# nuggy875/NeRF_pytorch_paeng

Hardware: AMD Instinct MI355X
Metric: rays/sec (4096-ray batch, 64c+128f samples) + 800×800 frame render ms (higher is better)
Workload: dtype f32

## Files before the change

### include/mi_nerf.h

```cpp
#ifndef MI_NERF_H
#define MI_NERF_H

#include <stddef.h>
#include <stdint.h>

#ifdef __cplusplus
extern "C" {
#endif

#define MI_NERF_ABI_VERSION 4

#define MI_NERF_MODE_F32 0
#define MI_NERF_MODE_BF16 1
#define MI_NERF_MODE_BF16_64 2
#define MI_NERF_MODE_BF16_32 3
#define MI_NERF_MODE_F16S 5
#define MI_NERF_MODE_F16S_BF16 6
#define MI_NERF_MODE_F16 8
#define MI_NERF_MODE_F16_BF16 9

#define MI_NERF_OK 0
#define MI_NERF_EINVAL 1
#define MI_NERF_EHIP 2
#define MI_NERF_ERCCL 3

int mi_nerf_abi_version(void);
const char* mi_nerf_last_error(void);

typedef struct mi_nerf_net {
    int32_t D;
    int32_t W;
    int32_t skip;
    int32_t L_x;
    int32_t L_d;
} mi_nerf_net;

typedef struct mi_nerf_params {
    const float* const* linear_x_w;
    const float* const* linear_x_b;
    const float* linear_density_w;
    const float* linear_density_b;
    const float* linear_feat_w;
    const float* linear_feat_b;
    const float* linear_d_w;
    const float* linear_d_b;
    const float* linear_color_w;
    const float* linear_color_b;
} mi_nerf_params;

size_t mi_nerf_packed_bytes(const mi_nerf_net* net);
int mi_nerf_pack_weights(const mi_nerf_net* net, const mi_nerf_params* params, void* host_blob, size_t blob_bytes);
size_t mi_nerf_packed_bytes_bf16(const mi_nerf_net* net);
int mi_nerf_pack_weights_bf16(const mi_nerf_net* net, const mi_nerf_params* params, void* host_blob, size_t blob_bytes);

int mi_nerf_make_o_d(int W, int H, const float k4[4], const float pose12[12], int row0, int n_rows,
                     float* rays_o_dev, float* rays_d_dev, void* stream);
int mi_nerf_make_o_d_pixels(int W, int H, const float k4[4], const float pose12[12], const int64_t* pix_dev,
                            int64_t n, float* rays_o_dev, float* rays_d_dev, void* stream);

int mi_nerf_ndc_rays(int H, int W, float focal, float near_, const float* o_in_dev, int64_t o_stride,
                     const float* d_in_dev, int64_t d_stride, int64_t n, float* o_out_dev, float* d_out_dev,
                     void* stream);

int mi_nerf_fill_uniform(uint32_t seed, uint32_t stream_id, int64_t ray0, int64_t n_rays, int n_samples,
                         float* out_dev, void* stream);

int mi_nerf_stratified_z(int64_t n_rays, int S, float near_, float far_, const float* t_rand_dev, float* z_dev,
                         void* stream);

int mi_nerf_sample_pdf(const float* bins_dev, const float* weights_dev, int64_t n, int B, int N, int det,
                       const float* u_dev, float* samples_dev, void* stream);
int mi_nerf_fine_z(const float* z_c_dev, const float* weights_c_dev, int64_t n, int Sc, int Nf, int det,
                   const float* u_dev, float* z_fine_dev, float* z_samples_dev, void* stream);

int mi_nerf_embed(const float* rays_dev, const float* z_dev, int64_t n_rays, int S, int L_x, int L_d,
                  float* embedded_dev, void* stream);

int mi_nerf_posenc(const float* x_dev, int64_t n, int L, float* out_dev, void* stream);

int mi_nerf_mlp_embedded(const mi_nerf_net* net, const void* packed_dev, const float* x_dev, int64_t n,
                         float* out_dev, void* stream);
int mi_nerf_mlp_rays(const mi_nerf_net* net, const void* packed_dev, const float* rays_dev, const float* z_dev,
                     int64_t n_rays, int S, float* raw_dev, void* stream);
int mi_nerf_mlp_rays_bf16(const mi_nerf_net* net, const void* packed_bf16_dev, const float* rays_dev,
                          const float* z_dev, int64_t n_rays, int S, float* raw_dev, void* stream);
int mi_nerf_mlp_rays_bf16_shape(const mi_nerf_net* net, const void* packed_bf16_dev, const float* rays_dev,
                                const float* z_dev, int64_t n_rays, int S, float* raw_dev, int points_per_wave, void* stream);

size_t mi_nerf_packed_bytes_f16s(const mi_nerf_net* net);
int mi_nerf_pack_weights_f16s(const mi_nerf_net* net, const mi_nerf_params* params, void* host_blob, size_t blob_bytes);
int mi_nerf_mlp_rays_f16s(const mi_nerf_net* net, const void* packed_f16s_dev, const float* rays_dev, const float* z_dev,
                          int64_t n_rays, int S, float* raw_dev, void* stream);
int mi_nerf_mlp_rays_train_f16s(const mi_nerf_net* net, const void* packed_f16s_dev, const float* rays_dev, const float* z_dev,
                                int64_t n_rays, int S, float* raw_dev, void* stash_dev, size_t stash_bytes, void* stream);
size_t mi_nerf_pack_map_f16s_len(const mi_nerf_net* net);
int mi_nerf_pack_map_f16s(const mi_nerf_net* net, int32_t* map_host, size_t map_len);
int mi_nerf_pack_apply_f16s(const mi_nerf_net* net, const int32_t* map_dev, const float* flat_dev, void* blob_dev, size_t blob_bytes,
                            uint32_t* out_of_range_dev, void* stream);
size_t mi_nerf_packed_bytes_bwd_f16s(const mi_nerf_net* net);
int mi_nerf_pack_weights_bwd_f16s(const mi_nerf_net* net, const mi_nerf_params* params, void* host_blob, size_t blob_bytes);
size_t mi_nerf_pack_map_bwd_f16s_len(const mi_nerf_net* net);
int mi_nerf_pack_map_bwd_f16s(const mi_nerf_net* net, int32_t* map_host, size_t map_len);
int mi_nerf_pack_apply_bwd_f16s(const mi_nerf_net* net, const int32_t* map_dev, const float* flat_dev, void* blob_dev, size_t blob_bytes,
                                uint32_t* out_of_range_dev, void* stream);

int mi_nerf_composite(const float* raw_dev, const float* z_dev, const float* rays_dev, int ray_stride, int64_t n,
                      int S, float* rgb_dev, float* disp_dev, float* acc_dev, float* weights_dev,
                      float* depth_dev, void* stream);

typedef struct mi_nerf_render_cfg {
    float near_, far_;
    int32_t Sc, Nf;
    int32_t det;
#if defined(__cplusplus) || (defined(__STDC_VERSION__) && __STDC_VERSION__ >= 201112L)
    union {
        int32_t mode;
        int32_t use_bf16;
    };
#else
    int32_t mode;
#endif
    uint32_t seed;
    uint32_t reserved;
    int64_t ray_offset;
} mi_nerf_render_cfg;
size_t mi_nerf_render_workspace_bytes(const mi_nerf_render_cfg* cfg, int64_t n_rays);
int mi_nerf_render_rays(const mi_nerf_net* net, const void* packed_coarse_dev, const void* packed_fine_dev,
                        const mi_nerf_render_cfg* cfg, const float* rays_dev, int64_t n_rays,
                        const float* t_rand_dev, const float* u_dev, void* workspace_dev, size_t workspace_bytes,
                        float* rgb_c_dev, float* disp_c_dev, float* rgb_f_dev, float* disp_f_dev, void* stream);
typedef struct mi_nerf_workspace_layout {
    size_t z_c, raw_c, weights_c, z_f, raw_f, total;
} mi_nerf_workspace_layout;
int mi_nerf_render_workspace_layout(const mi_nerf_render_cfg* cfg, int64_t n_rays, mi_nerf_workspace_layout* out);

int mi_nerf_composite_backward(const float* raw_dev, const float* z_dev, const float* rays_dev, int ray_stride,
                               int64_t n, int S, const float* d_rgb_dev, float* d_raw_dev, void* stream);

size_t mi_nerf_param_count(const mi_nerf_net* net);

size_t mi_nerf_packed_bytes_bwd(const mi_nerf_net* net);
int mi_nerf_pack_weights_bwd(const mi_nerf_net* net, const mi_nerf_params* params, void* host_blob, size_t blob_bytes);
int mi_nerf_pack_map(const mi_nerf_net* net, int kind, int32_t* map_host, size_t map_len);
int mi_nerf_pack_apply(const int32_t* map_dev, const float* flat_params_dev, size_t blob_bytes, void* blob_dev, void* stream);
size_t mi_nerf_pack_map_bf16_len(const mi_nerf_net* net);
int mi_nerf_pack_map_bf16(const mi_nerf_net* net, int32_t* map_host, size_t map_len);
int mi_nerf_pack_apply_bf16(const mi_nerf_net* net, const int32_t* map_dev, const float* flat_params_dev, void* blob_dev,
                            size_t blob_bytes, void* stream);

typedef struct mi_nerf_train_layout {
    size_t stash_h, stash_f, stash_g;
    size_t mask_h, mask_g, stash_bytes;
    size_t delta_h, delta_f, delta_d, emb, partial, work_bytes;
} mi_nerf_train_layout;
int mi_nerf_train_layout_query(const mi_nerf_net* net, int64_t n_rays, int S, mi_nerf_train_layout* out);

int mi_nerf_mlp_rays_train(const mi_nerf_net* net, const void* packed_dev, const float* rays_dev, const float* z_dev,
                           int64_t n_rays, int S, float* raw_dev, void* stash_dev, size_t stash_bytes, void* stream);
int mi_nerf_mlp_backward(const mi_nerf_net* net, const void* packed_dev, const void* packed_bwd_dev, const float* rays_dev,
                         const float* z_dev, int64_t n_rays, int S, const float* d_raw_dev, const void* stash_dev,
                         void* work_dev, size_t work_bytes, float* grads_dev, int stage, void* stream);
int mi_nerf_mlp_backward_mode(const mi_nerf_net* net, const void* packed_dev, const void* packed_bwd_dev, const float* rays_dev,
                              const float* z_dev, int64_t n_rays, int S, const float* d_raw_dev, const void* stash_dev, void* work_dev,
                              size_t work_bytes, float* grads_dev, int stage, int mode, void* stream);

int mi_nerf_mlp_embedded_train(const mi_nerf_net* net, const void* packed_dev, const float* x_dev, int64_t n, float* out_dev,
                               void* stash_dev, size_t stash_bytes, void* stream);
int mi_nerf_mlp_embedded_backward(const mi_nerf_net* net, const void* packed_dev, const void* packed_bwd_dev, const float* x_dev,
                                  int64_t n, const float* d_out_dev, const void* stash_dev, void* work_dev, size_t work_bytes,
                                  float* grads_dev, void* stream);

size_t mi_nerf_wgrad_scratch_bytes(void);
int mi_nerf_wgrad_products(int n, const float* const* delta_dev, const int* ldd, const int* M, const float* const* x_dev, const int* ldx,
                           const int* N, int64_t P, float* const* out_dev, const int* ldo, float* const* bias_dev, void* scratch_dev,
                           size_t scratch_bytes, int iters, float* avg_ms_out, void* stream);
int mi_nerf_wgrad_products_f16s(int n, const float* const* delta_dev, const int* ldd, const int* M, const float* const* x_dev, const int* ldx,
                                const int* N, int64_t P, float* const* out_dev, const int* ldo, float* const* bias_dev, void* scratch_dev,
                                size_t scratch_bytes, int iters, float* avg_ms, void* stream);

#define MI_NERF_REDUCE_SCRATCH_BYTES 8192
int mi_nerf_image_metrics(const float* pred_dev, const float* target_dev, int64_t n, float* out2_dev, void* scratch_dev,
                          size_t scratch_bytes, void* stream);
int mi_nerf_nanmax(const float* x_dev, int64_t n, float* out_dev, void* scratch_dev, size_t scratch_bytes, void* stream);
int mi_nerf_to8b(const float* x_dev, int64_t n, const float* divisor_dev, uint8_t* out_dev, void* stream);
int mi_nerf_rays_rgb(int W, int H, const float k4[4], const float* poses_dev, const float* images_dev, int64_t n_img,
                     float* rays_rgb_dev, void* stream);
int mi_nerf_permute_rows(const float* src_dev, const int64_t* perm_dev, int64_t n, int row_floats, float* dst_dev, void* stream);

#define MI_NERF_COMM_ID_BYTES 128
int mi_nerf_rccl_available(void);
int mi_nerf_comm_unique_id(void* id_host);
int mi_nerf_comm_init_rank(const void* id_host, int world, int rank, void** comm_out);
int mi_nerf_comm_info(void* comm, int* world_out, int* rank_out, int* device_out);
int mi_nerf_comm_destroy(void* comm);
size_t mi_nerf_all_gather_staging_bytes(int world, int H, int W, int C);
int mi_nerf_all_gather_tiles(void* comm, const float* tile_dev, int rows_local, int H, int W, int C, float* frame_dev, void* staging_dev,
                             size_t staging_bytes, void* stream);
int mi_nerf_unpad_tiles(const float* staging_dev, int world, int H, int W, int C, float* frame_dev, void* stream);

int mi_nerf_time_mlp_rays(const mi_nerf_net* net, const void* packed_dev, const float* rays_dev, const float* z_dev,
                          int64_t n_rays, int S, float* raw_dev, int iters, int mode, float* avg_ms_out,
                          void* stream);

int mi_nerf_selftest_mfma(void* stream);

#ifdef __cplusplus
}
#endif
#endif
```

### nerf_pytorch_paeng_amd/_lib.py

```python
from __future__ import annotations

import ctypes as C
import os
from typing import Optional

import torch

HERE = os.path.dirname(os.path.abspath(__file__))
LIB_PATH = os.environ.get("MI_NERF_LIB") or os.path.join(HERE, "libmi_nerf.so")
ABI_VERSION = 4


class MiNerfError(RuntimeError):
    pass


def loader(module: dict, prefix: str, first=None):
    handle: Optional[C.CDLL] = None

    def lib() -> C.CDLL:
        nonlocal handle
        if handle is None:
            path = module["LIB_PATH"]
            if not os.path.exists(path):
                raise MiNerfError(
                    f"{path} not found: build it with `python -m nerf_pytorch_paeng_amd.build` "
                    "(hipcc --offload-arch=gfx950).  There is no CPU/PyTorch fallback for this path.")
            if first is not None:
                first()
            h = C.CDLL(path)
            for name, (res, args) in module["SIGNATURES"].items():
                try:
                    fn = getattr(h, name)
                except AttributeError as e:
                    raise MiNerfError(f"{path} does not export {name}: stale build?") from e
                fn.restype, fn.argtypes = res, args
            v = getattr(h, prefix + "_abi_version")()
            if v != module["ABI_VERSION"]:
                raise MiNerfError(f"ABI mismatch: library {v}, binding {module['ABI_VERSION']}")
            handle = h
        return handle

    def last_error() -> str:
        msg = getattr(lib(), prefix + "_last_error")()
        return msg.decode() if msg else ""

    def check(rc: int, what: str) -> None:
        if rc != 0:
            raise MiNerfError(f"{what} failed (status {rc}): {last_error() or '?'}")

    return lib, check, last_error


class Net(C.Structure):
    _fields_ = [("D", C.c_int32), ("W", C.c_int32), ("skip", C.c_int32), ("L_x", C.c_int32), ("L_d", C.c_int32)]


class Params(C.Structure):
    _fields_ = [("linear_x_w", C.POINTER(C.c_void_p)), ("linear_x_b", C.POINTER(C.c_void_p)),
                ("linear_density_w", C.c_void_p), ("linear_density_b", C.c_void_p),
                ("linear_feat_w", C.c_void_p), ("linear_feat_b", C.c_void_p),
                ("linear_d_w", C.c_void_p), ("linear_d_b", C.c_void_p),
                ("linear_color_w", C.c_void_p), ("linear_color_b", C.c_void_p)]


class RenderCfg(C.Structure):
    _fields_ = [("near_", C.c_float), ("far_", C.c_float), ("Sc", C.c_int32), ("Nf", C.c_int32),
                ("det", C.c_int32), ("mode", C.c_int32), ("seed", C.c_uint32), ("reserved", C.c_uint32), ("ray_offset", C.c_int64)]


class WorkspaceLayout(C.Structure):
    _fields_ = [("z_c", C.c_size_t), ("raw_c", C.c_size_t), ("weights_c", C.c_size_t), ("z_f", C.c_size_t),
                ("raw_f", C.c_size_t), ("total", C.c_size_t)]


class TrainLayout(C.Structure):
    _fields_ = [(n, C.c_size_t) for n in ("stash_h", "stash_f", "stash_g", "mask_h", "mask_g", "stash_bytes", "delta_h", "delta_f",
                                          "delta_d", "emb", "partial", "work_bytes")]


_P, _I, _I64, _F, _U32, _SZ = C.c_void_p, C.c_int, C.c_int64, C.c_float, C.c_uint32, C.c_size_t
_NETP = C.POINTER(Net)
_CFGP = C.POINTER(RenderCfg)

SIGNATURES = {
    "mi_nerf_abi_version": (_I, []),
    "mi_nerf_last_error": (C.c_char_p, []),
    "mi_nerf_packed_bytes": (_SZ, [_NETP]),
    "mi_nerf_pack_weights": (_I, [_NETP, C.POINTER(Params), _P, _SZ]),
    "mi_nerf_packed_bytes_bf16": (_SZ, [_NETP]),
    "mi_nerf_pack_weights_bf16": (_I, [_NETP, C.POINTER(Params), _P, _SZ]),
    "mi_nerf_make_o_d": (_I, [_I, _I, C.POINTER(_F), C.POINTER(_F), _I, _I, _P, _P, _P]),
    "mi_nerf_make_o_d_pixels": (_I, [_I, _I, C.POINTER(_F), C.POINTER(_F), _P, _I64, _P, _P, _P]),
    "mi_nerf_ndc_rays": (_I, [_I, _I, _F, _F, _P, _I64, _P, _I64, _I64, _P, _P, _P]),
    "mi_nerf_fill_uniform": (_I, [_U32, _U32, _I64, _I64, _I, _P, _P]),
    "mi_nerf_stratified_z": (_I, [_I64, _I, _F, _F, _P, _P, _P]),
    "mi_nerf_sample_pdf": (_I, [_P, _P, _I64, _I, _I, _I, _P, _P, _P]),
    "mi_nerf_fine_z": (_I, [_P, _P, _I64, _I, _I, _I, _P, _P, _P, _P]),
    "mi_nerf_embed": (_I, [_P, _P, _I64, _I, _I, _I, _P, _P]),
    "mi_nerf_posenc": (_I, [_P, _I64, _I, _P, _P]),
    "mi_nerf_mlp_embedded": (_I, [_NETP, _P, _P, _I64, _P, _P]),
    "mi_nerf_mlp_rays": (_I, [_NETP, _P, _P, _P, _I64, _I, _P, _P]),
    "mi_nerf_mlp_rays_bf16": (_I, [_NETP, _P, _P, _P, _I64, _I, _P, _P]),
    "mi_nerf_mlp_rays_bf16_shape": (_I, [_NETP, _P, _P, _P, _I64, _I, _P, _I, _P]),
    "mi_nerf_packed_bytes_f16s": (_SZ, [_NETP]),
    "mi_nerf_pack_weights_f16s": (_I, [_NETP, C.POINTER(Params), _P, _SZ]),
    "mi_nerf_mlp_rays_f16s": (_I, [_NETP, _P, _P, _P, _I64, _I, _P, _P]),
    "mi_nerf_composite": (_I, [_P, _P, _P, _I, _I64, _I, _P, _P, _P, _P, _P, _P]),
    "mi_nerf_render_workspace_bytes": (_SZ, [_CFGP, _I64]),
    "mi_nerf_render_rays": (_I, [_NETP, _P, _P, _CFGP, _P, _I64, _P, _P, _P, _SZ, _P, _P, _P, _P, _P]),
    "mi_nerf_render_workspace_layout": (_I, [_CFGP, _I64, C.POINTER(WorkspaceLayout)]),
    "mi_nerf_composite_backward": (_I, [_P, _P, _P, _I, _I64, _I, _P, _P, _P]),
    "mi_nerf_param_count": (_SZ, [_NETP]),
    "mi_nerf_packed_bytes_bwd": (_SZ, [_NETP]),
    "mi_nerf_pack_weights_bwd": (_I, [_NETP, C.POINTER(Params), _P, _SZ]),
    "mi_nerf_pack_map": (_I, [_NETP, _I, _P, _SZ]),
    "mi_nerf_pack_apply": (_I, [_P, _P, _SZ, _P, _P]),
    "mi_nerf_pack_map_bf16_len": (_SZ, [_NETP]),
    "mi_nerf_pack_map_bf16": (_I, [_NETP, _P, _SZ]),
    "mi_nerf_pack_apply_bf16": (_I, [_NETP, _P, _P, _P, _SZ, _P]),
    "mi_nerf_train_layout_query": (_I, [_NETP, _I64, _I, C.POINTER(TrainLayout)]),
    "mi_nerf_mlp_rays_train": (_I, [_NETP, _P, _P, _P, _I64, _I, _P, _P, _SZ, _P]),
    "mi_nerf_mlp_rays_train_f16s": (_I, [_NETP, _P, _P, _P, _I64, _I, _P, _P, _SZ, _P]),
    "mi_nerf_pack_map_f16s_len": (_SZ, [_NETP]),
    "mi_nerf_pack_map_f16s": (_I, [_NETP, _P, _SZ]),
    "mi_nerf_pack_apply_f16s": (_I, [_NETP, _P, _P, _P, _SZ, _P, _P]),
    "mi_nerf_packed_bytes_bwd_f16s": (_SZ, [_NETP]),
    "mi_nerf_pack_weights_bwd_f16s": (_I, [_NETP, C.POINTER(Params), _P, _SZ]),
    "mi_nerf_pack_map_bwd_f16s_len": (_SZ, [_NETP]),
    "mi_nerf_pack_map_bwd_f16s": (_I, [_NETP, _P, _SZ]),
    "mi_nerf_pack_apply_bwd_f16s": (_I, [_NETP, _P, _P, _P, _SZ, _P, _P]),
    "mi_nerf_mlp_backward": (_I, [_NETP, _P, _P, _P, _P, _I64, _I, _P, _P, _P, _SZ, _P, _I, _P]),
    "mi_nerf_mlp_backward_mode": (_I, [_NETP, _P, _P, _P, _P, _I64, _I, _P, _P, _P, _SZ, _P, _I, _I, _P]),
    "mi_nerf_mlp_embedded_train": (_I, [_NETP, _P, _P, _I64, _P, _P, _SZ, _P]),
    "mi_nerf_mlp_embedded_backward": (_I, [_NETP, _P, _P, _P, _I64, _P, _P, _P, _SZ, _P, _P]),
    "mi_nerf_wgrad_scratch_bytes": (_SZ, []),
    "mi_nerf_wgrad_products": (_I, [_I, _P, _P, _P, _P, _P, _P, _I64, _P, _P, _P, _P, _SZ, _I, C.POINTER(_F), _P]),
    "mi_nerf_wgrad_products_f16s": (_I, [_I, _P, _P, _P, _P, _P, _P, _I64, _P, _P, _P, _P, _SZ, _I, C.POINTER(_F), _P]),
    "mi_nerf_image_metrics": (_I, [_P, _P, _I64, _P, _P, _SZ, _P]),
    "mi_nerf_nanmax": (_I, [_P, _I64, _P, _P, _SZ, _P]),
    "mi_nerf_to8b": (_I, [_P, _I64, _P, _P, _P]),
    "mi_nerf_rays_rgb": (_I, [_I, _I, C.POINTER(_F), _P, _P, _I64, _P, _P]),
    "mi_nerf_permute_rows": (_I, [_P, _P, _I64, _I, _P, _P]),
    "mi_nerf_rccl_available": (_I, []),
    "mi_nerf_comm_unique_id": (_I, [_P]),
    "mi_nerf_comm_init_rank": (_I, [_P, _I, _I, C.POINTER(_P)]),
    "mi_nerf_comm_info": (_I, [_P, C.POINTER(_I), C.POINTER(_I), C.POINTER(_I)]),
    "mi_nerf_comm_destroy": (_I, [_P]),
    "mi_nerf_all_gather_staging_bytes": (_SZ, [_I, _I, _I, _I]),
    "mi_nerf_all_gather_tiles": (_I, [_P, _P, _I, _I, _I, _I, _P, _P, _SZ, _P]),
    "mi_nerf_unpad_tiles": (_I, [_P, _I, _I, _I, _I, _P, _P]),
    "mi_nerf_time_mlp_rays": (_I, [_NETP, _P, _P, _P, _I64, _I, _P, _I, _I, C.POINTER(_F), _P]),
    "mi_nerf_selftest_mfma": (_I, [_P]),
}

lib, check, last_error = loader(globals(), "mi_nerf")


def dev_ptr(t: Optional[torch.Tensor], name: str = "tensor", dtype=torch.float32, align: int = 4) -> Optional[int]:
    if t is None:
        return None
    if not t.is_cuda:
        raise MiNerfError(f"{name} must live on a HIP device (got {t.device}); this path has no CPU fallback")
    if t.dtype != dtype:
        raise MiNerfError(f"{name} must be {dtype} (got {t.dtype})")
    if not t.is_contiguous():
        raise MiNerfError(f"{name} must be contiguous")
    p = t.data_ptr()
    if p % align:
        raise MiNerfError(f"{name} must be {align}-byte aligned")
    return p


def stream_ptr(device: torch.device) -> int:
    return torch.cuda.current_stream(device).cuda_stream


def as_f32_dev(t, device=None) -> torch.Tensor:
    if not isinstance(t, torch.Tensor):
        t = torch.as_tensor(t)
    if device is not None and t.device != torch.device(device):
        t = t.to(device)
    if t.dtype != torch.float32:
        t = t.float()
    return t.contiguous()
```

### nerf_pytorch_paeng_amd/csrc/api.hip

```cpp
#include <string>
#include "half_layout.h"

namespace minerf {

ABI_ERROR_STATE(, MI_NERF_EHIP)

int device_cus() {
    static std::atomic<int> cus[MN_MAX_DEVICES] = {};
    int dev = 0;
    if (hipGetDevice(&dev) != hipSuccess) return 256;
    std::atomic<int>& slot = cus[dev & (MN_MAX_DEVICES - 1)];
    int c = slot.load(std::memory_order_relaxed);
    if (c <= 0) {
        hipDeviceProp_t prop;
        c = (hipGetDeviceProperties(&prop, dev) == hipSuccess && prop.multiProcessorCount > 0) ? prop.multiProcessorCount : 256;
        slot.store(c, std::memory_order_relaxed);
    }
    return c;
}
int ensure_lds_opt_in(LdsOptIn& state, const void* kernel) {
    int dev = 0;
    MN_HIP(hipGetDevice(&dev));
    std::atomic<bool>& done = state.done[dev & (MN_MAX_DEVICES - 1)];
    if (!done.load(std::memory_order_acquire)) {
        MN_HIP(hipFuncSetAttribute(kernel, hipFuncAttributeMaxDynamicSharedMemorySize, 160 * 1024));
        done.store(true, std::memory_order_release);
    }
    return MI_NERF_OK;
}

int mlp_rays_fp32(const mi_nerf_net*, const void*, const float*, const float*, int64_t, int, float*, hipStream_t);
int mlp_embedded_fp32(const mi_nerf_net*, const void*, const float*, int64_t, float*, hipStream_t);
int mlp_rays_bf16(const mi_nerf_net*, const void*, const float*, const float*, int64_t, int, float*, hipStream_t, int points_per_wave, const StratDraw* strat,
                  FineDraw* fine = nullptr);
int mlp_rays_f16(const mi_nerf_net*, const void*, const float*, const float*, int64_t, int, float*, hipStream_t, int points_per_wave, const StratDraw* strat,
                 FineDraw* fine);
int mlp_rays_f16s(const mi_nerf_net*, const void*, const float*, const float*, int64_t, int, float*, hipStream_t);
int mlp_rays_f16s_stash(const mi_nerf_net*, const void*, const float*, const float*, int64_t, int, float*, float*, float*, float*, unsigned*, unsigned*,
                        hipStream_t);
int wgrad_products(int, const float* const*, const int*, const int*, const float* const*, const int*, const int*, int64_t, float* const*, const int*,
                   float* const*, void*, size_t, hipStream_t, bool);
int mlp_rays_fp32_stash(const mi_nerf_net*, const void*, const float*, const float*, int64_t, int, float*, float*, float*, float*, unsigned*,
                        unsigned*, hipStream_t);
int mlp_backward_fp32(const mi_nerf_net*, const void*, const void*, const float*, const float*, int64_t, int, const float*, const void*, void*,
                      size_t, float*, int, hipStream_t, const float*, int64_t, int);
int mlp_embedded_fp32_stash(const mi_nerf_net*, const void*, const float*, int64_t, float*, float*, float*, float*, unsigned*, unsigned*,
                            hipStream_t);
int train_layout(const mi_nerf_net*, int64_t, int, mi_nerf_train_layout*);
size_t wgrad_scratch_bytes();
int pack_apply(const int32_t*, const float*, size_t, void*, hipStream_t);
int frames_image_metrics(const float*, const float*, int64_t, float*, void*, size_t, hipStream_t);
int frames_nanmax(const float*, int64_t, float*, void*, size_t, hipStream_t);
int frames_to8b(const float*, int64_t, const float*, unsigned char*, hipStream_t);
int frames_rays_rgb(int, int, const float*, const float*, const float*, int64_t, float*, hipStream_t);
int frames_permute_rows(const float*, const int64_t*, int64_t, int, float*, hipStream_t);
int stage_make_o_d(int, int, const float*, const float*, int, int, float*, float*, hipStream_t);
int stage_make_o_d_pixels(int, int, const float*, const float*, const int64_t*, int64_t, float*, float*, hipStream_t);
int stage_ndc(int, int, float, float, const float*, int64_t, const float*, int64_t, int64_t, float*, float*, hipStream_t);
int stage_fill_uniform(uint32_t, uint32_t, int64_t, int64_t, int, float*, hipStream_t);
int stage_stratified(int64_t, int, float, float, const float*, uint32_t, int64_t, float*, hipStream_t);
int stage_embed(const float*, const float*, int64_t, int, int, int, float*, hipStream_t);
int stage_posenc(const float*, int64_t, int, float*, hipStream_t);
int stage_composite(const float*, const float*, const float*, int, int64_t, int, float*, float*, float*, float*, float*, hipStream_t);
int stage_composite_backward(const float*, const float*, const float*, int, int64_t, int, const float*, float*, hipStream_t);
int stage_sample_pdf(const float*, const float*, int64_t, int, int, int, const float*, float*, hipStream_t);
int stage_fine_z(const float*, const float*, int64_t, int, int, int, const float*, uint32_t, int64_t, float*, float*, hipStream_t);
int stage_composite_fine_z(const float*, const float*, const float*, int64_t, int, int, int, const float*, uint32_t, int64_t, float*, float*, float*,
                           float*, hipStream_t);

static int check_net_basic(const mi_nerf_net* net) {
    MN_CHECK_ARG(net != nullptr, "net is NULL");
    MN_CHECK_ARG(net->W >= 2 && net->W <= MAX_KERNEL_WIDTH, "unsupported width W=%d (the fp32 inference kernels run 2 <= W <= %d, padded to 128 / 256 / 384 / 512; "
                 "training, bf16 and split precision: 128 / 256 and 256)", net->W, MAX_KERNEL_WIDTH);
    MN_CHECK_ARG(net->D >= 2 && net->D <= 16, "unsupported depth D=%d", net->D);
    MN_CHECK_ARG(net->L_x >= 0 && net->L_x <= 10 && net->L_d >= 0 && net->L_d <= 4,
                 "unsupported encoding L_x=%d L_d=%d (the kernels evaluate up to 10 / 4 frequencies; fewer run with zero weights on the rest)", net->L_x, net->L_d);
    MN_CHECK_ARG(net->skip >= -1, "bad skip=%d", net->skip);
    return MI_NERF_OK;
}

enum class Family { FP32, F16S, BF16, F16 };
struct ModePlan { Family coarse, fine; int points_per_wave; };

static int mode_plan(int mode, ModePlan* p) {
    switch (mode) {
        case MI_NERF_MODE_F32:       *p = {Family::FP32, Family::FP32, 0}; return MI_NERF_OK;
        case MI_NERF_MODE_BF16:      *p = {Family::BF16, Family::BF16, 0}; return MI_NERF_OK;
        case MI_NERF_MODE_BF16_64:   *p = {Family::BF16, Family::BF16, 64}; return MI_NERF_OK;
        case MI_NERF_MODE_BF16_32:   *p = {Family::BF16, Family::BF16, 32}; return MI_NERF_OK;
        case MI_NERF_MODE_F16S:      *p = {Family::F16S, Family::F16S, 0}; return MI_NERF_OK;
        case MI_NERF_MODE_F16S_BF16: *p = {Family::F16S, Family::BF16, 0}; return MI_NERF_OK;
        case MI_NERF_MODE_F16:       *p = {Family::F16, Family::F16, 0}; return MI_NERF_OK;
        case MI_NERF_MODE_F16_BF16:  *p = {Family::F16, Family::BF16, 0}; return MI_NERF_OK;
    }
    set_error("mode must be one of MI_NERF_MODE_* (0..3, 5, 6, 8, 9; got %d)", mode);
    return MI_NERF_EINVAL;
}

static int mlp_rays_family(Family family, const mi_nerf_net* net, const void* packed, const float* rays, const float* z, int64_t n, int S, float* raw,
                           hipStream_t st, int points_per_wave, const StratDraw* strat = nullptr, FineDraw* fine = nullptr) {
    if (family == Family::FP32) return mlp_rays_fp32(net, packed, rays, z, n, S, raw, st);
    if (family == Family::F16S) return mlp_rays_f16s(net, packed, rays, z, n, S, raw, st);
    return (family == Family::F16 ? mlp_rays_f16 : mlp_rays_bf16)(net, packed, rays, z, n, S, raw, st, points_per_wave, strat, fine);
}

static inline size_t align256(size_t v) { return (v + 255) & ~(size_t)255; }

static int workspace_layout(const mi_nerf_render_cfg* cfg, int64_t n, mi_nerf_workspace_layout* L) {
    MN_CHECK_ARG(cfg && L, "NULL cfg/layout");
    MN_CHECK_ARG(n >= 0 && cfg->Sc >= 1 && cfg->Nf >= 0, "bad sizes n=%lld Sc=%d Nf=%d", (long long)n, cfg->Sc, cfg->Nf);
    MN_CHECK_ARG(cfg->Nf == 0 || cfg->Sc >= 3, "hierarchical sampling needs at least 3 coarse samples");
    size_t off = 0;
    const size_t nn = (size_t)n, Sc = (size_t)cfg->Sc, St = (size_t)(cfg->Sc + cfg->Nf);
    L->z_c = off;       off += align256(nn * Sc * 4);
    L->raw_c = off;     off += align256(nn * Sc * 16);
    L->weights_c = off; off += align256(nn * Sc * 4);
    L->z_f = off;       off += cfg->Nf > 0 ? align256(nn * St * 4) : 0;
    L->raw_f = off;     off += cfg->Nf > 0 ? align256(nn * St * 16) : 0;
    L->total = off;
    return MI_NERF_OK;
}

__global__ void mfma_selftest_kernel(const float* __restrict__ A, const float* __restrict__ B, float* __restrict__ D) {
    const int lane = threadIdx.x & 63;
    f32x16 acc;
#pragma unroll
    for (int r = 0; r < 16; ++r) acc[r] = 0.0f;
#pragma unroll
    for (int s = 0; s < 4; ++s) {
        const int k = 2 * s + (lane >> 5);
        const float a = A[(lane & 31) * 8 + k];
        const float b = B[k * 32 + (lane & 31)];
        acc = __builtin_amdgcn_mfma_f32_32x32x2f32(a, b, acc, 0, 0, 0);
    }
#pragma unroll
    for (int r = 0; r < 16; ++r) {
        const int i = (r & 3) + 8 * (r >> 2) + 4 * (lane >> 5);
        D[i * 32 + (lane & 31)] = acc[r];
    }
}

}

using namespace minerf;

extern "C" {

int mi_nerf_abi_version(void) { return MI_NERF_ABI_VERSION; }
const char* mi_nerf_last_error(void) { return g_err; }

size_t mi_nerf_packed_bytes(const mi_nerf_net* net) {
    if (check_net_basic(net)) return 0;
    return make_layout(net->D, net->W, net->skip, net->L_x, net->L_d).total_bytes;
}
int mi_nerf_pack_weights(const mi_nerf_net* net, const mi_nerf_params* params, void* blob, size_t bytes) {
    if (int rc = check_net_basic(net)) return rc;
    MN_CHECK_ARG(params && blob, "NULL params/blob");
    MN_CHECK_ARG(params->linear_x_w && params->linear_x_b && params->linear_density_w && params->linear_density_b &&
                 params->linear_feat_w && params->linear_feat_b && params->linear_d_w && params->linear_d_b &&
                 params->linear_color_w && params->linear_color_b, "NULL parameter pointer");
    for (int l = 0; l < net->D; ++l) MN_CHECK_ARG(params->linear_x_w[l] && params->linear_x_b[l], "NULL trunk layer %d", l);
    return pack_fp32(net, params, blob, bytes);
}
size_t mi_nerf_packed_bytes_bf16(const mi_nerf_net* net) {
    if (check_net_basic(net)) return 0;
    return packed_bytes_bf16(net);
}
size_t mi_nerf_packed_bytes_f16s(const mi_nerf_net* net) {
    return packed_bytes_f16s(net);
}
int mi_nerf_pack_weights_f16s(const mi_nerf_net* net, const mi_nerf_params* params, void* blob, size_t bytes) {
    MN_CHECK_ARG(net && params && blob, "NULL argument");
    return pack_f16s(net, params, blob, bytes);
}
int mi_nerf_pack_weights_bf16(const mi_nerf_net* net, const mi_nerf_params* params, void* blob, size_t bytes) {
    if (int rc = check_net_basic(net)) return rc;
    MN_CHECK_ARG(params && blob, "NULL params/blob");
    return pack_bf16(net, params, blob, bytes);
}

int mi_nerf_make_o_d(int W, int H, const float k4[4], const float pose12[12], int row0, int n_rows, float* o, float* d, void* st) {
    MN_CHECK_ARG(k4 && pose12, "NULL camera");
    return stage_make_o_d(W, H, k4, pose12, row0, n_rows, o, d, (hipStream_t)st);
}
int mi_nerf_make_o_d_pixels(int W, int H, const float k4[4], const float pose12[12], const int64_t* pix, int64_t n, float* o,
                            float* d, void* st) {
    MN_CHECK_ARG(k4 && pose12, "NULL camera");
    return stage_make_o_d_pixels(W, H, k4, pose12, pix, n, o, d, (hipStream_t)st);
}
int mi_nerf_ndc_rays(int H, int W, float focal, float near_, const float* o_in, int64_t os, const float* d_in, int64_t ds, int64_t n,
                     float* o_out, float* d_out, void* st) {
    return stage_ndc(H, W, focal, near_, o_in, os, d_in, ds, n, o_out, d_out, (hipStream_t)st);
}
int mi_nerf_fill_uniform(uint32_t seed, uint32_t stream_id, int64_t ray0, int64_t n_rays, int S, float* out, void* st) {
    return stage_fill_uniform(seed, stream_id, ray0, n_rays, S, out, (hipStream_t)st);
}
int mi_nerf_stratified_z(int64_t n_rays, int S, float near_, float far_, const float* t_rand, float* z, void* st) {
    MN_CHECK_ARG(t_rand != nullptr || n_rays == 0, "t_rand is NULL");
    return stage_stratified(n_rays, S, near_, far_, t_rand, 0, 0, z, (hipStream_t)st);
}
int mi_nerf_sample_pdf(const float* bins, const float* weights, int64_t n, int B, int N, int det, const float* u, float* out, void* st) {
    return stage_sample_pdf(bins, weights, n, B, N, det, u, out, (hipStream_t)st);
}
int mi_nerf_fine_z(const float* z_c, const float* w_c, int64_t n, int Sc, int Nf, int det, const float* u, float* z_f, float* z_s,
                   void* st) {
    MN_CHECK_ARG(det || u != nullptr || n == 0, "u is NULL (and det == 0)");
    return stage_fine_z(z_c, w_c, n, Sc, Nf, det, u, 0, 0, z_f, z_s, (hipStream_t)st);
}
int mi_nerf_embed(const float* rays, const float* z, int64_t n_rays, int S, int L_x, int L_d, float* out, void* st) {
    return stage_embed(rays, z, n_rays, S, L_x, L_d, out, (hipStream_t)st);
}
int mi_nerf_posenc(const float* x, int64_t n, int L, float* out, void* st) { return stage_posenc(x, n, L, out, (hipStream_t)st); }
int mi_nerf_mlp_embedded(const mi_nerf_net* net, const void* packed, const float* x, int64_t n, float* out, void* st) {
    return mlp_embedded_fp32(net, packed, x, n, out, (hipStream_t)st);
}
int mi_nerf_mlp_rays(const mi_nerf_net* net, const void* packed, const float* rays, const float* z, int64_t n_rays, int S, float* raw,
                     void* st) {
    return mlp_rays_fp32(net, packed, rays, z, n_rays, S, raw, (hipStream_t)st);
}
int mi_nerf_mlp_rays_bf16(const mi_nerf_net* net, const void* packed, const float* rays, const float* z, int64_t n_rays, int S,
                          float* raw, void* st) {
    MN_CHECK_ARG(z != nullptr || n_rays == 0, "z is NULL");
    return mlp_rays_bf16(net, packed, rays, z, n_rays, S, raw, (hipStream_t)st, 0, nullptr);
}
int mi_nerf_mlp_rays_f16s(const mi_nerf_net* net, const void* packed, const float* rays, const float* z, int64_t n_rays, int S, float* raw,
                          void* st) {
    return mlp_rays_f16s(net, packed, rays, z, n_rays, S, raw, (hipStream_t)st);
}
int mi_nerf_mlp_rays_bf16_shape(const mi_nerf_net* net, const void* packed, const float* rays, const float* z, int64_t n_rays, int S,
                                float* raw, int points_per_wave, void* st) {
    MN_CHECK_ARG(z != nullptr || n_rays == 0, "z is NULL");
    return mlp_rays_bf16(net, packed, rays, z, n_rays, S, raw, (hipStream_t)st, points_per_wave, nullptr);
}
int mi_nerf_composite(const float* raw, const float* z, const float* rays, int ray_stride, int64_t n, int S, float* rgb, float* disp,
                      float* acc, float* weights, float* depth, void* st) {
    return stage_composite(raw, z, rays, ray_stride, n, S, rgb, disp, acc, weights, depth, (hipStream_t)st);
}

int mi_nerf_composite_backward(const float* raw, const float* z, const float* rays, int ray_stride, int64_t n, int S,
                               const float* d_rgb, float* d_raw, void* st) {
    return stage_composite_backward(raw, z, rays, ray_stride, n, S, d_rgb, d_raw, (hipStream_t)st);
}

size_t mi_nerf_param_count(const mi_nerf_net* net) {
    if (check_net_basic(net)) return 0;
    return make_param_offsets(net->D, net->W, net->skip, net->L_x, net->L_d).total;
}
size_t mi_nerf_packed_bytes_bwd(const mi_nerf_net* net) {
    if (check_net_basic(net)) return 0;
    return packed_bytes_bwd(net);
}
int mi_nerf_pack_weights_bwd(const mi_nerf_net* net, const mi_nerf_params* params, void* host_blob, size_t blob_bytes) {
    if (int rc = check_net_basic(net)) return rc;
    MN_CHECK_ARG(params && host_blob, "NULL params/blob");
    return pack_bwd_fp32(net, params, host_blob, blob_bytes);
}
int mi_nerf_pack_map(const mi_nerf_net* net, int kind, int32_t* map_host, size_t map_len) {
    if (int rc = check_net_basic(net)) return rc;
    return pack_map(net, kind, map_host, map_len);
}
size_t mi_nerf_pack_map_bf16_len(const mi_nerf_net* net) {
    if (!net) return 0;
    return pack_map_bf16_len(net);
}
int mi_nerf_pack_map_bf16(const mi_nerf_net* net, int32_t* map_host, size_t map_len) {
    MN_CHECK_ARG(net && map_host, "NULL pointer");
    return pack_map_bf16(net, map_host, map_len);
}
int mi_nerf_pack_apply_bf16(const mi_nerf_net* net, const int32_t* map_dev, const float* flat_dev, void* blob_dev, size_t blob_bytes, void* st) {
    MN_CHECK_ARG(net, "net is NULL");
    return pack_apply_bf16(net, map_dev, flat_dev, blob_dev, blob_bytes, (hipStream_t)st);
}
int mi_nerf_pack_apply(const int32_t* map_dev, const float* flat_dev, size_t blob_bytes, void* blob_dev, void* st) {
    return pack_apply(map_dev, flat_dev, blob_bytes, blob_dev, (hipStream_t)st);
}
int mi_nerf_train_layout_query(const mi_nerf_net* net, int64_t n_rays, int S, mi_nerf_train_layout* out) {
    if (int rc = check_net_basic(net)) return rc;
    return train_layout(net, n_rays, S, out);
}
int mi_nerf_mlp_rays_train(const mi_nerf_net* net, const void* packed, const float* rays, const float* z, int64_t n_rays, int S,
                           float* raw, void* stash, size_t stash_bytes, void* st) {
    if (int rc = check_net_basic(net)) return rc;
    MN_CHECK_ARG(n_rays >= 0 && S >= 1, "bad sizes n_rays=%lld S=%d", (long long)n_rays, S);
    mi_nerf_train_layout L;
    if (int rc = train_layout(net, n_rays, S, &L)) return rc;
    if (n_rays == 0) return MI_NERF_OK;
    MN_CHECK_ARG(stash != nullptr && stash_bytes >= L.stash_bytes, "stash too small: %zu < %zu", stash_bytes, L.stash_bytes);
    return mlp_rays_fp32_stash(net, packed, rays, z, n_rays, S, raw, (float*)((char*)stash + L.stash_h), (float*)((char*)stash + L.stash_f),
                               (float*)((char*)stash + L.stash_g), (unsigned*)((char*)stash + L.mask_h), (unsigned*)((char*)stash + L.mask_g),
                               (hipStream_t)st);
}
int mi_nerf_mlp_rays_train_f16s(const mi_nerf_net* net, const void* packed_f16s, const float* rays, const float* z, int64_t n_rays, int S,
                                float* raw, void* stash, size_t stash_bytes, void* st) {
    if (int rc = check_net_basic(net)) return rc;
    MN_CHECK_ARG(n_rays >= 0 && S >= 1, "bad sizes n_rays=%lld S=%d", (long long)n_rays, S);
    mi_nerf_train_layout L;
    if (int rc = train_layout(net, n_rays, S, &L)) return rc;
    if (n_rays == 0) return MI_NERF_OK;
    MN_CHECK_ARG(stash != nullptr && stash_bytes >= L.stash_bytes, "stash too small: %zu < %zu", stash_bytes, L.stash_bytes);
    return mlp_rays_f16s_stash(net, packed_f16s, rays, z, n_rays, S, raw, (float*)((char*)stash + L.stash_h), (float*)((char*)stash + L.stash_f),
                               (float*)((char*)stash + L.stash_g), (unsigned*)((char*)stash + L.mask_h), (unsigned*)((char*)stash + L.mask_g),
                               (hipStream_t)st);
}
size_t mi_nerf_pack_map_f16s_len(const mi_nerf_net* net) {
    if (!net) return 0;
    return pack_map_f16s_len(net);
}
int mi_nerf_pack_map_f16s(const mi_nerf_net* net, int32_t* map_host, size_t map_len) {
    MN_CHECK_ARG(net && map_host, "NULL pointer");
    return pack_map_f16s(net, map_host, map_len);
}
size_t mi_nerf_packed_bytes_bwd_f16s(const mi_nerf_net* net) {
    if (!net) return 0;
    return packed_bytes_bwd_f16s(net);
}
int mi_nerf_pack_weights_bwd_f16s(const mi_nerf_net* net, const mi_nerf_params* params, void* host_blob, size_t blob_bytes) {
    MN_CHECK_ARG(net && params && host_blob, "NULL pointer");
    return pack_bwd_f16s(net, params, host_blob, blob_bytes);
}
size_t mi_nerf_pack_map_bwd_f16s_len(const mi_nerf_net* net) {
    if (!net) return 0;
    return pack_map_bwd_f16s_len(net);
}
int mi_nerf_pack_map_bwd_f16s(const mi_nerf_net* net, int32_t* map_host, size_t map_len) {
    MN_CHECK_ARG(net && map_host, "NULL pointer");
    return pack_map_bwd_f16s(net, map_host, map_len);
}
int mi_nerf_pack_apply_bwd_f16s(const mi_nerf_net* net, const int32_t* map_dev, const float* flat_dev, void* blob_dev, size_t blob_bytes,
                                uint32_t* out_of_range_dev, void* st) {
    MN_CHECK_ARG(net, "net is NULL");
    return pack_apply_bwd_f16s(net, map_dev, flat_dev, blob_dev, blob_bytes, out_of_range_dev, (hipStream_t)st);
}
int mi_nerf_pack_apply_f16s(const mi_nerf_net* net, const int32_t* map_dev, const float* flat_dev, void* blob_dev, size_t blob_bytes,
                            uint32_t* out_of_range_dev, void* st) {
    MN_CHECK_ARG(net, "net is NULL");
    return pack_apply_f16s(net, map_dev, flat_dev, blob_dev, blob_bytes, out_of_range_dev, (hipStream_t)st);
}
int mi_nerf_mlp_backward(const mi_nerf_net* net, const void* packed, const void* packed_bwd, const float* rays, const float* z,
                         int64_t n_rays, int S, const float* d_raw, const void* stash, void* work, size_t work_bytes, float* grads,
                         int stage, void* st) {
    if (int rc = check_net_basic(net)) return rc;
    return mlp_backward_fp32(net, packed, packed_bwd, rays, z, n_rays, S, d_raw, stash, work, work_bytes, grads, stage, (hipStream_t)st, nullptr, -1, 0);
}
int mi_nerf_mlp_backward_mode(const mi_nerf_net* net, const void* packed, const void* packed_bwd, const float* rays, const float* z,
                              int64_t n_rays, int S, const float* d_raw, const void* stash, void* work, size_t work_bytes, float* grads,
                              int stage, int mode, void* st) {
    if (int rc = check_net_basic(net)) return rc;
    MN_CHECK_ARG((mode & ~3) == 0, "unknown backward mode %d", mode);
    return mlp_backward_fp32(net, packed, packed_bwd, rays, z, n_rays, S, d_raw, stash, work, work_bytes, grads, stage, (hipStream_t)st, nullptr, -1, mode);
}
int mi_nerf_mlp_embedded_train(const mi_nerf_net* net, const void* packed, const float* x, int64_t n, float* out, void* stash, size_t stash_bytes,
                               void* st) {
    if (int rc = check_net_basic(net)) return rc;
    MN_CHECK_ARG(n >= 0, "bad n=%lld", (long long)n);
    mi_nerf_train_layout L;
    if (int rc = train_layout(net, (n + 31) / 32, 32, &L)) return rc;
    if (n == 0) return MI_NERF_OK;
    MN_CHECK_ARG(stash != nullptr && stash_bytes >= L.stash_bytes, "stash too small: %zu < %zu", stash_bytes, L.stash_bytes);
    return mlp_embedded_fp32_stash(net, packed, x, n, out, (float*)((char*)stash + L.stash_h), (float*)((char*)stash + L.stash_f),
                                   (float*)((char*)stash + L.stash_g), (unsigned*)((char*)stash + L.mask_h), (unsigned*)((char*)stash + L.mask_g),
                                   (hipStream_t)st);
}
int mi_nerf_mlp_embedded_backward(const mi_nerf_net* net, const void* packed, const void* packed_bwd, const float* x, int64_t n, const float* d_out,
                                  const void* stash, void* work, size_t work_bytes, float* grads, void* st) {
    if (int rc = check_net_basic(net)) return rc;
    MN_CHECK_ARG(n >= 0, "bad n=%lld", (long long)n);
    MN_CHECK_ARG(x != nullptr || n == 0, "NULL device pointer");
    static const float no_rows = 0.0f;
    return mlp_backward_fp32(net, packed, packed_bwd, nullptr, nullptr, (n + 31) / 32, 32, d_out, stash, work, work_bytes, grads, 0, (hipStream_t)st,
                             x ? x : &no_rows, n, 0);
}

int mi_nerf_image_metrics(const float* pred, const float* target, int64_t n, float* out2, void* scratch, size_t scratch_bytes, void* st) {
    return frames_image_metrics(pred, target, n, out2, scratch, scratch_bytes, (hipStream_t)st);
}
int mi_nerf_nanmax(const float* x, int64_t n, float* out, void* scratch, size_t scratch_bytes, void* st) {
    return frames_nanmax(x, n, out, scratch, scratch_bytes, (hipStream_t)st);
}
int mi_nerf_to8b(const float* x, int64_t n, const float* divisor, uint8_t* out, void* st) {
    return frames_to8b(x, n, divisor, out, (hipStream_t)st);
}
int mi_nerf_rays_rgb(int W, int H, const float k4[4], const float* poses, const float* images, int64_t n_img, float* out, void* st) {
    return frames_rays_rgb(W, H, k4, poses, images, n_img, out, (hipStream_t)st);
}
int mi_nerf_permute_rows(const float* src, const int64_t* perm, int64_t n, int row_floats, float* dst, void* st) {
    return frames_permute_rows(src, perm, n, row_floats, dst, (hipStream_t)st);
}

size_t mi_nerf_render_workspace_bytes(const mi_nerf_render_cfg* cfg, int64_t n_rays) {
    mi_nerf_workspace_layout L;
    if (workspace_layout(cfg, n_rays, &L)) return 0;
    return L.total;
}
int mi_nerf_render_workspace_layout(const mi_nerf_render_cfg* cfg, int64_t n_rays, mi_nerf_workspace_layout* out) {
    return workspace_layout(cfg, n_rays, out);
}

int mi_nerf_render_rays(const mi_nerf_net* net, const void* packed_c, const void* packed_f, const mi_nerf_render_cfg* cfg,
                        const float* rays, int64_t n, const float* t_rand, const float* u, void* ws, size_t ws_bytes,
                        float* rgb_c, float* disp_c, float* rgb_f, float* disp_f, void* stream) {
    hipStream_t st = (hipStream_t)stream;
    mi_nerf_workspace_layout L;
    if (int rc = workspace_layout(cfg, n, &L)) return rc;
    if (n == 0) return MI_NERF_OK;
    MN_CHECK_ARG(ws_bytes >= L.total, "workspace too small: %zu < %zu", ws_bytes, L.total);
    MN_CHECK_ARG(rays && rgb_c && disp_c && packed_c && (ws || L.total == 0), "NULL pointer");
    MN_CHECK_ARG(cfg->Nf == 0 || (packed_f && rgb_f && disp_f), "fine pass needs packed_fine and outputs");
    MN_CHECK_ARG(cfg->reserved == 0, "mi_nerf_render_cfg.reserved must be 0");
    char* w = (char*)ws;
    float* z_c = (float*)(w + L.z_c);
    float* raw_c = (float*)(w + L.raw_c);
    float* wts_c = (float*)(w + L.weights_c);
    const int Sc = cfg->Sc, St = cfg->Sc + cfg->Nf;
    ModePlan p;
    if (int rc = mode_plan(cfg->mode, &p)) return rc;
    if (p.coarse == Family::F16 || p.fine == Family::F16)
        if (int rc = check_net_half(net, "f16")) return rc;
    FineDraw fd{};
    if (p.coarse == Family::BF16 || p.coarse == Family::F16) {
        const StratDraw sd{cfg->near_, cfg->far_, t_rand, cfg->seed, cfg->ray_offset, z_c};
        if (cfg->Nf > 0) fd = FineDraw{cfg->Nf, cfg->det, u, cfg->seed, cfg->ray_offset, rgb_c, disp_c, wts_c, (float*)(w + L.z_f), false};
        if (int rc = mlp_rays_family(p.coarse, net, packed_c, rays, nullptr, n, Sc, raw_c, st, p.points_per_wave, &sd,
                                     cfg->Nf > 0 && p.points_per_wave == 0 ? &fd : nullptr))
            return rc;
    } else {
        if (int rc = stage_stratified(n, Sc, cfg->near_, cfg->far_, t_rand, cfg->seed, cfg->ray_offset, z_c, st)) return rc;
        if (int rc = mlp_rays_family(p.coarse, net, packed_c, rays, z_c, n, Sc, raw_c, st, p.points_per_wave)) return rc;
    }
    if (cfg->Nf == 0) return stage_composite(raw_c, z_c, rays, 6, n, Sc, rgb_c, disp_c, nullptr, wts_c, nullptr, st);
    {
        float* z_f = (float*)(w + L.z_f);
        float* raw_f = (float*)(w + L.raw_f);
        if (!fd.taken)
            if (int rc = stage_composite_fine_z(raw_c, z_c, rays, n, Sc, cfg->Nf, cfg->det, u, cfg->seed, cfg->ray_offset, rgb_c, disp_c, wts_c, z_f, st))
                return rc;
        if (int rc = mlp_rays_family(p.fine, net, packed_f, rays, z_f, n, St, raw_f, st, p.points_per_wave)) return rc;
        if (int rc = stage_composite(raw_f, z_f, rays, 6, n, St, rgb_f, disp_f, nullptr, nullptr, nullptr, st)) return rc;
    }
    return MI_NERF_OK;
}

int mi_nerf_time_mlp_rays(const mi_nerf_net* net, const void* packed, const float* rays, const float* z, int64_t n_rays, int S,
                          float* raw, int iters, int mode, float* avg_ms, void* stream) {
    hipStream_t st = (hipStream_t)stream;
    MN_CHECK_ARG(iters >= 1 && avg_ms, "bad iters / NULL output");
    ModePlan p;
    if (int rc = mode_plan(mode, &p)) return rc;
    MN_CHECK_ARG(p.coarse == p.fine, "MI_NERF_MODE_* %d is two kernel families (mi_nerf_render_rays only): one network, one kernel family", mode);
    if (p.fine == Family::F16)
        if (int rc = check_net_half(net, "f16")) return rc;
    hipEvent_t e0, e1;
    MN_HIP(hipEventCreate(&e0));
    MN_HIP(hipEventCreate(&e1));
    int rc = MI_NERF_OK;
    MN_HIP(hipEventRecord(e0, st));
    for (int i = 0; i < iters && rc == MI_NERF_OK; ++i)
        rc = mlp_rays_family(p.fine, net, packed, rays, z, n_rays, S, raw, st, p.points_per_wave);
    MN_HIP(hipEventRecord(e1, st));
    MN_HIP(hipEventSynchronize(e1));
    float ms = 0.f;
    MN_HIP(hipEventElapsedTime(&ms, e0, e1));
    (void)hipEventDestroy(e0);
    (void)hipEventDestroy(e1);
    *avg_ms = ms / (float)iters;
    return rc;
}

size_t mi_nerf_wgrad_scratch_bytes(void) { return wgrad_scratch_bytes(); }
extern "C++" template <typename F>
static int timed_launches(int iters, float* avg_ms, hipStream_t st, F body) {
    MN_CHECK_ARG(iters >= 1, "bad iters");
    hipEvent_t e0 = nullptr, e1 = nullptr;
    if (avg_ms) {
        MN_HIP(hipEventCreate(&e0));
        MN_HIP(hipEventCreate(&e1));
        MN_HIP(hipEventRecord(e0, st));
    }
    int rc = MI_NERF_OK;
    for (int i = 0; i < iters && rc == MI_NERF_OK; ++i) rc = body();
    if (avg_ms) {
        MN_HIP(hipEventRecord(e1, st));
        MN_HIP(hipEventSynchronize(e1));
        float ms = 0.f;
        MN_HIP(hipEventElapsedTime(&ms, e0, e1));
        (void)hipEventDestroy(e0);
        (void)hipEventDestroy(e1);
        *avg_ms = ms / (float)iters;
    }
    return rc;
}
int mi_nerf_wgrad_products(int n, const float* const* delta, const int* ldd, const int* M, const float* const* x, const int* ldx, const int* N,
                           int64_t P, float* const* out, const int* ldo, float* const* bias, void* scratch, size_t scratch_bytes, int iters,
                           float* avg_ms, void* stream) {
    hipStream_t st = (hipStream_t)stream;
    return timed_launches(iters, avg_ms, st, [&] { return wgrad_products(n, delta, ldd, M, x, ldx, N, P, out, ldo, bias, scratch, scratch_bytes, st, false); });
}
int mi_nerf_wgrad_products_f16s(int n, const float* const* delta, const int* ldd, const int* M, const float* const* x, const int* ldx, const int* N,
                                int64_t P, float* const* out, const int* ldo, float* const* bias, void* scratch, size_t scratch_bytes, int iters,
                                float* avg_ms, void* stream) {
    hipStream_t st = (hipStream_t)stream;
    return timed_launches(iters, avg_ms, st, [&] { return wgrad_products(n, delta, ldd, M, x, ldx, N, P, out, ldo, bias, scratch, scratch_bytes, st, true); });
}

int mi_nerf_selftest_mfma(void* stream) {
    hipStream_t st = (hipStream_t)stream;
    float hA[32 * 8], hB[8 * 32], hD[32 * 32], ref[32 * 32];
    for (int i = 0; i < 32; ++i) for (int k = 0; k < 8; ++k) hA[i * 8 + k] = (float)((i * 3 + k * 7) % 11 - 5);
    for (int k = 0; k < 8; ++k) for (int j = 0; j < 32; ++j) hB[k * 32 + j] = (float)((k * 5 + j * 2 + (j > 9)) % 13 - 6);
    for (int i = 0; i < 32; ++i) for (int j = 0; j < 32; ++j) {
        float s = 0.f;
        for (int k = 0; k < 8; ++k) s += hA[i * 8 + k] * hB[k * 32 + j];
        ref[i * 32 + j] = s;
    }
    float *dA, *dB, *dD;
    MN_HIP(hipMalloc(&dA, sizeof(hA)));
    MN_HIP(hipMalloc(&dB, sizeof(hB)));
    MN_HIP(hipMalloc(&dD, sizeof(hD)));
    MN_HIP(hipMemcpyAsync(dA, hA, sizeof(hA), hipMemcpyHostToDevice, st));
    MN_HIP(hipMemcpyAsync(dB, hB, sizeof(hB), hipMemcpyHostToDevice, st));
    hipLaunchKernelGGL(mfma_selftest_kernel, dim3(1), dim3(64), 0, st, dA, dB, dD);
    MN_LAUNCH_CHECK("mfma_selftest_kernel");
    MN_HIP(hipMemcpyAsync(hD, dD, sizeof(hD), hipMemcpyDeviceToHost, st));
    MN_HIP(hipStreamSynchronize(st));
    (void)hipFree(dA); (void)hipFree(dB); (void)hipFree(dD);
    for (int i = 0; i < 32 * 32; ++i)
        if (hD[i] != ref[i]) {
            set_error("MFMA layout mismatch at D[%d][%d]: got %g want %g", i / 32, i % 32, hD[i], ref[i]);
            return MI_NERF_EINVAL;
        }
    return MI_NERF_OK;
}

}
```

### nerf_pytorch_paeng_amd/csrc/layout.h

```cpp
#pragma once
#include <stdint.h>
#include <stddef.h>

namespace minerf {

constexpr int QUAD_BYTES = 1024;
constexpr int SLOT_QUADS = 16;
constexpr int SLOT_BYTES = QUAD_BYTES * SLOT_QUADS;
constexpr int HEADER_BYTES = 1024;
constexpr uint32_t BLOB_MAGIC = 0x4D494E46u;

__host__ __device__ constexpr int pe_ksteps(int L) { return ((3 * L + 2 + 3) / 4) * 4; }

constexpr int KERNEL_LX = 10, KERNEL_LD = 4;

constexpr int MAX_KERNEL_WIDTH = 512;
__host__ __device__ constexpr int kernel_width(int W) { return W <= 128 ? 128 : (W <= 256 ? 256 : (W <= 384 ? 384 : 512)); }
__host__ __device__ constexpr bool wide_kernel_width(int Wk) { return Wk > 256; }
__host__ __device__ constexpr int pe_ksteps16(int L) { return (((3 * L + 1) / 2 + 1 + 3) / 4) * 4; }
__host__ __device__ constexpr bool native_width(int W) { return W == 128 || W == 256; }

struct BlobLayout {
    uint32_t stream_off;
    uint32_t stream_bytes_hoist;
    uint32_t stream_bytes_full;
    uint32_t side_off;
    uint32_t side_floats;
    uint32_t bias_trunk;
    uint32_t bias_feat;
    uint32_t bias_d;
    uint32_t dens_w;
    uint32_t dens_b;
    uint32_t color_w;
    uint32_t color_b;
    uint32_t wdir_t;
    uint32_t total_bytes;
};

__host__ __device__ inline uint32_t round_up_u32(uint32_t v, uint32_t m) { return (v + m - 1) / m * m; }

inline BlobLayout make_layout(int D, int W_net, int skip, int , int ) {
    constexpr int L_x = KERNEL_LX, L_d = KERNEL_LD;
    const int W = kernel_width(W_net);
    BlobLayout b{};
    const int NT = W / 32;
    const int in_d = 3 + 6 * L_d;
    const uint32_t pe_quads = (uint32_t)(pe_ksteps(L_x) / 4) * NT;
    const uint32_t h_quads = (uint32_t)(W / 2 / 4) * NT;
    uint32_t quads = pe_quads;
    for (int l = 1; l < D; ++l) quads += h_quads + ((skip >= 0 && l == skip + 1) ? pe_quads : 0);
    quads += h_quads;
    quads += (uint32_t)(W / 2 / 4) * (NT / 2);
    b.stream_off = HEADER_BYTES;
    b.stream_bytes_hoist = round_up_u32(quads, SLOT_QUADS) * QUAD_BYTES;
    uint32_t full = round_up_u32(quads, SLOT_QUADS) + round_up_u32((uint32_t)(pe_ksteps(L_d) / 4) * (NT / 2), SLOT_QUADS);
    b.stream_bytes_full = full * QUAD_BYTES;
    b.side_off = b.stream_off + b.stream_bytes_full;
    uint32_t f = 0;
    b.bias_trunk = f; f += (uint32_t)D * W;
    b.bias_feat = f;  f += W;
    b.bias_d = f;     f += W / 2;
    b.dens_w = f;     f += W;
    b.dens_b = f;     f += 4;
    b.color_w = f;    f += 3 * (W / 2);
    b.color_b = f;    f += 4;
    b.wdir_t = f;     f += (uint32_t)in_d * (W / 2);
    b.side_floats = round_up_u32(f, 4);
    b.total_bytes = b.side_off + b.side_floats * 4;
    return b;
}

struct ParamOffsets {
    uint32_t w_x[16], b_x[16];
    int in_l[16];
    uint32_t w_d, b_d, w_feat, b_feat, w_dens, b_dens, w_color, b_color;
    uint32_t total;
};

inline ParamOffsets make_param_offsets(int D, int W, int skip, int L_x, int L_d) {
    ParamOffsets p{};
    const int in_x = 3 + 6 * L_x, in_d = 3 + 6 * L_d;
    uint32_t f = 0;
    for (int l = 0; l < D; ++l) {
        p.in_l[l] = (l == 0) ? in_x : ((skip >= 0 && l == skip + 1) ? W + in_x : W);
        p.w_x[l] = f; f += (uint32_t)W * p.in_l[l];
        p.b_x[l] = f; f += W;
    }
    p.w_d = f;     f += (uint32_t)(W / 2) * (W + in_d);
    p.b_d = f;     f += W / 2;
    p.w_feat = f;  f += (uint32_t)W * W;
    p.b_feat = f;  f += W;
    p.w_dens = f;  f += W;
    p.b_dens = f;  f += 1;
    p.w_color = f; f += 3 * (W / 2);
    p.b_color = f; f += 3;
    p.total = f;
    return p;
}

inline uint32_t bwd_stream_bytes(int D, int W) {
    const uint32_t NT = W / 32;
    const uint32_t quads = (uint32_t)(W / 16) * NT + (uint32_t)D * (uint32_t)(W / 8) * NT;
    return round_up_u32(quads, SLOT_QUADS) * QUAD_BYTES;
}

}
```

### nerf_pytorch_paeng_amd/csrc/mlp_fp32.hip

```cpp
#include <stdlib.h>
#include <vector>
#include "common.h"
#include "layout.h"
#include "mlp_core.h"


namespace minerf {


struct MlpArgs {
    const char* stream;
    const float* side;
    const float* rays;
    const float* z;
    const float* x;
    int Lx_net, Ld_net;
    float* out;
    long long n_wtiles;
    long long n_pts;
    long long n_rays, walk_ray, walk_carry, n_iter;
    int walk_chunk, ray_major;
    int S;
    int tpr;
    int D;
    int skip_layer;
    unsigned stream_bytes;
    unsigned side_floats;
    unsigned o_bias_trunk, o_bias_feat, o_bias_d, o_dens_w, o_dens_b, o_color_w, o_color_b, o_wdir_t;
    unsigned long long* diag;
    float* stash_h;
    float* stash_f;
    float* stash_g;
    unsigned* mask_h;
    unsigned* mask_g;
    long long stash_rows;
};


template <int L, bool SLOW, int NPE>
__device__ __forceinline__ void encode_regs(float (&pe)[NPE], const float (&p)[3], int hh) {
#pragma unroll
    for (int s = 0; s < 3 * L; ++s) {
        const float y = p[s % 3] * (float)(1 << (s / 3));
        pe[s] = SLOW ? sin_cos_slow(y, hh) : sin_cos_fast(y, hh);
    }
    pe[3 * L] = hh ? p[1] : p[0];
    pe[3 * L + 1] = hh ? 0.0f : p[2];
#pragma unroll
    for (int s = 3 * L + 2; s < NPE; ++s) pe[s] = 0.0f;
}

template <int L, int NPE>
__device__ __forceinline__ void gather_regs(float (&pe)[NPE], const float* row, int hh, bool valid, int L_net) {
#pragma unroll
    for (int s = 0; s < 3 * L; ++s) {
        const int ch = 3 + 6 * (s / 3) + (s % 3) + 3 * hh;
        const bool have = valid && (s / 3) < L_net;
        pe[s] = have ? row[have ? ch : 0] : 0.0f;
    }
    pe[3 * L] = valid ? row[hh] : 0.0f;
    pe[3 * L + 1] = (valid && !hh) ? row[2] : 0.0f;
#pragma unroll
    for (int s = 3 * L + 2; s < NPE; ++s) pe[s] = 0.0f;
}

template <int W, int MODE, int LX, int LD, bool STASH>
__global__ __launch_bounds__(256) __attribute__((amdgpu_waves_per_eu(1, 1)))
void mlp_fp32_kernel(const MlpArgs a) {
    constexpr int NT = W / 32;
    constexpr int HN = W / 2;
    constexpr int KPE = pe_ksteps(LX);
    constexpr int KDE = pe_ksteps(LD);
    constexpr int IN_D = 3 + 6 * LD;
    constexpr int HK_B = NT - 3, HK_M = NT - 2, HK_S = NT - 1;
    constexpr int AL = STASH ? 8 : 4;
    extern __shared__ __attribute__((aligned(16))) char smem[];
    float* side = (float*)(smem + RING_BYTES);
    const int tid = threadIdx.x;
    const int lane = tid & 63;
    const int wave = __builtin_amdgcn_readfirstlane(tid >> 6);
    const int col = lane & 31, hh = lane >> 5;
    float* scratch = side + a.side_floats + wave * (W / 2);

    for (unsigned i = tid * 4; i < a.side_floats; i += 256 * 4) *(f32x4*)(side + i) = *(const f32x4*)(a.side + i);

    const long long n_wg_tiles = (a.n_wtiles + 3) >> 2;
    if ((long long)blockIdx.x >= n_wg_tiles) return;

    WRing ring = ring_start(a.stream, a.stream_bytes, smem, wave, lane);

    f32x16 acc[8];
    f32x4 aq[8];
    float h[HN];
    float pe[KPE];
    ring_advance(ring);
#pragma unroll
    for (int t = 0; t < NT; ++t) aq[t] = ring_read(smem, ring, lane, t);

#ifdef MN_DIAG
    unsigned long long seg[8] = {0, 0, 0, 0, 0, 0, 0, 0};
    unsigned long long tprev = mn_stamp();
#endif
    long long t_ray = 0;
    int t_chunk = 0;
    long long bias_ray = -1;
    float nx_o[3] = {0.f, 0.f, 0.f}, nx_d[3] = {0.f, 0.f, 0.f}, nx_z = 0.f;
    auto tile_inputs = [&](long long ray, int chunk) __attribute__((always_inline)) {
        const int sample = chunk * 32 + col;
        const int sc = sample < a.S ? sample : a.S - 1;
        const float* rp = a.rays + ray * 6;
        nx_o[0] = rp[0]; nx_o[1] = rp[1]; nx_o[2] = rp[2]; nx_d[0] = rp[3]; nx_d[1] = rp[4]; nx_d[2] = rp[5];
        nx_z = a.z[ray * a.S + sc];
    };
    const long long wid = (long long)blockIdx.x * 4 + wave;
    if constexpr (MODE == 0) {
        if (a.ray_major) { t_ray = wid; t_chunk = 0; }
        else { t_ray = wid / a.tpr; t_chunk = (int)(wid - t_ray * a.tpr); }
        const bool in = t_ray < a.n_rays;
        tile_inputs(in ? t_ray : a.n_rays - 1, in ? t_chunk : a.tpr - 1);
    }
    for (long long it = 0; it < a.n_iter; ++it) {
#ifdef MN_DIAG
        ring.dlog = (a.diag && it == 2 && blockIdx.x < 4) ? a.diag + (size_t)gridDim.x * 32 + ((size_t)blockIdx.x * 4 + wave) * 512 : nullptr;
        ring.dcnt = 0;
#endif
        bool wave_active;
        long long wt;
        bool valid;
        long long out_idx;
        float de[KDE];
        if constexpr (MODE == 0) {
            wave_active = t_ray < a.n_rays;
            const long long ray = wave_active ? t_ray : a.n_rays - 1;
            const int chunk = wave_active ? t_chunk : a.tpr - 1;
            wt = ray * a.tpr + chunk;
            const int sample = chunk * 32 + col;
            valid = wave_active && sample < a.S;
            const int sc = sample < a.S ? sample : a.S - 1;
            out_idx = ray * a.S + sc;
            const float ox = nx_o[0], oy = nx_o[1], oz = nx_o[2], dx = nx_d[0], dy = nx_d[1], dz = nx_d[2];
            const float zv = nx_z;
            t_ray += a.walk_ray;
            t_chunk += a.walk_chunk;
            if (t_chunk >= a.tpr) { t_chunk -= a.tpr; t_ray += a.walk_carry; }
            {
                const bool in = t_ray < a.n_rays;
                tile_inputs(in ? t_ray : a.n_rays - 1, in ? t_chunk : a.tpr - 1);
            }
            const float p[3] = {ox + dx * zv, oy + dy * zv, oz + dz * zv};
            const float amax = __builtin_fmaxf(__builtin_fmaxf(__builtin_fabsf(p[0]), __builtin_fabsf(p[1])), __builtin_fabsf(p[2])) * (float)(1 << (LX - 1));
            if (__builtin_expect(amax < SINCOS_FAST_LIMIT, 1)) encode_regs<LX, false>(pe, p, hh);
            else encode_regs<LX, true>(pe, p, hh);
            if (ray != bias_ray) {
                bias_ray = ray;
                const float nrm = __builtin_sqrtf(dx * dx + dy * dy + dz * dz);
                const float v[3] = {dx / nrm, dy / nrm, dz / nrm};
                float g[IN_D];
                g[0] = v[0]; g[1] = v[1]; g[2] = v[2];
#pragma unroll
                for (int k = 0; k < LD; ++k)
#pragma unroll
                    for (int c = 0; c < 3; ++c) {
                        const float y = v[c] * (float)(1 << k);
                        g[3 + 6 * k + c] = sin_cos_fast(y, 0);
                        g[3 + 6 * k + 3 + c] = sin_cos_fast(y, 1);
                    }
                const float* wdt = side + a.o_wdir_t;
                const float* bd = side + a.o_bias_d;
#pragma unroll
                for (int n0 = 0; n0 < W / 2; n0 += 64) {
                    const int n = n0 + lane;
                    float sacc = bd[n];
#pragma unroll
                    for (int f = 0; f < IN_D; ++f) sacc = __builtin_fmaf(wdt[f * (W / 2) + n], g[f], sacc);
                    scratch[n] = sacc;
                }
            }
        } else {
            wt = it * ((long long)gridDim.x * 4) + wid;
            wave_active = wt < a.n_wtiles;
            if (!wave_active) wt = a.n_wtiles - 1;
            const long long p0 = wt * 32 + col;
            valid = wave_active && p0 < a.n_pts;
            out_idx = p0 < a.n_pts ? p0 : a.n_pts - 1;
            const int in_x_net = 3 + 6 * a.Lx_net;
            const float* row = a.x + out_idx * (in_x_net + 3 + 6 * a.Ld_net);
            gather_regs<LX>(pe, row, hh, true, a.Lx_net);
            gather_regs<LD>(de, row + in_x_net, hh, true, a.Ld_net);
        }

        MN_STAMP(0);
        acc_init<NT>(acc, side + a.o_bias_trunk, hh);
        gemm_part<NT, KPE, NT, AL>(acc, pe, aq, smem, ring, lane);
        MN_STAMP(1);
#pragma unroll 1
        for (int l = 1; l < a.D; ++l) {
            acc_to_b<NT, true>(acc, h);
            acc_init<NT>(acc, side + a.o_bias_trunk + l * W, hh);
            if (l == a.skip_layer) gemm_part<NT, KPE, NT, AL>(acc, pe, aq, smem, ring, lane);
            if constexpr (STASH) {
                float* row = a.stash_h + ((long long)(l - 1) * a.stash_rows + out_idx) * W + 4 * hh;
                unsigned mw[4] = {0u, 0u, 0u, 0u};
                unsigned mb[4];
                auto hook = [&](int kq, int t) __attribute__((always_inline)) {
                    if (t == HK_B) mask_bits_chunk(h, kq, mb);
                    if (t == HK_M) mask_merge_chunk(mb, kq, mw);
                    if (t == HK_S) store_chunk(h, kq, row);
                };
                gemm_part<NT, HN, NT, AL>(acc, h, aq, smem, ring, lane, hook);
                if (wave_active) {
                    u32x4 m; m[0] = mw[0]; m[1] = mw[1]; m[2] = mw[2]; m[3] = mw[3];
                    *(u32x4*)(a.mask_h + (((long long)(l - 1) * a.n_wtiles + wt) * 64 + lane) * 4) = m;
                }
            } else {
                gemm_part<NT, HN, NT, AL>(acc, h, aq, smem, ring, lane);
            }
        }
        acc_to_b<NT, true>(acc, h);
        MN_STAMP(2);
        const float dens = xhalf_sum(dot_half<HN>(h, side + a.o_dens_w, hh)) + side[a.o_dens_b];
        acc_init<NT>(acc, side + a.o_bias_feat, hh);
        if constexpr (STASH) {
            float* row = a.stash_h + ((long long)(a.D - 1) * a.stash_rows + out_idx) * W + 4 * hh;
            unsigned mw[4] = {0u, 0u, 0u, 0u};
            unsigned mb[4];
            auto hook = [&](int kq, int t) __attribute__((always_inline)) {
                if (t == HK_B) mask_bits_chunk(h, kq, mb);
                if (t == HK_M) mask_merge_chunk(mb, kq, mw);
                if (t == HK_S) store_chunk(h, kq, row);
            };
            gemm_part<NT, HN, NT / 2, AL>(acc, h, aq, smem, ring, lane, hook);
            if (wave_active) {
                u32x4 m; m[0] = mw[0]; m[1] = mw[1]; m[2] = mw[2]; m[3] = mw[3];
                *(u32x4*)(a.mask_h + (((long long)(a.D - 1) * a.n_wtiles + wt) * 64 + lane) * 4) = m;
            }
        } else {
            gemm_part<NT, HN, NT / 2, AL>(acc, h, aq, smem, ring, lane);
        }
        acc_to_b<NT, false>(acc, h);
        MN_STAMP(3);
        if constexpr (MODE == 0) {
            acc_init<NT / 2>(acc, scratch, hh);
            if constexpr (STASH) {
                float* row = a.stash_f + out_idx * W + 4 * hh;
                auto hook = [&](int kq, int t) __attribute__((always_inline)) {
                    if (t == NT / 2 - 1) store_chunk(h, kq, row);
                };
                gemm_part<NT / 2, HN, NT, AL>(acc, h, aq, smem, ring, lane, hook);
            } else {
                gemm_part<NT / 2, HN, NT, AL>(acc, h, aq, smem, ring, lane);
            }
        } else {
            acc_init<NT / 2>(acc, side + a.o_bias_d, hh);
            if constexpr (STASH) {
                float* row = a.stash_f + out_idx * W + 4 * hh;
                auto hook = [&](int kq, int t) __attribute__((always_inline)) {
                    if (t == NT / 2 - 1) store_chunk(h, kq, row);
                };
                gemm_part<NT / 2, HN, NT / 2, AL>(acc, h, aq, smem, ring, lane, hook);
            } else {
                gemm_part<NT / 2, HN, NT / 2, AL>(acc, h, aq, smem, ring, lane);
            }
            gemm_part<NT / 2, KDE, NT, AL>(acc, de, aq, smem, ring, lane);
        }
        float h2[HN / 2];
        acc_to_b<NT / 2, true>(acc, h2);
        if constexpr (STASH) {
            store_rows<NT / 2>(h2, a.stash_g + out_idx * (W / 2) + 4 * hh, valid);
            unsigned mg[2] = {0u, 0u};
#pragma unroll
            for (int q = 0; q < HN / 8; ++q) mask_pack_chunk(h2, q, mg);
            if (wave_active) {
                u32x2 m; m[0] = mg[0]; m[1] = mg[1];
                *(u32x2*)(a.mask_g + (wt * 64 + lane) * 2) = m;
            }
        }
        MN_STAMP(4);
        const float* cw = side + a.o_color_w;
        const float r0 = xhalf_sum(dot_half<HN / 2>(h2, cw, hh)) + side[a.o_color_b + 0];
        const float r1 = xhalf_sum(dot_half<HN / 2>(h2, cw + W / 2, hh)) + side[a.o_color_b + 1];
        const float r2 = xhalf_sum(dot_half<HN / 2>(h2, cw + W, hh)) + side[a.o_color_b + 2];
        if (valid && hh == 0) {
            f32x4 o; o[0] = r0; o[1] = r1; o[2] = r2; o[3] = dens;
            *(f32x4*)(a.out + out_idx * 4) = o;
        }
        MN_STAMP(5);
    }
#ifdef MN_DIAG
    if (a.diag && lane == 0) {
        unsigned long long* d = a.diag + ((size_t)blockIdx.x * 4 + wave) * 8;
        for (int i = 0; i < 8; ++i) d[i] = seg[i];
    }
#endif
    asm volatile("s_waitcnt vmcnt(0)" ::: "memory");
    __syncthreads();
}

static int check_net(const mi_nerf_net* net) {
    MN_CHECK_ARG(net != nullptr, "net is NULL");
    MN_CHECK_ARG(net->W >= 2 && net->W <= MAX_KERNEL_WIDTH, "unsupported width W=%d (the fp32 inference kernels run 2 <= W <= %d, padded to 128 / 256 / 384 / 512)", net->W, MAX_KERNEL_WIDTH);
    MN_CHECK_ARG(net->D >= 2 && net->D <= 16, "unsupported depth D=%d", net->D);
    MN_CHECK_ARG(net->L_x >= 0 && net->L_x <= KERNEL_LX && net->L_d >= 0 && net->L_d <= KERNEL_LD,
                 "unsupported encoding L_x=%d L_d=%d (the kernels evaluate up to %d / %d frequencies)", net->L_x, net->L_d, KERNEL_LX, KERNEL_LD);
    MN_CHECK_ARG(net->skip >= -1, "bad skip=%d", net->skip);
    return MI_NERF_OK;
}

static int num_cus() { return device_cus(); }

int mlp_rays_fp32_wide(const mi_nerf_net*, const void*, const float*, const float*, int64_t, int, float*, hipStream_t);
int mlp_embedded_fp32_wide(const mi_nerf_net*, const void*, const float*, int64_t, float*, hipStream_t);

template <int W, int MODE, bool STASH = false>
static int launch(const MlpArgs& args_in, long long n_wtiles, hipStream_t st) {
    MlpArgs args = args_in;
    const size_t lds = RING_BYTES + (size_t)args.side_floats * 4 + 4 * (W / 2) * 4;
    MN_CHECK_ARG(lds <= 160 * 1024, "LDS budget exceeded: %zu bytes", lds);
    auto kern = mlp_fp32_kernel<W, MODE, 10, 4, STASH>;
    static LdsOptIn opt_in = {};
    if (int rc = ensure_lds_opt_in(opt_in, (const void*)kern)) return rc;
    const long long n_wg = (n_wtiles + 3) / 4;
    const int grid = (int)(n_wg < (long long)num_cus() ? n_wg : (long long)num_cus());
    {
        const long long NW = (long long)grid * 4;
        const long long it_ray = (args.n_rays + NW - 1) / NW * args.tpr, it_flat = (n_wg + grid - 1) / grid;
        args.ray_major = (MODE == 0 && args.n_rays >= NW && it_ray <= it_flat) ? 1 : 0;
        if (args.ray_major) {
            args.walk_ray = 0; args.walk_chunk = 1; args.walk_carry = NW;
            args.n_iter = (args.n_rays + NW - 1) / NW * args.tpr;
        } else {
            const long long tpr = MODE == 0 ? args.tpr : 1;
            args.walk_ray = NW / tpr; args.walk_chunk = (int)(NW % tpr); args.walk_carry = 1;
            args.n_iter = (n_wg + grid - 1) / grid;
        }
    }
#ifdef MN_DIAG
    {
        MlpArgs da = args;
        unsigned long long* dbuf = nullptr;
        const size_t n = (size_t)grid * 4 * 8 + 16 * 512;
        MN_HIP(hipMalloc(&dbuf, n * 8));
        MN_HIP(hipMemsetAsync(dbuf, 0, n * 8, st));
        da.diag = dbuf;
        hipLaunchKernelGGL(kern, dim3(grid), dim3(256), lds, st, da);
        MN_HIP(hipStreamSynchronize(st));
        std::vector<unsigned long long> hbuf(n);
        MN_HIP(hipMemcpy(hbuf.data(), dbuf, n * 8, hipMemcpyDeviceToHost));
        (void)hipFree(dbuf);
        const double tiles = (double)((n_wg + grid - 1) / grid);
        static const char* names[6] = {"prologue", "layer0", "trunk", "dens+feature", "viewdir", "colour+store"};
        double tot = 0;
        fprintf(stderr, "[mn_diag] W=%d MODE=%d grid=%d tiles/wg=%.1f  cycles per tile (mean over waves):\n", W, MODE, grid, tiles);
        for (int sgi = 0; sgi < 6; ++sgi) {
            double sum = 0;
            for (size_t w = 0; w < (size_t)grid * 4; ++w) sum += (double)hbuf[w * 8 + sgi];
            const double per = sum / ((double)grid * 4) / tiles;
            tot += per;
            fprintf(stderr, "[mn_diag]   %-14s %10.0f\n", names[sgi], per);
        }
        fprintf(stderr, "[mn_diag]   %-14s %10.0f\n", "total", tot);
        if (const char* e = getenv("MN_DIAG_KQ")) {
            const int wsel = atoi(e);
            const unsigned long long* lg = hbuf.data() + (size_t)grid * 32 + (size_t)wsel * 512;
            fprintf(stderr, "[mn_diag] k-quad deltas (cycles; ideal %d) of wave %d, tile 2:", 4 * 64 * (W / 32), wsel);
            for (int i = 1; i < 500 && lg[i]; ++i) fprintf(stderr, "%s%llu", (i % 16 == 1) ? "\n[mn_diag]   " : " ", lg[i] - lg[i - 1]);
            fprintf(stderr, "\n");
        }
        return MI_NERF_OK;
    }
#endif
    hipLaunchKernelGGL(kern, dim3(grid), dim3(256), lds, st, args);
    MN_LAUNCH_CHECK("mlp_fp32_kernel");
    return MI_NERF_OK;
}

static void fill_common(MlpArgs& a, const mi_nerf_net* net, const void* packed_dev, bool full_stream) {
    const BlobLayout L = make_layout(net->D, net->W, net->skip, net->L_x, net->L_d);
    a.stream = (const char*)packed_dev + L.stream_off;
    a.side = (const float*)((const char*)packed_dev + L.side_off);
    a.D = net->D;
    a.Lx_net = net->L_x; a.Ld_net = net->L_d;
    a.skip_layer = (net->skip >= 0 && net->skip + 1 < net->D) ? net->skip + 1 : -1;
    a.stream_bytes = full_stream ? L.stream_bytes_full : L.stream_bytes_hoist;
    a.side_floats = L.side_floats;
    a.o_bias_trunk = L.bias_trunk; a.o_bias_feat = L.bias_feat; a.o_bias_d = L.bias_d;
    a.o_dens_w = L.dens_w; a.o_dens_b = L.dens_b; a.o_color_w = L.color_w; a.o_color_b = L.color_b;
    a.o_wdir_t = L.wdir_t;
}

int mlp_rays_fp32(const mi_nerf_net* net, const void* packed_dev, const float* rays_dev, const float* z_dev,
                  int64_t n_rays, int S, float* raw_dev, hipStream_t st) {
    if (int rc = check_net(net)) return rc;
    MN_CHECK_ARG(n_rays >= 0 && S >= 1, "bad sizes n_rays=%lld S=%d", (long long)n_rays, S);
    if (n_rays == 0) return MI_NERF_OK;
    MN_CHECK_ARG(packed_dev && rays_dev && z_dev && raw_dev, "NULL device pointer");
    if (wide_kernel_width(kernel_width(net->W))) return mlp_rays_fp32_wide(net, packed_dev, rays_dev, z_dev, n_rays, S, raw_dev, st);
    MlpArgs a{};
    fill_common(a, net, packed_dev, false);
    a.rays = rays_dev; a.z = z_dev; a.out = raw_dev; a.S = S; a.tpr = (S + 31) / 32;
    a.n_wtiles = (long long)n_rays * a.tpr; a.n_rays = n_rays;
    return kernel_width(net->W) == 256 ? launch<256, 0>(a, a.n_wtiles, st) : launch<128, 0>(a, a.n_wtiles, st);
}

int mlp_rays_fp32_stash(const mi_nerf_net* net, const void* packed_dev, const float* rays_dev, const float* z_dev,
                        int64_t n_rays, int S, float* raw_dev, float* stash_h, float* stash_f, float* stash_g, unsigned* mask_h,
                        unsigned* mask_g, hipStream_t st) {
    if (int rc = check_net(net)) return rc;
    MN_CHECK_ARG(native_width(net->W), "the training kernels exist for W = 128 and 256 (got %d)", net->W);
    MN_CHECK_ARG(n_rays >= 0 && S >= 1, "bad sizes n_rays=%lld S=%d", (long long)n_rays, S);
    if (n_rays == 0) return MI_NERF_OK;
    MN_CHECK_ARG(packed_dev && rays_dev && z_dev && raw_dev && stash_h && stash_f && stash_g && mask_h && mask_g, "NULL device pointer");
    MlpArgs a{};
    fill_common(a, net, packed_dev, false);
    a.rays = rays_dev; a.z = z_dev; a.out = raw_dev; a.S = S; a.tpr = (S + 31) / 32;
    a.n_wtiles = (long long)n_rays * a.tpr; a.n_rays = n_rays;
    a.stash_h = stash_h; a.stash_f = stash_f; a.stash_g = stash_g; a.stash_rows = (long long)n_rays * S;
    a.mask_h = mask_h; a.mask_g = mask_g;
    return net->W == 256 ? launch<256, 0, true>(a, a.n_wtiles, st) : launch<128, 0, true>(a, a.n_wtiles, st);
}

int mlp_embedded_fp32_stash(const mi_nerf_net* net, const void* packed_dev, const float* x_dev, int64_t n, float* out_dev, float* stash_h,
                            float* stash_f, float* stash_g, unsigned* mask_h, unsigned* mask_g, hipStream_t st) {
    if (int rc = check_net(net)) return rc;
    MN_CHECK_ARG(native_width(net->W), "the training kernels exist for W = 128 and 256 (got %d)", net->W);
    MN_CHECK_ARG(n >= 0, "bad n=%lld", (long long)n);
    if (n == 0) return MI_NERF_OK;
    MN_CHECK_ARG(packed_dev && x_dev && out_dev && stash_h && stash_f && stash_g && mask_h && mask_g, "NULL device pointer");
    MlpArgs a{};
    fill_common(a, net, packed_dev, true);
    a.x = x_dev; a.out = out_dev; a.n_pts = n;
    a.n_wtiles = (n + 31) / 32;
    a.stash_h = stash_h; a.stash_f = stash_f; a.stash_g = stash_g; a.stash_rows = a.n_wtiles * 32;
    a.mask_h = mask_h; a.mask_g = mask_g;
    return net->W == 256 ? launch<256, 1, true>(a, a.n_wtiles, st) : launch<128, 1, true>(a, a.n_wtiles, st);
}

int mlp_embedded_fp32(const mi_nerf_net* net, const void* packed_dev, const float* x_dev, int64_t n, float* out_dev,
                      hipStream_t st) {
    if (int rc = check_net(net)) return rc;
    MN_CHECK_ARG(n >= 0, "bad n=%lld", (long long)n);
    if (n == 0) return MI_NERF_OK;
    MN_CHECK_ARG(packed_dev && x_dev && out_dev, "NULL device pointer");
    if (wide_kernel_width(kernel_width(net->W))) return mlp_embedded_fp32_wide(net, packed_dev, x_dev, n, out_dev, st);
    MlpArgs a{};
    fill_common(a, net, packed_dev, true);
    a.x = x_dev; a.out = out_dev; a.n_pts = n;
    a.n_wtiles = (n + 31) / 32;
    return kernel_width(net->W) == 256 ? launch<256, 1>(a, a.n_wtiles, st) : launch<128, 1>(a, a.n_wtiles, st);
}

}
```

### nerf_pytorch_paeng_amd/csrc/occ.hip

```cpp
#include <hip/hip_runtime.h>
#include <math.h>
#include "../../include/mi_nerf_occ.h"
#include "abi_error.h"

namespace miocc {

ABI_ERROR_STATE(static, MI_OCC_EHIP)
ABI_NERF_FAIL(MI_OCC_EINVAL, MI_OCC_EHIP)
#define OCC_CHECK_ARG(cond, ...) ABI_CHECK_ARG(::miocc, MI_OCC_EINVAL, cond, __VA_ARGS__)
#define OCC_HIP(call) ABI_HIP(::miocc, call, #call)
#define OCC_LAUNCH_CHECK(name) ABI_LAUNCH_CHECK(::miocc, name)
#define OCC_NERF(call) ABI_NERF(::miocc, call, #call)

constexpr int TILE = MI_OCC_TILE;
static inline size_t align256(size_t v) { return (v + 255) & ~(size_t)255; }

struct GridDev {
    float lo[3], scale[3], fres[3];
    int res[3];
    int outside;
    long long cells;
};

static int resolve_grid(const mi_occ_grid* g, GridDev* out) {
// ... 146 lines not shown
}

__global__ __launch_bounds__(256) void cscan_reduce_kernel(const unsigned long long* __restrict__ data, long long n, unsigned long long* __restrict__ bsum) {
    __shared__ unsigned long long lds[4];
    const long long base = (long long)blockIdx.x * CSCAN_TILE + threadIdx.x * 4;
    unsigned long long s = 0;
#pragma unroll
    for (int k = 0; k < 4; ++k)
        if (base + k < n) s += data[base + k];
#pragma unroll
    for (int m = 32; m >= 1; m >>= 1) s += __shfl_xor(s, m, 64);
    if ((threadIdx.x & 63) == 0) lds[threadIdx.x >> 6] = s;
    __syncthreads();
    if (threadIdx.x == 0) bsum[blockIdx.x] = (lds[0] + lds[1]) + (lds[2] + lds[3]);
}

__global__ __launch_bounds__(1024) void cscan_sums_kernel(unsigned long long* __restrict__ bsum, int nb, unsigned* __restrict__ counts) {
    __shared__ unsigned long long lds[17];
    unsigned long long carry = 0;
    for (int c = 0; c < nb; c += 1024) {
        const int i = c + (int)threadIdx.x;
        const unsigned long long v = i < nb ? bsum[i] : 0ull;
        unsigned long long sum;
        const unsigned long long ex = cscan_block<1024>(v, &sum, lds);
        if (i < nb) bsum[i] = carry + ex;
        carry += sum;
    }
    if (threadIdx.x == 0) {
        counts[0] = (unsigned)(carry & 0xffffffffull);
        counts[1] = (unsigned)(carry >> 32);
    }
}

__global__ __launch_bounds__(256) void cscan_apply_kernel(unsigned long long* __restrict__ data, long long n, const unsigned long long* __restrict__ bsum) {
    __shared__ unsigned long long lds[5];
    const long long base = (long long)blockIdx.x * CSCAN_TILE + threadIdx.x * 4;
    unsigned long long v[4], s = 0;
#pragma unroll
    for (int k = 0; k < 4; ++k) {
        v[k] = base + k < n ? data[base + k] : 0ull;
        s += v[k];
    }
    unsigned long long sum;
    unsigned long long run = bsum[blockIdx.x] + cscan_block<256>(s, &sum, lds);
#pragma unroll
    for (int k = 0; k < 4; ++k) {
        if (base + k < n) data[base + k] = run;
        run += v[k];
    }
}

__global__ __launch_bounds__(256) void occ_compact_emit_kernel(GridDev G, const uint32_t* __restrict__ bits, const float* __restrict__ rays,
                                                               const float* __restrict__ z, long long n, int S,
                                                               const unsigned long long* __restrict__ first, float* __restrict__ tile_rays,
                                                               float* __restrict__ tile_z, int* __restrict__ tile_src, int* __restrict__ slot) {
    const int lane = threadIdx.x & 63;
    const long long ray = (long long)blockIdx.x * 4 + (threadIdx.x >> 6);
    if (ray >= n) return;
    const float* rp = rays + ray * 6;
    const float o[3] = {rp[0], rp[1], rp[2]}, d[3] = {rp[3], rp[4], rp[5]};
    const float* zr = z + ray * S;
    const long long base = (long long)(first[ray] & 0xffffffffull);
    const int j0 = (int)base * TILE;
    int run = 0;
    float last_z = 0.0f;
    for (int c = 0; c < S; c += 64) {
        const int s = c + lane;
        const float zv = s < S ? zr[s] : 0.0f;
        const bool occ = s < S && occ_lookup(G, bits, o, d, zv);
        const unsigned long long m = __ballot(occ);
        const int j = j0 + run + __popcll(m & ((1ull << lane) - 1ull));
        if (s < S) slot[ray * S + s] = occ ? j : -1;
        if (occ) {
            tile_z[j] = zv;
            tile_src[j] = (int)(ray * S + s);
        }
        run += __popcll(m);
        if (m) last_z = __shfl(zv, 63 - __clzll((long long)m), 64);
    }
    const int ntiles = (run + TILE - 1) / TILE;
    const int pad = ntiles * TILE - run;
    if (lane < pad) {
        tile_z[j0 + run + lane] = last_z;
        tile_src[j0 + run + lane] = -1;
    }
    for (int i = lane; i < ntiles * 6; i += 64) tile_rays[base * 6 + i] = rp[i % 6];
}

__global__ __launch_bounds__(256) void occ_gather_kernel(const int* __restrict__ tile_src, const float4* __restrict__ src, long long n_lanes,
                                                         float4* __restrict__ out) {
    const long long i = (long long)blockIdx.x * 256 + threadIdx.x;
    if (i >= n_lanes) return;
    const int j = tile_src[i];
    out[i] = j >= 0 ? src[j] : make_float4(0.0f, 0.0f, 0.0f, 0.0f);
}

struct BakeGeom {
    float lo[3], step[3];
    int rx, ry, rz, sub;
    int S;
    long long rows;
};

__global__ __launch_bounds__(256) void occ_bake_gen_kernel(BakeGeom B, long long row0, long long n_rows, float* __restrict__ rays, float* __restrict__ z) {
    const long long i = (long long)blockIdx.x * 256 + threadIdx.x;
    if (i >= n_rows * B.S) return;
    const long long r = i / B.S;
    const int jx = (int)(i - r * B.S);
    z[i] = ((float)jx + 0.5f) * B.step[0];
    if (jx == 0) {
        const long long row = row0 + r;
        const int ny = B.ry * B.sub;
        const int jz = (int)(row / ny), jy = (int)(row - (long long)jz * ny);
        float* rp = rays + r * 6;
        rp[0] = B.lo[0];
        rp[1] = B.lo[1] + ((float)jy + 0.5f) * B.step[1];
        rp[2] = B.lo[2] + ((float)jz + 0.5f) * B.step[2];
        rp[3] = 1.0f;
        rp[4] = 0.0f;
        rp[5] = 0.0f;
    }
}

__global__ __launch_bounds__(256) void occ_bake_reduce_kernel(BakeGeom B, long long row0, long long n_rows, const float* __restrict__ raw, float sigma_min,
                                                              uint32_t* __restrict__ bits) {
    const long long i = (long long)blockIdx.x * 256 + threadIdx.x;
    if (i >= n_rows * B.rx) return;
    const long long r = i / B.rx;
    const int ix = (int)(i - r * B.rx);
    const float* p = raw + (r * B.S + (long long)ix * B.sub) * 4 + 3;
    bool any = false;
    for (int a = 0; a < B.sub; ++a) any = any || p[a * 4] > sigma_min;
    if (!any) return;
    const long long row = row0 + r;
    const int ny = B.ry * B.sub;
    const int jz = (int)(row / ny), jy = (int)(row - (long long)jz * ny);
    const int b = ((jz / B.sub) * B.ry + jy / B.sub) * B.rx + ix;
    atomicOr(&bits[b >> 5], 1u << (b & 31));
}

__global__ __launch_bounds__(256) void occ_dilate_kernel(GridDev G, const uint32_t* __restrict__ in, uint32_t* __restrict__ out, int radius) {
    const long long cell = (long long)blockIdx.x * 256 + threadIdx.x;
    bool any = false;
    if (cell < G.cells) {
        const int rx = G.res[0], ry = G.res[1], rz = G.res[2];
        const int cx = (int)(cell % rx), cy = (int)((cell / rx) % ry), cz = (int)(cell / ((long long)rx * ry));
        for (int dz = -radius; dz <= radius; ++dz)
            for (int dy = -radius; dy <= radius; ++dy)
                for (int dx = -radius; dx <= radius; ++dx) {
                    const int x = cx + dx, y = cy + dy, zz = cz + dz;
                    if (x < 0 || x >= rx || y < 0 || y >= ry || zz < 0 || zz >= rz) continue;
                    const int b = (zz * ry + y) * rx + x;
                    any = any || ((in[b >> 5] >> (b & 31)) & 1u);
                }
    }
    const unsigned long long m = __ballot(any);
    const int lane = threadIdx.x & 63;
    const long long w0 = (cell - lane) >> 5;
    const long long words = (G.cells + 31) >> 5;
    if (lane == 0 && w0 < words) out[w0] = (uint32_t)m;
    if (lane == 32 && w0 + 1 < words) out[w0 + 1] = (uint32_t)(m >> 32);
}

__global__ __launch_bounds__(256) void occ_count_kernel(GridDev G, const uint32_t* __restrict__ bits, unsigned long long* __restrict__ count) {
    const long long words = (G.cells + 31) >> 5;
    unsigned long long c = 0;
    for (long long w = (long long)blockIdx.x * 256 + threadIdx.x; w < words; w += (long long)gridDim.x * 256) {
        uint32_t v = bits[w];
        const long long left = G.cells - w * 32;
        if (left < 32) v &= (1u << left) - 1u;
        c += __popc(v);
    }
#pragma unroll
    for (int m = 32; m >= 1; m >>= 1) c += __shfl_xor(c, m, 64);
    if ((threadIdx.x & 63) == 0 && c) atomicAdd(count, c);
}

static inline unsigned blocks_for(long long n, int per) { return (unsigned)((n + per - 1) / per); }

static int resolve_bake(const mi_occ_grid* grid, int sub, GridDev* G, BakeGeom* B) {
    if (int rc = resolve_grid(grid, G)) return rc;
    OCC_CHECK_ARG(sub >= 1 && sub <= MI_OCC_MAX_SUB, "sub=%d: 1..%d lattice points per cell and axis", sub, MI_OCC_MAX_SUB);
    for (int i = 0; i < 3; ++i) {
        B->lo[i] = grid->lo[i];
        B->step[i] = (grid->hi[i] - grid->lo[i]) / (float)(grid->res[i] * sub);
    }
    B->rx = grid->res[0]; B->ry = grid->res[1]; B->rz = grid->res[2]; B->sub = sub;
    B->S = B->rx * sub;
    B->rows = (long long)B->ry * sub * B->rz * sub;
    return MI_OCC_OK;
}

static inline size_t bake_slab_bytes(long long R, int S) {
    return align256((size_t)R * 24) + align256((size_t)R * S * 4) + align256((size_t)R * S * 16);
}
static inline long long bake_min_rows(const BakeGeom& B) {
    const long long want = ((1LL << 22) + B.S - 1) / B.S;
    return want < B.rows ? want : B.rows;
}

typedef int (*mlp_rays_fn)(const mi_nerf_net*, const void*, const float*, const float*, int64_t, int, float*, void*);
static int mlp_entry(int mode, mlp_rays_fn* fn) {
    switch (mode) {
        case MI_NERF_MODE_F32:  *fn = mi_nerf_mlp_rays; return MI_OCC_OK;
        case MI_NERF_MODE_F16S: *fn = mi_nerf_mlp_rays_f16s; return MI_OCC_OK;
        case MI_NERF_MODE_BF16: *fn = mi_nerf_mlp_rays_bf16; return MI_OCC_OK;
    }
    set_error("mode %d: the occupancy path runs MI_NERF_MODE_F32 (0), MI_NERF_MODE_BF16 (1) and MI_NERF_MODE_F16S (5)", mode);
    return MI_OCC_EINVAL;
}

static int bake(const mi_occ_grid* grid, uint32_t* bits, const mi_nerf_net* net, const void* packed, int mode, int sub, float sigma_min, int accumulate,
                void* scratch, size_t scratch_bytes, hipStream_t st) {
    GridDev G;
    BakeGeom B;
    if (int rc = resolve_bake(grid, sub, &G, &B)) return rc;
    mlp_rays_fn fn;
    if (int rc = mlp_entry(mode, &fn)) return rc;
    OCC_CHECK_ARG(bits && net && packed && scratch, "NULL pointer (bits, net, packed and scratch are required)");
    OCC_CHECK_ARG(!isnan(sigma_min), "sigma_min is NaN");
    OCC_CHECK_ARG(((uintptr_t)scratch & 255) == 0, "scratch must be 256-byte aligned");
    const size_t need = bake_slab_bytes(bake_min_rows(B), B.S);
    OCC_CHECK_ARG(scratch_bytes >= need, "scratch too small: %zu < %zu (mi_occ_bake_scratch_bytes)", scratch_bytes, need);
    long long R = (long long)((scratch_bytes - 768) / ((size_t)24 + (size_t)B.S * 20));
    if (R < bake_min_rows(B)) R = bake_min_rows(B);
    if (R > B.rows) R = B.rows;
    const long long r_cap = ((1LL << 31) - 1) / B.S;
    if (R > r_cap) R = r_cap;
    char* w = (char*)scratch;
    float* rays = (float*)w;
    float* z = (float*)(w + align256((size_t)R * 24));
    float* raw = (float*)(w + align256((size_t)R * 24) + align256((size_t)R * B.S * 4));
    if (!accumulate) OCC_HIP(hipMemsetAsync(bits, 0, grid_words(G) * 4, st));
    for (long long r0 = 0; r0 < B.rows; r0 += R) {
        const long long nr = B.rows - r0 < R ? B.rows - r0 : R;
        hipLaunchKernelGGL(occ_bake_gen_kernel, dim3(blocks_for(nr * B.S, 256)), dim3(256), 0, st, B, r0, nr, rays, z);
        OCC_LAUNCH_CHECK("occ_bake_gen_kernel");
        OCC_NERF(fn(net, packed, rays, z, nr, B.S, raw, (void*)st));
        hipLaunchKernelGGL(occ_bake_reduce_kernel, dim3(blocks_for(nr * B.rx, 256)), dim3(256), 0, st, B, r0, nr, raw, sigma_min, bits);
        OCC_LAUNCH_CHECK("occ_bake_reduce_kernel");
    }
    return MI_OCC_OK;
}

static int render_layout(const mi_nerf_render_cfg* cfg, int64_t n, mi_occ_workspace_layout* L) {
    OCC_CHECK_ARG(cfg && L, "NULL cfg/layout");
    OCC_CHECK_ARG(n >= 0 && cfg->Sc >= 1 && cfg->Nf >= 0, "bad sizes n=%lld Sc=%d Nf=%d", (long long)n, cfg->Sc, cfg->Nf);
    OCC_CHECK_ARG(cfg->Nf == 0 || cfg->Sc >= 3, "hierarchical sampling needs at least 3 coarse samples");
    OCC_CHECK_ARG((long long)cfg->Sc + cfg->Nf <= 1024, "Sc + Nf = %lld: at most 1024 samples per ray (mi_nerf_composite)", (long long)cfg->Sc + cfg->Nf);
    const size_t nn = (size_t)n, Sc = (size_t)cfg->Sc, Nf = (size_t)cfg->Nf, St = Sc + Nf;
    OCC_CHECK_ARG((long long)n * (long long)(St + 31) < (1LL << 31), "n_rays=%lld x %zu samples: n_rays * (Sc + Nf + 31) must stay below 2^31", (long long)n, St);
    const size_t T = nn * ((St + TILE - 1) / TILE);
    size_t off = 0;
    L->z_c = off;       off += align256(nn * Sc * 4);
    L->raw_c = off;     off += align256(nn * Sc * 16);
    L->weights_c = off; off += align256(nn * Sc * 4);
    L->z_f = off;       off += Nf > 0 ? align256(nn * St * 4) : 0;
    L->raw_f = off;     off += Nf > 0 ? align256(nn * St * 16) : 0;
    L->t_rand = off;    off += align256(nn * Sc * 4);
    L->u = off;         off += Nf > 0 ? align256(nn * Nf * 4) : 0;
    L->slot = off;      off += align256(nn * St * 4);
    L->tile_rays = off; off += align256(T * 6 * 4);
    L->tile_z = off;    off += align256(T * TILE * 4);
    L->tile_src = off;  off += align256(T * TILE * 4);
    L->tile_raw = off;  off += align256(T * TILE * 16);
    L->counters = off;  off += 256;
    L->total = off;
    return MI_OCC_OK;
}

struct Pass {
    float* tile_rays; float* tile_z; int* tile_src; float* tile_raw; int* slot; unsigned* counters;
};

static int network_pass(const GridDev& G, const uint32_t* bits, mlp_rays_fn fn, const mi_nerf_net* net, const void* packed, const float* rays, const float* z,
                        int64_t n, int S, const Pass& P, float* raw, int64_t* evaluated, int64_t* padded, hipStream_t st) {
    static thread_local unsigned* pinned = nullptr;
    if (!pinned) OCC_HIP(hipHostMalloc((void**)&pinned, 8, hipHostMallocPortable));
    OCC_HIP(hipMemsetAsync(P.counters, 0, 8, st));
    hipLaunchKernelGGL(occ_cull_kernel, dim3(blocks_for(n, 4)), dim3(256), 0, st, G, bits, rays, z, (long long)n, S, P.tile_rays, P.tile_z, P.tile_src, P.slot,
                       P.counters);
    OCC_LAUNCH_CHECK("occ_cull_kernel");
    OCC_HIP(hipMemcpyAsync(pinned, P.counters, 8, hipMemcpyDeviceToHost, st));
    OCC_HIP(hipStreamSynchronize(st));
    const int64_t tiles = pinned[0], survivors = pinned[1];
    *evaluated = survivors;
    *padded = tiles * TILE - survivors;
    if (tiles > 0) OCC_NERF(fn(net, packed, P.tile_rays, P.tile_z, tiles, TILE, P.tile_raw, (void*)st));
    hipLaunchKernelGGL(occ_scatter_kernel, dim3(blocks_for((long long)n * S, 256)), dim3(256), 0, st, P.slot, (const float4*)P.tile_raw, (long long)n * S,
                       (float4*)raw);
    OCC_LAUNCH_CHECK("occ_scatter_kernel");
    return MI_OCC_OK;
}

static int render(const mi_nerf_net* net, const void* packed_c, const void* packed_f, const mi_nerf_render_cfg* cfg, const mi_occ_grid* grid,
                  const uint32_t* bits_c, const uint32_t* bits_f, const float* rays, int64_t n, const float* t_rand, const float* u, void* ws, size_t ws_bytes,
                  float* rgb_c, float* disp_c, float* rgb_f, float* disp_f, mi_occ_stats* stats, hipStream_t st) {
    mi_occ_workspace_layout L;
    if (int rc = render_layout(cfg, n, &L)) return rc;
    GridDev G;
    if (int rc = resolve_grid(grid, &G)) return rc;
    mlp_rays_fn fn;
    if (int rc = mlp_entry(cfg->mode, &fn)) return rc;
    OCC_CHECK_ARG(cfg->reserved == 0, "mi_nerf_render_cfg.reserved must be 0");
    OCC_CHECK_ARG(net != nullptr, "net is NULL");
    OCC_CHECK_ARG(rays && rgb_c && disp_c && packed_c && bits_c && ws, "NULL pointer (rays, rgb_c, disp_c, packed_coarse, bits_coarse and workspace are required)");
    OCC_CHECK_ARG(cfg->Nf == 0 || (packed_f && bits_f && rgb_f && disp_f), "the fine pass needs packed_fine, bits_fine and its outputs");
    OCC_CHECK_ARG(ws_bytes >= L.total, "workspace too small: %zu < %zu", ws_bytes, L.total);
    OCC_CHECK_ARG(((uintptr_t)ws & 255) == 0, "workspace must be 256-byte aligned");
    if (stats) *stats = mi_occ_stats{0, 0, 0, 0, 0, 0};
    if (n == 0) return MI_OCC_OK;
    hipStreamCaptureStatus cap = hipStreamCaptureStatusNone;
    OCC_HIP(hipStreamIsCapturing(st, &cap));
    OCC_CHECK_ARG(cap == hipStreamCaptureStatusNone, "the stream is being captured: mi_occ_render_rays synchronises it once per network pass and cannot be recorded into a graph");
    char* w = (char*)ws;
    float* z_c = (float*)(w + L.z_c);
    float* raw_c = (float*)(w + L.raw_c);
    float* wts_c = (float*)(w + L.weights_c);
    const Pass P{(float*)(w + L.tile_rays), (float*)(w + L.tile_z), (int*)(w + L.tile_src), (float*)(w + L.tile_raw), (int*)(w + L.slot), (unsigned*)(w + L.counters)};
    const int Sc = cfg->Sc, St = cfg->Sc + cfg->Nf;
    mi_occ_stats s{0, 0, 0, 0, 0, 0};
    if (!t_rand) {
        float* tr = (float*)(w + L.t_rand);
        OCC_NERF(mi_nerf_fill_uniform(cfg->seed, 0, cfg->ray_offset, n, Sc, tr, (void*)st));
        t_rand = tr;
    }
    OCC_NERF(mi_nerf_stratified_z(n, Sc, cfg->near_, cfg->far_, t_rand, z_c, (void*)st));
    s.total_c = n * Sc;
    if (int rc = network_pass(G, bits_c, fn, net, packed_c, rays, z_c, n, Sc, P, raw_c, &s.evaluated_c, &s.padded_c, st)) return rc;
    OCC_NERF(mi_nerf_composite(raw_c, z_c, rays, 6, n, Sc, rgb_c, disp_c, nullptr, wts_c, nullptr, (void*)st));
    if (cfg->Nf > 0) {
        float* z_f = (float*)(w + L.z_f);
        float* raw_f = (float*)(w + L.raw_f);
        if (!cfg->det && !u) {
            float* ub = (float*)(w + L.u);
            OCC_NERF(mi_nerf_fill_uniform(cfg->seed, 1, cfg->ray_offset, n, cfg->Nf, ub, (void*)st));
            u = ub;
        }
        OCC_NERF(mi_nerf_fine_z(z_c, wts_c, n, Sc, cfg->Nf, cfg->det, cfg->det ? nullptr : u, z_f, nullptr, (void*)st));
        s.total_f = n * St;
        if (int rc = network_pass(G, bits_f, fn, net, packed_f, rays, z_f, n, St, P, raw_f, &s.evaluated_f, &s.padded_f, st)) return rc;
        OCC_NERF(mi_nerf_composite(raw_f, z_f, rays, 6, n, St, rgb_f, disp_f, nullptr, nullptr, nullptr, (void*)st));
    }
    if (stats) *stats = s;
    return MI_OCC_OK;
}

static inline size_t compact_scratch_bytes(int64_t n) {
    const size_t nb = ((size_t)n + CSCAN_TILE - 1) / CSCAN_TILE;
    return align256((size_t)n * 8) + align256(nb * 8) + 256;
}

static int check_tile_sizes(int64_t n, int S) {
    OCC_CHECK_ARG(n >= 0, "bad size n_rays=%lld", (long long)n);
    OCC_CHECK_ARG(S >= 1 && S <= 1024, "S=%d: 1..1024 samples per ray", S);
    OCC_CHECK_ARG((long long)n * ((S + TILE - 1) / TILE) * TILE < (1LL << 31), "n_rays=%lld x %d samples: n_rays * ceil(S / 32) * 32 must stay below 2^31",
                  (long long)n, S);
    return MI_OCC_OK;
}

static int compact(const mi_occ_grid* grid, const uint32_t* bits, const float* rays, const float* z, int64_t n, int S, float* tile_rays, float* tile_z,
                   int* tile_src, int* slot, unsigned* counts, void* scratch, size_t scratch_bytes, hipStream_t st) {
    GridDev G;
    if (int rc = resolve_grid(grid, &G)) return rc;
    if (int rc = check_tile_sizes(n, S)) return rc;
    OCC_CHECK_ARG(counts != nullptr, "counts is NULL");
    OCC_CHECK_ARG(((uintptr_t)counts & 3) == 0, "counts must be 4-byte aligned");
    if (n == 0) {
        OCC_HIP(hipMemsetAsync(counts, 0, 8, st));
        return MI_OCC_OK;
    }
    OCC_CHECK_ARG(bits && rays && z && tile_rays && tile_z && tile_src && slot && scratch,
                  "NULL pointer (bits, rays, z, tile_rays, tile_z, tile_src, slot, counts and scratch are required)");
    OCC_CHECK_ARG(((uintptr_t)scratch & 255) == 0, "scratch must be 256-byte aligned");
    const size_t need = compact_scratch_bytes(n);
    OCC_CHECK_ARG(scratch_bytes >= need, "scratch too small: %zu < %zu (mi_occ_compact_scratch_bytes)", scratch_bytes, need);
    unsigned long long* per_ray = (unsigned long long*)scratch;
    unsigned long long* sums = (unsigned long long*)((char*)scratch + align256((size_t)n * 8));
    const unsigned nb = blocks_for(n, CSCAN_TILE);
    hipLaunchKernelGGL(occ_compact_count_kernel, dim3(blocks_for(n, 4)), dim3(256), 0, st, G, bits, rays, z, (long long)n, S, per_ray);
    OCC_LAUNCH_CHECK("occ_compact_count_kernel");
    hipLaunchKernelGGL(cscan_reduce_kernel, dim3(nb), dim3(256), 0, st, per_ray, (long long)n, sums);
    OCC_LAUNCH_CHECK("cscan_reduce_kernel");
    hipLaunchKernelGGL(cscan_sums_kernel, dim3(1), dim3(1024), 0, st, sums, (int)nb, counts);
    OCC_LAUNCH_CHECK("cscan_sums_kernel");
    hipLaunchKernelGGL(cscan_apply_kernel, dim3(nb), dim3(256), 0, st, per_ray, (long long)n, sums);
    OCC_LAUNCH_CHECK("cscan_apply_kernel");
    hipLaunchKernelGGL(occ_compact_emit_kernel, dim3(blocks_for(n, 4)), dim3(256), 0, st, G, bits, rays, z, (long long)n, S, per_ray, tile_rays, tile_z, tile_src,
                       slot);
    OCC_LAUNCH_CHECK("occ_compact_emit_kernel");
    return MI_OCC_OK;
}

}

using namespace miocc;

extern "C" {

int mi_occ_abi_version(void) { return MI_OCC_ABI_VERSION; }
const char* mi_occ_last_error(void) { return g_err; }

size_t mi_occ_grid_words(const mi_occ_grid* grid) {
    GridDev G;
    return resolve_grid(grid, &G) == MI_OCC_OK ? grid_words(G) : 0;
}

size_t mi_occ_bake_scratch_bytes(const mi_occ_grid* grid, int sub) {
    GridDev G;
    BakeGeom B;
    if (resolve_bake(grid, sub, &G, &B) != MI_OCC_OK) return 0;
    return bake_slab_bytes(bake_min_rows(B), B.S);
}

int mi_occ_bake(const mi_occ_grid* grid, uint32_t* bits, const mi_nerf_net* net, const void* packed, int mode, int sub, float sigma_min, int accumulate,
                void* scratch, size_t scratch_bytes, void* stream) {
    return bake(grid, bits, net, packed, mode, sub, sigma_min, accumulate, scratch, scratch_bytes, (hipStream_t)stream);
}

int mi_occ_dilate(const mi_occ_grid* grid, const uint32_t* bits_in, uint32_t* bits_out, int radius, void* stream) {
    GridDev G;
    if (int rc = resolve_grid(grid, &G)) return rc;
    OCC_CHECK_ARG(radius >= 0 && radius <= MI_OCC_MAX_RADIUS, "radius=%d: 0..%d", radius, MI_OCC_MAX_RADIUS);
    OCC_CHECK_ARG(bits_in && bits_out, "NULL pointer");
    OCC_CHECK_ARG(bits_in != bits_out, "mi_occ_dilate works out of place: bits_out must not be bits_in");
    hipLaunchKernelGGL(occ_dilate_kernel, dim3(blocks_for(G.cells, 256)), dim3(256), 0, (hipStream_t)stream, G, bits_in, bits_out, radius);
    OCC_LAUNCH_CHECK("occ_dilate_kernel");
    return MI_OCC_OK;
}

int mi_occ_count(const mi_occ_grid* grid, const uint32_t* bits, uint64_t* count, void* stream) {
    GridDev G;
    if (int rc = resolve_grid(grid, &G)) return rc;
    OCC_CHECK_ARG(bits && count, "NULL pointer");
    OCC_CHECK_ARG(((uintptr_t)count & 7) == 0, "count must be 8-byte aligned");
    OCC_HIP(hipMemsetAsync(count, 0, 8, (hipStream_t)stream));
    const long long words = (long long)grid_words(G);
    const unsigned nb = blocks_for(words, 256) < 1024 ? blocks_for(words, 256) : 1024;
    hipLaunchKernelGGL(occ_count_kernel, dim3(nb), dim3(256), 0, (hipStream_t)stream, G, bits, (unsigned long long*)count);
    OCC_LAUNCH_CHECK("occ_count_kernel");
    return MI_OCC_OK;
}

int mi_occ_mark(const mi_occ_grid* grid, const uint32_t* bits, const float* rays, const float* z, int64_t n_rays, int S, uint8_t* mask, void* stream) {
    GridDev G;
    if (int rc = resolve_grid(grid, &G)) return rc;
    OCC_CHECK_ARG(n_rays >= 0 && S >= 1 && (long long)n_rays * S < (1LL << 38), "bad sizes n_rays=%lld S=%d", (long long)n_rays, S);
    if (n_rays == 0) return MI_OCC_OK;
    OCC_CHECK_ARG(bits && rays && z && mask, "NULL pointer");
    hipLaunchKernelGGL(occ_mark_kernel, dim3(blocks_for((long long)n_rays * S, 256)), dim3(256), 0, (hipStream_t)stream, G, bits, rays, z, (long long)n_rays * S, S,
                       mask);
    OCC_LAUNCH_CHECK("occ_mark_kernel");
    return MI_OCC_OK;
}

size_t mi_occ_compact_scratch_bytes(int64_t n_rays) {
    if (n_rays < 0 || n_rays >= (1LL << 26)) {
        set_error("n_rays=%lld: 0 .. 2^26 - 1 rays (n_rays * 32 tile lanes stay below 2^31)", (long long)n_rays);
        return 0;
    }
    return compact_scratch_bytes(n_rays);
}

int mi_occ_compact(const mi_occ_grid* grid, const uint32_t* bits, const float* rays, const float* z, int64_t n_rays, int S, float* tile_rays, float* tile_z,
                   int32_t* tile_src, int32_t* slot, uint32_t* counts, void* scratch, size_t scratch_bytes, void* stream) {
    return compact(grid, bits, rays, z, n_rays, S, tile_rays, tile_z, tile_src, slot, counts, scratch, scratch_bytes, (hipStream_t)stream);
}

int mi_occ_scatter_raw(const float* tile_vals, const int32_t* slot, int64_t n_rays, int S, float* out, void* stream) {
    if (int rc = check_tile_sizes(n_rays, S)) return rc;
    if (n_rays == 0) return MI_OCC_OK;
    OCC_CHECK_ARG(tile_vals && slot && out, "NULL pointer (tile_vals, slot and out are required)");
    OCC_CHECK_ARG((((uintptr_t)tile_vals | (uintptr_t)out) & 15) == 0, "tile_vals and out must be 16-byte aligned");
    const long long n_pts = (long long)n_rays * S;
    hipLaunchKernelGGL(occ_scatter_kernel, dim3(blocks_for(n_pts, 256)), dim3(256), 0, (hipStream_t)stream, slot, (const float4*)tile_vals, n_pts, (float4*)out);
    OCC_LAUNCH_CHECK("occ_scatter_kernel");
    return MI_OCC_OK;
}

int mi_occ_gather_raw(const float* src, const int32_t* tile_src, int64_t n_tiles, float* out, void* stream) {
    OCC_CHECK_ARG(n_tiles >= 0 && n_tiles * TILE < (1LL << 31), "n_tiles=%lld: n_tiles * 32 must stay below 2^31", (long long)n_tiles);
    if (n_tiles == 0) return MI_OCC_OK;
    OCC_CHECK_ARG(src && tile_src && out, "NULL pointer (src, tile_src and out are required)");
    OCC_CHECK_ARG((((uintptr_t)src | (uintptr_t)out) & 15) == 0, "src and out must be 16-byte aligned");
    const long long n_lanes = (long long)n_tiles * TILE;
    hipLaunchKernelGGL(occ_gather_kernel, dim3(blocks_for(n_lanes, 256)), dim3(256), 0, (hipStream_t)stream, tile_src, (const float4*)src, n_lanes, (float4*)out);
    OCC_LAUNCH_CHECK("occ_gather_kernel");
    return MI_OCC_OK;
}

size_t mi_occ_render_workspace_bytes(const mi_nerf_render_cfg* cfg, int64_t n_rays) {
    mi_occ_workspace_layout L;
    return render_layout(cfg, n_rays, &L) == MI_OCC_OK ? L.total : 0;
}

int mi_occ_render_workspace_layout(const mi_nerf_render_cfg* cfg, int64_t n_rays, mi_occ_workspace_layout* out) { return render_layout(cfg, n_rays, out); }

int mi_occ_render_rays(const mi_nerf_net* net, const void* packed_c, const void* packed_f, const mi_nerf_render_cfg* cfg, const mi_occ_grid* grid,
                       const uint32_t* bits_c, const uint32_t* bits_f, const float* rays, int64_t n_rays, const float* t_rand, const float* u, void* ws,
                       size_t ws_bytes, float* rgb_c, float* disp_c, float* rgb_f, float* disp_f, mi_occ_stats* stats, void* stream) {
    return render(net, packed_c, packed_f, cfg, grid, bits_c, bits_f, rays, n_rays, t_rand, u, ws, ws_bytes, rgb_c, disp_c, rgb_f, disp_f, stats,
                  (hipStream_t)stream);
}

}
```

### nerf_pytorch_paeng_amd/dist.py

```python
from __future__ import annotations

import ctypes as C
from typing import Callable, Dict, Optional, Sequence, Tuple

import torch
import torch.distributed as dist

from ._lib import MiNerfError, check, dev_ptr, lib, stream_ptr

COMM_ID_BYTES = 128


def shard_rows(H: int, world: int, rank: int) -> Tuple[int, int]:
    base, extra = divmod(H, world)
    n = base + (1 if rank < extra else 0)
    row0 = rank * base + min(rank, extra)
    return row0, n


def shard_range(n: int, world: int, rank: int) -> Tuple[int, int]:
    return shard_rows(n, world, rank)


class TileComm:

    def __init__(self, id_bytes: bytes, world: int, rank: int, device):
        self.device = torch.device(device)
        if self.device.type != "cuda":
            raise MiNerfError(f"TileComm lives on a HIP device, got {self.device}")
        if len(id_bytes) != COMM_ID_BYTES:
            raise MiNerfError(f"the unique id has {COMM_ID_BYTES} bytes, got {len(id_bytes)}")
        self.world, self.rank = int(world), int(rank)
        self._staging: Optional[torch.Tensor] = None
        handle = C.c_void_p()
        with torch.cuda.device(self.device):
            check(lib().mi_nerf_comm_init_rank(C.c_char_p(bytes(id_bytes)), self.world, self.rank, C.byref(handle)), "mi_nerf_comm_init_rank")
        self._handle = handle

    @staticmethod
    def available() -> None:
        check(lib().mi_nerf_rccl_available(), "mi_nerf_rccl_available")

    @staticmethod
    def unique_id() -> bytes:
        buf = C.create_string_buffer(COMM_ID_BYTES)
        check(lib().mi_nerf_comm_unique_id(buf), "mi_nerf_comm_unique_id")
        return buf.raw

    @classmethod
    def from_group(cls, device, group=None) -> "TileComm":
        device = torch.device(device)
        world, rank = dist.get_world_size(group), dist.get_rank(group)
        carrier = device if dist.get_backend(group) == "nccl" else torch.device("cpu")
        ident, why = bytes(COMM_ID_BYTES), None
        try:
            cls.available()
            if rank == 0:
                ident = cls.unique_id()
        except MiNerfError as e:
            why = e
        ok = torch.tensor([0 if why is not None else 1], dtype=torch.int32, device=carrier)
        dist.all_reduce(ok, op=dist.ReduceOp.MIN, group=group)
        if int(ok.item()) == 0:
            raise MiNerfError(f"TileComm.from_group: RCCL is not usable on every rank of the group (rank {rank}: {why if why is not None else 'ok here'})")
        t = torch.frombuffer(bytearray(ident), dtype=torch.uint8).to(carrier)
        dist.broadcast(t, src=dist.get_global_rank(group, 0) if group is not None else 0, group=group)
        return cls(bytes(t.cpu().numpy().tobytes()), world, rank, device)

    def all_gather_tiles(self, local: torch.Tensor, H: int, W: int, out: Optional[torch.Tensor] = None) -> torch.Tensor:
        if self._handle is None:
            raise MiNerfError("the communicator is closed")
        if local.dim() != 2 or local.shape[0] % W:
            raise MiNerfError(f"tile must be [rows_local * {W}, C], got {tuple(local.shape)}")
        Cc = int(local.shape[1])
        rows = local.shape[0] // W
        frame = torch.empty(H * W, Cc, dtype=torch.float32, device=local.device) if out is None else out
        if tuple(frame.shape) != (H * W, Cc) or frame.device != local.device:
            raise MiNerfError(f"out must be [{H * W}, {Cc}] on {local.device}, got {tuple(frame.shape)} on {frame.device}")
        need = int(lib().mi_nerf_all_gather_staging_bytes(self.world, H, W, Cc))
        if need and (self._staging is None or self._staging.numel() < need):
            self._staging = torch.empty(need, dtype=torch.uint8, device=local.device)
        with torch.cuda.device(local.device):
            check(lib().mi_nerf_all_gather_tiles(self._handle, dev_ptr(local, "tile"), rows, H, W, Cc, dev_ptr(frame, "frame"),
                                                 dev_ptr(self._staging, "staging", torch.uint8, 16) if need else None, need,
                                                 stream_ptr(local.device)), "mi_nerf_all_gather_tiles")
        return frame

    def close(self) -> None:
        if self._handle is not None:
            h, self._handle = self._handle, None
            with torch.cuda.device(self.device):
                check(lib().mi_nerf_comm_destroy(h), "mi_nerf_comm_destroy")


def unpad_tiles(staging: torch.Tensor, world: int, H: int, W: int, C_: int) -> torch.Tensor:
    frame = torch.empty(H * W, C_, dtype=torch.float32, device=staging.device)
    with torch.cuda.device(staging.device):
        check(lib().mi_nerf_unpad_tiles(dev_ptr(staging, "staging"), int(world), int(H), int(W), int(C_), dev_ptr(frame), stream_ptr(staging.device)),
              "mi_nerf_unpad_tiles")
    return frame


_tile_comms: Dict[Tuple[int, int], TileComm] = {}


def tile_comm(device, group=None) -> TileComm:
    device = torch.device(device)
    key = (id(group) if group is not None else 0, device.index if device.index is not None else torch.cuda.current_device())
    if key not in _tile_comms:
        _tile_comms[key] = TileComm.from_group(device, group)
    return _tile_comms[key]


def close_tile_comms() -> None:
    while _tile_comms:
        _tile_comms.popitem()[1].close()


def gather_tiles(local: torch.Tensor, H: int, W: int, group=None, force_collective: bool = False, via: str = "torch") -> torch.Tensor:
    if via not in ("torch", "c_abi"):
        raise ValueError(f"via must be 'torch' or 'c_abi', got {via!r}")
    if not (dist.is_available() and dist.is_initialized()) or (dist.get_world_size(group) == 1 and not force_collective):
        return local
    world, rank = dist.get_world_size(group), dist.get_rank(group)
    if via == "c_abi":
        if not local.is_cuda:
            raise MiNerfError(f"via='c_abi' gathers through the library's RCCL communicator and needs tiles on a HIP device (got {local.device}); there is no host fallback")
        _, n_rows = shard_rows(H, world, rank)
        if local.shape[0] != n_rows * W:
            raise ValueError(f"rank {rank}: tile has {local.shape[0]} rays, expected {n_rows * W}")
        return tile_comm(local.device, group).all_gather_tiles(local.contiguous(), H, W)
    C = local.shape[1]
    max_rows = (H + world - 1) // world
    _, n_rows = shard_rows(H, world, rank)
    if local.shape[0] != n_rows * W:
        raise ValueError(f"rank {rank}: tile has {local.shape[0]} rays, expected {n_rows * W}")
    padded = local
    if n_rows < max_rows:
        padded = torch.zeros(max_rows * W, C, dtype=local.dtype, device=local.device)
        padded[:n_rows * W] = local
    dev = local.device
    if dev.type == "cuda" and dist.get_backend(group) == "gloo":
        padded = padded.cpu()
    out = torch.empty(world * max_rows * W, C, dtype=local.dtype, device=padded.device)
    dist.all_gather_into_tensor(out, padded.contiguous(), group=group)
    out = out.to(dev)
    if H % world == 0:
        return out
    parts = []
    for r in range(world):
        _, nr = shard_rows(H, world, r)
        parts.append(out[r * max_rows * W:r * max_rows * W + nr * W])
    return torch.cat(parts, 0)


def assemble_tiles(tiles: Sequence[torch.Tensor], H: int, W: int) -> torch.Tensor:
    world = len(tiles)
    for r, t in enumerate(tiles):
        _, nr = shard_rows(H, world, r)
        if t.shape[0] != nr * W:
            raise ValueError(f"tile {r} of {world} has {t.shape[0]} rays, expected {nr * W}")
    return tiles[0] if world == 1 else torch.cat(list(tiles), 0)


def render_shard(H: int, W: int, K, pose, model, opts, world: int, rank: int, *, seed: int = 0, bf16: bool = False,
                 f16s: bool = False, coarse_f16s: bool = False) -> torch.Tensor:
    from . import nerf_process as NP
    from . import ops
    from .weights import packed_for
    packed = packed_for(model)
    r0, nr = shard_rows(H, world, rank)
    _, d = ops.make_o_d(W, H, K, pose, packed.device, row0=r0, n_rows=nr, want_origins=False)
    p = pose if isinstance(pose, torch.Tensor) else torch.as_tensor(pose)
    o = p[:3, -1].to(packed.device, torch.float32).expand(d.shape)
    rc, dc, rf, df = NP.batchify_rays_and_render_by_chunk(o, d, packed, None, H, W, K, opts, seed=seed, ray_offset=r0 * W, bf16=bf16, f16s=f16s,
                                                          coarse_f16s=coarse_f16s)
    rgb, disp = (rc, dc) if int(opts.N_samples_f) == 0 else (rf, df)
    return torch.cat([rgb, disp[:, None]], -1)


def render_frame(H: int, W: int, K, pose, model, opts, *, seed: int = 0, group=None, bf16: bool = False, f16s: bool = False,
                 render_rows_fn: Optional[Callable[[int, int], torch.Tensor]] = None, via: str = "torch",
                 force_collective: bool = False, coarse_f16s: bool = False) -> Tuple[torch.Tensor, torch.Tensor]:
    if dist.is_available() and dist.is_initialized():
        world, rank = dist.get_world_size(group), dist.get_rank(group)
    else:
        world, rank = 1, 0
    if render_rows_fn is None:
        local = render_shard(H, W, K, pose, model, opts, world, rank, seed=seed, bf16=bf16, f16s=f16s, coarse_f16s=coarse_f16s)
    else:
        local = render_rows_fn(*shard_rows(H, world, rank))
    full = gather_tiles(local, H, W, group, force_collective=force_collective, via=via)
    return full[:, :3].reshape(H, W, 3), full[:, 3].reshape(H, W)
```

### nerf_pytorch_paeng_amd/harness.py

```python
from __future__ import annotations

import os
import struct
import zlib
from typing import Dict, List, Optional, Sequence

import numpy as np
import torch

from . import nerf_process as NP
from . import ops
from ._lib import MiNerfError, as_f32_dev
from .rays import make_o_d


def write_png(path: str, img: np.ndarray) -> None:
    a = np.ascontiguousarray(img)
    if a.dtype != np.uint8:
        raise MiNerfError(f"write_png wants uint8, got {a.dtype}")
    if a.ndim == 3 and a.shape[2] == 1:
        a = a[:, :, 0]
    if a.ndim == 2:
        color, raw = 0, a
    elif a.ndim == 3 and a.shape[2] == 3:
        color, raw = 2, a.reshape(a.shape[0], -1)
    else:
        raise MiNerfError(f"write_png: unsupported shape {a.shape}")
    h, w = a.shape[0], a.shape[1]
    rows = np.concatenate([np.zeros((h, 1), np.uint8), raw], axis=1).tobytes()

    def chunk(tag: bytes, data: bytes) -> bytes:
        return struct.pack(">I", len(data)) + tag + data + struct.pack(">I", zlib.crc32(tag + data) & 0xFFFFFFFF)

    with open(path, "wb") as f:
        f.write(b"\x89PNG\r\n\x1a\n" + chunk(b"IHDR", struct.pack(">IIBBBBB", w, h, 8, color, 0, 0, 0))
                + chunk(b"IDAT", zlib.compress(rows, 6)) + chunk(b"IEND", b""))


def load_checkpoint(path: str, model: Optional[torch.nn.Module] = None, *, allow_pickle: bool = False) -> Dict:
    ck = torch.load(path, map_location="cpu", weights_only=not allow_pickle)
    if "model_state_dict" not in ck:
        raise MiNerfError(f"{path}: no 'model_state_dict' (keys: {sorted(ck)[:8]})")
    if model is not None:
        model.load_state_dict(ck["model_state_dict"])
    return ck


def _ckpt_path(log_dir: str, exp_name: str, idx) -> str:
    return os.path.join(log_dir, exp_name, f"{exp_name}_{idx}.pth.tar")


def spherical_poses(theta_deg, phi_deg: float, radius: float) -> np.ndarray:
    th = np.atleast_1d(np.asarray(theta_deg, dtype=np.float64)) / 180.0 * np.pi
    ph = float(phi_deg) / 180.0 * np.pi
    ct, st = np.cos(th).astype(np.float32), np.sin(th).astype(np.float32)
    cp, sp, r = np.float32(np.cos(ph)), np.float32(np.sin(ph)), np.float32(radius)
    zero, one = np.zeros_like(ct), np.ones_like(ct)
    fwd = np.stack([st * cp, ct * cp, -sp * one], -1)
    rows = np.stack([np.stack([-ct, st * sp, fwd[:, 0], fwd[:, 0] * r], -1),
                     np.stack([st, ct * sp, fwd[:, 1], fwd[:, 1] * r], -1),
                     np.stack([zero, cp * one, fwd[:, 2], fwd[:, 2] * r], -1),
                     np.stack([zero, zero, zero, one], -1)], 1)
    return rows.astype(np.float32)


def pose_spherical(theta: float, phi: float, radius: float) -> torch.Tensor:
    return torch.from_numpy(spherical_poses([theta], phi, radius)[0])


def get_render_pose(n_angle: int = 1, single_angle: float = -1, phi: float = -30.0, nf: float = 4.0, device=None) -> torch.Tensor:
    circle = n_angle != 1 and single_angle == -1
    azimuths = np.linspace(-180, 180, n_angle + 1)[:-1] if circle else [single_angle]
    poses = torch.from_numpy(spherical_poses(azimuths, phi, nf))
    return poses.to(device) if device is not None else poses


def _unit(v: np.ndarray) -> np.ndarray:
    if v.ndim == 1:
        return v / np.linalg.norm(v)
    return v / np.sqrt(np.square(v).sum(-1, keepdims=True))


def look_frames(back: np.ndarray, up: np.ndarray, eye: np.ndarray) -> np.ndarray:
    z = _unit(np.asarray(back))
    x = _unit(np.cross(np.broadcast_to(up, z.shape), z))
    y = _unit(np.cross(z, x))
    return np.stack([x, y, z, np.broadcast_to(eye, z.shape)], -1)


def rig_average(poses: np.ndarray) -> np.ndarray:
    frame = look_frames(_unit(poses[:, :3, 2].sum(0)), poses[:, :3, 1].sum(0), poses[:, :3, 3].mean(0))
    return np.concatenate([frame, poses[0, :3, -1:]], 1)


def spiral_path(c2w: np.ndarray, up: np.ndarray, radii, focus: float, zrate: float, rots: float, n: int) -> np.ndarray:
    t = np.linspace(0.0, 2.0 * np.pi * rots, int(n) + 1)[:-1]
    frame = c2w[:3, :4]
    local = np.stack([np.cos(t), -np.sin(t), -np.sin(t * zrate), np.ones_like(t)], -1) * np.append(np.asarray(radii, dtype=np.float64), 1.0)
    eyes = (local[:, None, :] * frame[None]).sum(-1)
    target = (frame * np.array([0.0, 0.0, -focus, 1.0])).sum(-1)
    cams = look_frames(eyes - target, up, eyes)
    return np.concatenate([cams, np.broadcast_to(c2w[:, 4:5], (len(t), 3, 1))], -1)


def recenter_rig(poses: np.ndarray) -> np.ndarray:
    last_row = np.array([0.0, 0.0, 0.0, 1.0])
    world_from_avg = np.vstack([rig_average(poses)[:3, :4], last_row])
    homog = np.concatenate([poses[:, :3, :4], np.broadcast_to(last_row, (poses.shape[0], 1, 4))], 1)
    out = poses + 0
    out[:, :3, :4] = (np.linalg.inv(world_from_avg) @ homog)[:, :3, :4]
    return out


def llff_render_poses(poses, bds, path_zflat: bool = False, n_views: int = 120, n_rots: int = 2) -> np.ndarray:
    centre = rig_average(poses)
    up = _unit(poses[:, :3, 1].sum(0))
    nearest, farthest = bds.min() * .9, bds.max() * 5.
    focus = 1. / (.25 / nearest + .75 / farthest)
    radii = np.percentile(np.abs(poses[:, :3, 3]), 90, 0)
    if path_zflat:
        centre[:3, 3] = centre[:3, 3] - nearest * .1 * centre[:3, 2]
        radii[2] = 0.
        n_rots, n_views = 1, n_views // 2
    return spiral_path(centre, up, radii, focus, zrate=.5, rots=n_rots, n=n_views).astype(np.float32)


def llff_cameras(raw_poses, raw_bds, bd_factor=.75, path_zflat: bool = False) -> Dict:
    poses = np.moveaxis(np.concatenate([raw_poses[:, 1:2, :], -raw_poses[:, 0:1, :], raw_poses[:, 2:, :]], 1), -1, 0).astype(np.float32)
    bds = np.moveaxis(raw_bds, -1, 0).astype(np.float32)
    scale = 1. if bd_factor is None else 1. / (bds.min() * bd_factor)
    poses[:, :3, 3] *= scale
    bds *= scale
    poses = recenter_rig(poses)
    render_poses = llff_render_poses(poses, bds, path_zflat)
    poses = poses.astype(np.float32)
    H, W, focal = poses[0, :3, -1]
    H, W = int(H), int(W)
    K = np.array([[focal, 0, 0.5 * W], [0, focal, 0.5 * H], [0, 0, 1]])
    return {"poses": poses, "bds": bds, "render_poses": render_poses, "gt_extrinsic": poses[:, :3, :4], "gt_intrinsic": K, "hw": [H, W]}


_PRECISIONS = {"fp32": (), "f16s": ("f16s",), "bf16": ("bf16",), "f16s+bf16": ("bf16", "coarse_f16s"), "f16": ("f16",), "f16+bf16": ("bf16", "coarse_f16")}


def _precision(opts) -> Dict[str, bool]:
    mode = str(getattr(opts, "precision", "fp32")).lower()
    if mode not in _PRECISIONS:
        raise ValueError(f"opts.precision must be one of {', '.join(repr(k) for k in _PRECISIONS)}, got {mode!r}")
    return {k: k in _PRECISIONS[mode] for k in ops.PRECISION_FLAGS}


def _frozen(model, opts):
    from .weights import packed_for
    packed = packed_for(model)
    if ops.precision(**_precision(opts)).reads_f16s:
        packed.f16s()
        packed.check_f16s_range()
    return packed


def _render_pose(model, posenc, K, pose, hw, opts):
    img_h, img_w = hw
    rays_o, rays_d = make_o_d(img_w, img_h, K, pose[:3, :4])
    rgb_c, disp_c, rgb_f, disp_f = NP.batchify_rays_and_render_by_chunk(rays_o, rays_d, model, posenc, img_h, img_w, K, opts, **_precision(opts),
                                                                        occupancy=getattr(opts, "occupancy", None))
    return (rgb_c, disp_c) if int(opts.N_samples_f) == 0 else (rgb_f, disp_f)


def test(idx, i_test, posenc, model, test_imgs, gt_intrinsic, gt_extrinsic, hw, opts, *, log_dir: Optional[str] = None,
         save_dir: Optional[str] = None, keep_frames: bool = False, ssim: bool = False) -> Dict:
    want_ssim = bool(ssim) or bool(getattr(opts, "ssim", False))
    if isinstance(model, torch.nn.Module):
        model.eval()
        if log_dir is not None:
            load_checkpoint(_ckpt_path(log_dir, opts.exp_name, idx), model)
    if save_dir is not None:
        os.makedirs(save_dir, exist_ok=True)
    img_h, img_w = hw
    dev = next(model.parameters()).device if isinstance(model, torch.nn.Module) else model.device
    n_pose = len(gt_extrinsic)
    want_frames = save_dir is not None or keep_frames
    metrics = torch.empty(n_pose, 3 if want_ssim else 2, dtype=torch.float32, device=dev)
    rgbs8 = torch.empty(n_pose, img_h, img_w, 3, dtype=torch.uint8, device=dev) if want_frames else None
    disps8 = torch.empty(n_pose, img_h, img_w, 1, dtype=torch.uint8, device=dev) if want_frames else None
    with torch.no_grad():
        frozen = _frozen(model, opts)
        for i, pose in enumerate(gt_extrinsic):
            pose = as_f32_dev(pose, dev)
            pred_rgb, pred_disp = _render_pose(frozen, posenc, gt_intrinsic, pose, hw, opts)
            target = as_f32_dev(test_imgs[i], pred_rgb.device).reshape(-1, 3)
            metrics[i, :2] = ops.image_metrics(pred_rgb, target)
            if want_ssim:
                metrics[i, 2:] = ops.ssim(pred_rgb.reshape(-1, 3), target, hw=(img_h, img_w))
            if want_frames:
                rgbs8[i] = ops.to8b(pred_rgb).reshape(img_h, img_w, 3)
                disps8[i] = ops.to8b(pred_disp, ops.nanmax(pred_disp)).reshape(img_h, img_w, 1)
    m_host = metrics.cpu().numpy()
    losses: List[float] = [float(v) for v in m_host[:, 0]]
    psnrs: List[float] = [float(v) for v in m_host[:, 1]]
    frames = []
    if want_frames:
        rgbs_np, disps_np = rgbs8.cpu().numpy(), disps8.cpu().numpy()
        for i in range(n_pose):
            if save_dir is not None:
                write_png(os.path.join(save_dir, f"{i:03d}.png"), rgbs_np[i])
                write_png(os.path.join(save_dir, f"{i:03d}_disp.png"), disps_np[i])
            if keep_frames:
                frames.append((rgbs_np[i], disps_np[i]))
    ssims: Optional[List[float]] = [float(v) for v in m_host[:, 2]] if want_ssim else None
    best = int(np.argmax(psnrs)) if psnrs else -1
    res = {"loss": losses, "psnr": psnrs, "ssim": ssims, "lpips": None, "best_idx": best,
           "best_psnr": psnrs[best] if psnrs else None, "mean_psnr": float(np.mean(psnrs)) if psnrs else None}
    if want_ssim:
        res["best_ssim"] = max(ssims) if ssims else None
        res["mean_ssim"] = float(np.mean(ssims)) if ssims else None
    if keep_frames:
        res["frames"] = frames
    if save_dir is not None:
        with open(os.path.join(save_dir, "_result.txt"), "w") as f:
            for i in range(len(losses)):
                f.write(f"idx:{i}\tloss:{losses[i]}\tpsnr:{psnrs[i]}\tssim:{ssims[i] if want_ssim else 'n/a'}\tlpips:n/a\n")
            f.write(f"\nBest Value ) PSNR : {res['best_psnr']}\tSSIM : {res['best_ssim'] if want_ssim else 'n/a'}\tLPIPS : n/a\n")
            f.write(f"Mean Value ) PSNR : {res['mean_psnr']}\tSSIM : {res['mean_ssim'] if want_ssim else 'n/a'}\tLPIPS : n/a")
    return res


def render(idx, posenc, model, gt_intrinsic, render_pose, hw, opts, *, log_dir: Optional[str] = None, save_dir: Optional[str] = None):
    dev = next(model.parameters()).device if isinstance(model, torch.nn.Module) else model.device
    if getattr(opts, "data_type", None) in ("blender", "custom"):
        render_pose = get_render_pose(n_angle=opts.n_angle, single_angle=opts.single_angle, phi=opts.phi, nf=opts.nf)
    elif render_pose is None:
        raise MiNerfError("render(): llff data needs the loader's render poses (harness.llff_render_poses); got None")
    poses = torch.as_tensor(np.asarray(render_pose) if not isinstance(render_pose, torch.Tensor) else render_pose, dtype=torch.float32).to(dev)
    if isinstance(model, torch.nn.Module):
        model.eval()
        if log_dir is not None:
            load_checkpoint(_ckpt_path(log_dir, opts.exp_name, idx), model)
    if save_dir is not None:
        os.makedirs(save_dir, exist_ok=True)
    img_h, img_w = hw
    n = poses.shape[0]
    rgbs = torch.empty(n, img_h, img_w, 3, dtype=torch.uint8, device=dev)
    disps = torch.empty(n, img_h, img_w, dtype=torch.uint8, device=dev)
    with torch.no_grad():
        frozen = _frozen(model, opts)
        for i in range(n):
            rgb, disp = _render_pose(frozen, posenc, gt_intrinsic, poses[i], hw, opts)
            rgbs[i] = ops.to8b(rgb).reshape(img_h, img_w, 3)
            disps[i] = ops.to8b(disp, ops.nanmax(disp)).reshape(img_h, img_w)
    rgbs_np, disps_np = rgbs.cpu().numpy(), disps.cpu().numpy()
    if save_dir is not None:
        for i in range(n):
            write_png(os.path.join(save_dir, f"{i}_rgb.png"), rgbs_np[i])
            write_png(os.path.join(save_dir, f"{i}_disp.png"), disps_np[i])
    return rgbs_np, disps_np


class ShuffledRows:

    def __init__(self, table: torch.Tensor, perm: torch.Tensor):
        self.table, self.perm = table, perm

    @property
    def shape(self):
        return self.table.shape

    @property
    def device(self):
        return self.table.device

    def __len__(self) -> int:
        return int(self.table.shape[0])

    def __getitem__(self, key) -> torch.Tensor:
        if not isinstance(key, slice):
            raise MiNerfError("a shuffled global batch is read in slices of consecutive rows (train.py:29); materialize() gives the whole array")
        return ops.gather_rows(self.table, self.perm[key].contiguous())

    def materialize(self) -> torch.Tensor:
        return ops.permute_rows(self.table, self.perm)


class GetterRayBatchIdx:

    def __init__(self, rays_rgb: torch.Tensor, generator: Optional[torch.Generator] = None, shuffle: bool = False):
        self.table = rays_rgb
        self.perm: Optional[torch.Tensor] = None
        self.epoch = 0
        self.i_batch = 0
        self._gen = generator
        if shuffle:
            self._draw()

    def _draw(self) -> None:
        self.perm = torch.randperm(self.table.shape[0], device=self.table.device, generator=self._gen)

    @property
    def rays_rgb(self):
        return self.table if self.perm is None else ShuffledRows(self.table, self.perm)

    def shuffle_ray_idx(self, batch_size: int) -> None:
        self._draw()
        self.i_batch = batch_size
        self.epoch += 1

    def __call__(self, batch_size: int):
        self.i_batch += batch_size
        if self.i_batch >= self.table.shape[0]:
            self.shuffle_ray_idx(batch_size)
        return self.i_batch, self.rays_rgb, self.epoch


def global_batch(images, gt_intrinsic, gt_extrinsic, i_train: Sequence[int], hw, device, generator: Optional[torch.Generator] = None,
                 shuffle: bool = True) -> GetterRayBatchIdx:
    img_h, img_w = hw
    idx = torch.as_tensor(np.asarray(list(i_train)), dtype=torch.long)
    imgs = torch.as_tensor(np.asarray(images) if not isinstance(images, torch.Tensor) else images)
    poses = torch.as_tensor(np.asarray(gt_extrinsic) if not isinstance(gt_extrinsic, torch.Tensor) else gt_extrinsic)
    imgs = imgs[idx.to(imgs.device)].to(device=device, dtype=torch.float32).contiguous()
    poses = poses[idx.to(poses.device)][:, :3, :4].to(device=device, dtype=torch.float32).contiguous()
    rr = ops.rays_rgb(img_w, img_h, gt_intrinsic, poses, imgs)
    return GetterRayBatchIdx(rr, generator, shuffle=shuffle)


def sample_rays_and_pixel(i, img_w, img_h, K, pose, target_img, opts, generator: Optional[torch.Generator] = None, *, pose_grad: bool = False):
    target_img = as_f32_dev(target_img)
    dev = target_img.device
    if i < int(getattr(opts, "precrop_iters", 0)):
        dH = int(img_h // 2 * opts.precrop_frac)
        dW = int(img_w // 2 * opts.precrop_frac)
        ys = torch.arange(img_h // 2 - dH, img_h // 2 + dH, device=dev)
        xs = torch.arange(img_w // 2 - dW, img_w // 2 + dW, device=dev)
    else:
        ys = torch.arange(img_h, device=dev)
        xs = torch.arange(img_w, device=dev)
    n_coords = ys.numel() * xs.numel()
    n = int(opts.N_rays)
    if n > n_coords:
        raise MiNerfError(f"cannot draw {n} pixels without replacement from {n_coords}")
    sel = torch.randperm(n_coords, device=dev, generator=generator)[:n]
    py, px = ys[sel // xs.numel()], xs[sel % xs.numel()]
    pix = (py * img_w + px).contiguous()
    if pose_grad:
        from . import pose as pose_mod
        rays_o, rays_d = pose_mod.make_o_d(int(img_w), int(img_h), K, pose, pixels=pix)
    else:
        rays_o, rays_d = ops.make_o_d_pixels(int(img_w), int(img_h), K, pose, pix)
    target = target_img.reshape(-1, 3)[pix]
    return rays_o, rays_d, target


def train(idx, i_train, images, gt_cam_param, hw, model, criterion, posenc, optimizer, global_batch_idx, vis, opts, *,
          log_dir: Optional[str] = None, generator: Optional[torch.Generator] = None) -> Dict:
    from . import geometry as geo
    geom = geo.parse_options(getattr(opts, "geometry", None), float(opts.near), float(opts.far))
    refiner = getattr(opts, "pose_refine", None)
    if refiner is not None:
        from .pose import CameraRefiner
        if not isinstance(refiner, CameraRefiner):
            raise MiNerfError(f"opts.pose_refine must be a pose.CameraRefiner, got {type(refiner).__name__}")
        if global_batch_idx is not None and getattr(opts, "global_batch", True):
            raise MiNerfError("opts.pose_refine needs the per-image branch: the global batch holds rays precomputed from fixed poses "
                              "(pass global_batch_idx=None or opts.global_batch=False)")
    model.train()
    img_h, img_w = hw
    gt_intrinsic, gt_extrinsic = gt_cam_param
    dev = next(model.parameters()).device
    if global_batch_idx is not None and getattr(opts, "global_batch", True):
        i_batch, rays_rgb, _ = global_batch_idx(int(opts.N_rays))
        batch = rays_rgb[i_batch - int(opts.N_rays):i_batch]
        rays_o, rays_d, target_img = batch[:, 0], batch[:, 1], batch[:, 2]
    else:
        i_img = int(np.random.choice(i_train))
        target_full = as_f32_dev(torch.as_tensor(images[i_img]), dev)
        pose = torch.as_tensor(np.asarray(gt_extrinsic[i_img]) if not isinstance(gt_extrinsic, torch.Tensor) else gt_extrinsic[i_img])
        if refiner is not None:
            rays_o, rays_d, target_img = sample_rays_and_pixel(idx, img_w, img_h, gt_intrinsic, refiner(i_img, pose[:3, :4]), target_full, opts,
                                                               generator, pose_grad=True)
        else:
            rays_o, rays_d, target_img = sample_rays_and_pixel(idx, img_w, img_h, gt_intrinsic, pose[:3, :4], target_full, opts, generator)
    train_grid = getattr(opts, "train_occupancy", None)
    rebake = int(getattr(opts, "occupancy_rebake_every", 0) or 0)
    if train_grid is not None and rebake > 0 and idx % rebake == 0:
        with torch.no_grad():
            train_grid.bake(model, **getattr(opts, "occupancy_bake_args", {}))
    rgb_c, _, rgb_f, _, *extras = NP.batchify_rays_and_render_by_chunk(rays_o.contiguous(), rays_d.contiguous(), model, posenc, img_h, img_w,
                                                                       gt_intrinsic, opts, **_precision(opts), train_occupancy=train_grid,
                                                                       **({} if geom is None else {"geometry": True}),
                                                                       **({} if refiner is None else {"ray_grad": True}))
    optimizer.zero_grad()
    target_img = target_img.contiguous()
    loss = criterion(rgb_c, target_img)
    out = {"loss_c": loss.detach(), "psnr_c": -10.0 * torch.log10(loss.detach())}
    if int(opts.N_samples_f) > 0:
        loss_f = criterion(rgb_f, target_img)
        out.update(loss_f=loss_f.detach(), psnr_f=-10.0 * torch.log10(loss_f.detach()))
        loss = loss + loss_f
    if geom is not None:
        acc_t = depth_t = None
        if geom["targets"] is not None:
            with torch.no_grad():
                acc_t, depth_t = geom["targets"](torch.cat([rays_o, rays_d], -1).detach().contiguous())
        for key in ("c", "f") if int(opts.N_samples_f) > 0 else ("c",):
            for name, term in geo.loss_terms(geom, extras[0], key, acc_t, depth_t).items():
                loss = loss + geom[name + "_weight"] * term
                out["loss_" + name] = out.get("loss_" + name, 0.0) + term.detach()
    out["loss"] = loss.detach()
    loss.backward()
    optimizer.step()
    if _precision(opts)["f16s"] and idx % int(getattr(opts, "idx_print", 0) or 100) == 0:
        from . import train_path
        out["f16s"] = train_path.f16s_status(model, reset=False)
    if log_dir is not None and idx % int(getattr(opts, "idx_save", 0) or (1 << 62)) == 0 and idx > 0:
        save_path = os.path.join(log_dir, opts.exp_name)
        os.makedirs(save_path, exist_ok=True)
        torch.save({"idx": idx, "model_state_dict": model.state_dict(), "optimizer_state_dict": optimizer.state_dict()},
                   _ckpt_path(log_dir, opts.exp_name, idx))
    return out
```

### nerf_pytorch_paeng_amd/nerf_process.py

```python
from __future__ import annotations

from typing import Dict, Optional

import torch

from . import ops
from ._lib import MiNerfError, as_f32_dev
from .weights import PackedNeRF, packed_for
from . import train_path
from . import occupancy as occ
from . import occupancy_train
from . import geometry as geo

MAX_RAYS_PER_LAUNCH = 1 << 20

_rng = {"seed": 0, "calls": 0}


def manual_seed(seed: int) -> None:
    _rng["seed"], _rng["calls"] = int(seed), 0


def _next_seed(seed: Optional[int]) -> int:
    if seed is not None:
        return int(seed)
    s = (_rng["seed"] * 0x9E3779B1 + _rng["calls"]) & 0xFFFFFFFF
    _rng["calls"] += 1
    return s


def _det(opts) -> bool:
    p = getattr(opts, "perturb", 1.0)
    return isinstance(p, (int, float)) and p == 0.0


def ndc_rays(H, W, focal, near, rays_o, rays_d):
    lead = rays_d.shape[:-1]
    d = as_f32_dev(rays_d).reshape(-1, 3)
    o = rays_o.to(torch.float32) if rays_o.dtype != torch.float32 else rays_o
    o = o.expand(rays_d.shape).reshape(-1, 3) if o.shape != rays_d.shape else o.reshape(-1, 3)
    if isinstance(focal, torch.Tensor):
        focal = float(focal.item())
    oo, dd = ops.ndc_rays(int(H), int(W), float(focal), float(near), o, d)
    return oo.reshape(*lead, 3), dd.reshape(*lead, 3)


def sample_pdf(bins, weights, N_samples, det=False, opts=None, *, u=None):
    assert opts is not None
    bins, weights = as_f32_dev(bins), as_f32_dev(weights, bins.device)
    lead = bins.shape[:-1]
    b2, w2 = bins.reshape(-1, bins.shape[-1]), weights.reshape(-1, weights.shape[-1])
    if not det:
        u = (ops.fill_uniform(_next_seed(None), 1, 0, b2.shape[0], int(N_samples), bins.device) if u is None
             else as_f32_dev(u, bins.device).reshape(-1, int(N_samples)))
    out = ops.sample_pdf(b2, w2, int(N_samples), bool(det), u)
    return out.reshape(*lead, int(N_samples))


def pre_process(rays, posenc, opts, z_vals=None, weights=None, isFine=False, *, t_rand=None, u=None):
    rays = as_f32_dev(rays)
    n = rays.shape[0]
    L_x, L_d = int(getattr(posenc[0], "L", 10)), int(getattr(posenc[1], "L", 4))
    if not isFine:
        if t_rand is None:
            t_rand = ops.fill_uniform(_next_seed(None), 0, 0, n, int(opts.N_samples_c), rays.device)
        z = ops.stratified_z(float(opts.near), float(opts.far), as_f32_dev(t_rand, rays.device))
    else:
        det = _det(opts)
        if not det and u is None:
            u = ops.fill_uniform(_next_seed(None), 1, 0, n, int(opts.N_samples_f), rays.device)
        z = ops.fine_z(as_f32_dev(z_vals, rays.device), as_f32_dev(weights, rays.device), int(opts.N_samples_f), det,
                       None if det else as_f32_dev(u, rays.device))
    embedded = ops.embed(rays, z, L_x, L_d)
    return embedded, z, rays[:, 3:]


class _Composite(torch.autograd.Function):

    @staticmethod
    def forward(ctx, raw, z, d, weights_grad=False):
        rgb, disp, acc, wts, depth = ops.composite(raw, z, d, want_all=True)
        ctx.save_for_backward(raw, z, d)
        ctx.mark_non_differentiable(*((disp,) if weights_grad else (disp, wts)))
        ctx.set_materialize_grads(False)
        return rgb, disp, acc, wts, depth

    @staticmethod
    def backward(ctx, g_rgb, g_disp, g_acc, g_wts, g_depth):
        if g_rgb is None and g_acc is None and g_wts is None and g_depth is None:
            return None, None, None, None
        raw, z, d = ctx.saved_tensors
        if g_acc is None and g_wts is None and g_depth is None:
            return ops.composite_backward(raw, z, d, g_rgb.contiguous().float()), None, None, None
        g_rgb, g_acc, g_wts, g_depth = (None if g is None else g.contiguous().float() for g in (g_rgb, g_acc, g_wts, g_depth))
        return geo.composite_geo_backward(raw, z, d, 0.0, 1.0, g_rgb, g_acc, g_depth, None, g_wts), None, None, None


def post_process(outputs, z_vals, rays_d, *, weights_grad: bool = False):
    z = as_f32_dev(z_vals)
    raw = as_f32_dev(outputs, z.device)
    d = as_f32_dev(rays_d, z.device)
    if torch.is_grad_enabled() and raw.requires_grad:
        return _Composite.apply(raw, z.detach(), d.detach(), bool(weights_grad))
    return ops.composite(raw, z, d, want_all=True)


raw2outputs = post_process


def run_network(model, embedded, is_fine: bool = False):
    if train_path.wants_grad(model):
        return model(embedded, is_fine)
    packed = packed_for(model)
    return ops.mlp_embedded(packed.net, packed.blob(is_fine), as_f32_dev(embedded, packed.device))


def _render(rays: torch.Tensor, packed: PackedNeRF, opts, t_rand, u, seed: int, ray_offset: int, prec: ops.Precision,
            intermediates: bool, occupancy=None, geometry: bool = False) -> Dict[str, torch.Tensor]:
    n = rays.shape[0]
    dev = rays.device
    Sc, Nf = int(opts.N_samples_c), int(opts.N_samples_f)
    det = _det(opts)
    cfg = ops.render_cfg(float(opts.near), float(opts.far), Sc, Nf, det, seed=seed, ray_offset=ray_offset)
    cfg.mode = prec.mode
    if t_rand is not None:
        t_rand = as_f32_dev(t_rand, dev)
    elif intermediates:
        t_rand = ops.fill_uniform(seed, 0, ray_offset, n, Sc, dev)
    if Nf > 0 and not det:
        if u is not None:
            u = as_f32_dev(u, dev)
        elif intermediates:
            u = ops.fill_uniform(seed, 1, ray_offset, n, Nf, dev)
    else:
        u = None
    net, blob_c, blob_f = packed.kernel_blobs(prec)
    stats = None
    if occupancy is None:
        rgb_c, disp_c, rgb_f, disp_f, ws = ops.render_rays(net, blob_c, blob_f if Nf > 0 else None, cfg, rays, t_rand, u)
        views = ops.workspace_views
    else:
        rgb_c, disp_c, rgb_f, disp_f, ws, stats = occ.render_rays(net, blob_c, blob_f if Nf > 0 else None, cfg, occupancy, rays, t_rand, u)
        occupancy.last_stats = occ.add_stats(occupancy.last_stats, stats)
        views = occ.workspace_views
    out = {"rgb_c": rgb_c, "disp_c": disp_c}
    if Nf > 0:
        out["rgb_f"], out["disp_f"] = rgb_f, disp_f
    if geometry:
        v = views(cfg, n, ws)
        for key in ("c", "f") if Nf > 0 else ("c",):
            extra = geo.composite_geo(v["raw_" + key], v["z_" + key], rays, float(opts.near), float(opts.far))
            out.update({name + "_" + key: t for name, t in zip(geo.EXTRA_KEYS, (extra[2], extra[4], extra[5]))})
    if intermediates:
        for k, v in views(cfg, n, ws).items():
            out["_" + k] = v
        out["_t_rand"], out["_u"] = t_rand, u
        if stats is not None:
            out["_occ_stats"] = stats
    return out


def _occupancy_arg(occupancy, training: bool, prec: ops.Precision):
    if occupancy is None:
        return None
    if training:
        raise MiNerfError("occupancy= is an inference feature (call under torch.no_grad(), or freeze the model); to train with a grid pass it as "
                          "train_occupancy=")
    if not isinstance(occupancy, occ.OccupancyGrid):
        raise MiNerfError(f"occupancy must be an occupancy.OccupancyGrid, got {type(occupancy).__name__}")
    occ.check_precision(prec)
    occupancy.last_stats = None
    return occupancy


def _train_occupancy_arg(grid, training: bool, prec: ops.Precision):
    if grid is None:
        return None
    if not isinstance(grid, occ.OccupancyGrid):
        raise MiNerfError(f"train_occupancy must be an occupancy.OccupancyGrid, got {type(grid).__name__}")
    if not training:
        raise MiNerfError("train_occupancy= is a training feature: gradients are disabled or no parameter of the model requires them "
                          "(under torch.no_grad() render with occupancy=)")
    if prec.coarse != prec.fine or prec.fine not in ("fp32", "f16s"):
        raise MiNerfError(f"training with a grid runs fp32 or f16s for both networks (got coarse {prec.coarse}, fine {prec.fine})")
    grid.last_stats = None
    return grid


def _train_f16s(prec: ops.Precision, intermediates: bool = False) -> bool:
    if prec.fine not in ("fp32", "f16s") or intermediates:
        raise MiNerfError("the training path has no bf16 / f16 mode (fp32, or f16s=True: split-precision forward, fp32 backward) and returns no intermediates")
    return prec.fine == "f16s"


def _geometry_kw(geometry, ray_grad=False) -> Dict[str, bool]:
    return {**({"geometry": True} if geometry else {}), **({"ray_grad": True} if ray_grad else {})}


def _ray_grad_arg(ray_grad, train_occupancy) -> bool:
    if ray_grad and train_occupancy is not None:
        raise MiNerfError("ray_grad=True with train_occupancy= is not built: the occupancy-training node differentiates the parameters only")
    return bool(ray_grad)


def render_rays(rays, model, posenc, opts, *, t_rand=None, u=None, seed=None, ray_offset: int = 0, bf16: bool = False,
                return_intermediates: bool = False, f16s: bool = False, coarse_f16s: bool = False, f16: bool = False, coarse_f16: bool = False,
                occupancy=None, train_occupancy=None, geometry: bool = False, ray_grad: bool = False):
    prec = ops.precision(bf16, f16s, coarse_f16s, f16, coarse_f16)
    ray_grad = _ray_grad_arg(ray_grad, train_occupancy)
    training = train_path.wants_grad(model) or train_path.wants_ray_grad(model, ray_grad, rays)
    occupancy = _occupancy_arg(occupancy, training, prec)
    train_occupancy = _train_occupancy_arg(train_occupancy, training, prec)
    if training:
        train_f16s = _train_f16s(prec, return_intermediates)
        if rays.dim() != 2 or rays.shape[1] != 6:
            raise MiNerfError(f"rays must be [n, 6] (o, d), got {tuple(rays.shape)}")
        if train_occupancy is not None:
            return occupancy_train.render_train(rays, model, opts, train_occupancy, t_rand=t_rand, u=u, seed=_next_seed(seed),
                                                ray_offset=int(ray_offset), f16s=train_f16s, **_geometry_kw(geometry))
        return train_path.render_train(rays, model, opts, t_rand=t_rand, u=u, seed=_next_seed(seed), ray_offset=int(ray_offset), f16s=train_f16s,
                                       **_geometry_kw(geometry, ray_grad))
    packed = packed_for(model)
    rays = as_f32_dev(rays, packed.device)
    if rays.dim() != 2 or rays.shape[1] != 6:
        raise MiNerfError(f"rays must be [n, 6] (o, d), got {tuple(rays.shape)}")
    if occupancy is not None and rays.shape[0] > occ.MAX_RAYS_PER_LAUNCH:
        raise MiNerfError(f"render_rays with a grid takes at most {occ.MAX_RAYS_PER_LAUNCH} rays per call (batchify_rays_and_render_by_chunk slabs them)")
    return _render(rays, packed, opts, t_rand, u, _next_seed(seed), int(ray_offset), prec, return_intermediates, occupancy, **_geometry_kw(geometry))


def batchify_rays_and_render_by_chunk(ray_o, ray_d, model, posenc, H, W, K, opts, *, t_rand=None, u=None, seed=None,
                                      ray_offset: int = 0, bf16: bool = False, f16s: bool = False, coarse_f16s: bool = False, f16: bool = False,
                                      coarse_f16: bool = False, occupancy=None, train_occupancy=None, geometry: bool = False,
                                      ray_grad: bool = False):
    prec = ops.precision(bf16, f16s, coarse_f16s, f16, coarse_f16)
    ray_grad = _ray_grad_arg(ray_grad, train_occupancy)
    training = train_path.wants_grad(model) or train_path.wants_ray_grad(model, ray_grad, ray_o, ray_d)
    occupancy = _occupancy_arg(occupancy, training, prec)
    train_occupancy = _train_occupancy_arg(train_occupancy, training, prec)
    train_f16s = _train_f16s(prec) if training else False
    packed = None if training else packed_for(model)
    dev = next(model.parameters()).device if training else packed.device
    ray_d = as_f32_dev(ray_d, dev)
    flat_d = ray_d.reshape(-1, 3)
    ray_o = ray_o.to(dev) if ray_o.device != dev else ray_o
    flat_o = ray_o.to(torch.float32).expand(ray_d.shape).reshape(-1, 3)
    if getattr(opts, "data_type", None) == "llff":
        k00 = K[0][0]
        focal = float(k00.item()) if isinstance(k00, torch.Tensor) else float(k00)
        if ray_grad:
            from . import pose
            flat_o, flat_d = pose.ndc_rays(H, W, focal, 1.0, flat_o, flat_d)
        else:
            flat_o, flat_d = ndc_rays(H, W, focal, 1.0, flat_o, flat_d)
    rays = torch.cat((flat_o, flat_d), dim=-1)
    N = rays.shape[0]
    seed = _next_seed(seed)
    Nf = int(opts.N_samples_f)
    parts = []
    train_stats = None
    slab = train_path.MAX_TRAIN_RAYS if training else (MAX_RAYS_PER_LAUNCH if occupancy is None else occ.MAX_RAYS_PER_LAUNCH)
    for i in range(0, N, slab):
        j = min(N, i + slab)
        tr, uu = (None if t_rand is None else t_rand[i:j]), (None if u is None else u[i:j])
        if train_occupancy is not None:
            parts.append(occupancy_train.render_train(rays[i:j].contiguous(), model, opts, train_occupancy, t_rand=tr, u=uu, seed=seed,
                                                      ray_offset=int(ray_offset) + i, f16s=train_f16s, **_geometry_kw(geometry)))
            train_stats = occ.add_stats(train_stats, train_occupancy.last_stats)
        elif training:
            parts.append(train_path.render_train(rays[i:j].contiguous(), model, opts, t_rand=tr, u=uu, seed=seed,
                                                 ray_offset=int(ray_offset) + i, f16s=train_f16s, **_geometry_kw(geometry, ray_grad)))
        else:
            parts.append(_render(rays[i:j], packed, opts, tr, uu, seed, int(ray_offset) + i, prec, False, occupancy, **_geometry_kw(geometry)))
    if train_occupancy is not None:
        train_occupancy.last_stats = train_stats
    def cat(key):
        return parts[0][key] if len(parts) == 1 else torch.cat([p[key] for p in parts], dim=0)
    res = (cat("rgb_c"), cat("disp_c"), cat("rgb_f"), cat("disp_f")) if Nf > 0 else (cat("rgb_c"), cat("disp_c"), None, None)
    if geometry:
        return (*res, {name + "_" + key: cat(name + "_" + key) for key in (("c", "f") if Nf > 0 else ("c",)) for name in geo.EXTRA_KEYS})
    return res
```

### nerf_pytorch_paeng_amd/ops.py

```python
from __future__ import annotations

import ctypes as C
from typing import Dict, NamedTuple, Optional, Sequence, Tuple

import numpy as np
import torch

from . import _lib as L
from ._lib import MiNerfError, Net, RenderCfg, TrainLayout, WorkspaceLayout, check, dev_ptr, lib, stream_ptr


def _guard(device):
    device = torch.device(device)
    if device.type != "cuda":
        raise MiNerfError(f"tensors must live on a HIP device (got {device}); this path has no CPU fallback")
    return torch.cuda.device(device)


def make_net(D: int, W: int, skip: int = 4, L_x: int = 10, L_d: int = 4) -> Net:
    return Net(D, W, skip, L_x, L_d)


def pack_module(sd: Dict[str, "np.ndarray | torch.Tensor"], prefix: str, net: Net, bf16: bool = False, backward: bool = False,
                f16s: bool = False) -> torch.Tensor:
# ... 247 lines not shown
def train_layout(net: Net, n_rays: int, S: int) -> TrainLayout:
    lay = TrainLayout()
    check(lib().mi_nerf_train_layout_query(C.byref(net), int(n_rays), int(S), C.byref(lay)), "mi_nerf_train_layout_query")
    return lay


def pack_map(net: Net, backward: bool = False) -> torch.Tensor:
    nbytes = (lib().mi_nerf_packed_bytes_bwd if backward else lib().mi_nerf_packed_bytes)(C.byref(net))
    if nbytes == 0:
        check(1, "mi_nerf_packed_bytes")
    m = torch.empty(nbytes // 4, dtype=torch.int32)
    check(lib().mi_nerf_pack_map(C.byref(net), int(backward), m.data_ptr(), m.numel()), "mi_nerf_pack_map")
    return m


def pack_apply(map_dev: torch.Tensor, flat: torch.Tensor, out: Optional[torch.Tensor] = None) -> torch.Tensor:
    dev = flat.device
    nbytes = map_dev.numel() * 4
    if out is None:
        out = torch.empty(nbytes, dtype=torch.uint8, device=dev)
    if out.numel() != nbytes:
        raise MiNerfError(f"blob must have {nbytes} bytes, got {out.numel()}")
    with _guard(dev):
        check(lib().mi_nerf_pack_apply(dev_ptr(map_dev, "map", torch.int32), dev_ptr(flat, "flat"), nbytes, dev_ptr(out, "blob", torch.uint8, 16),
                                       stream_ptr(dev)), "mi_nerf_pack_apply")
    return out


def pack_map_bf16(net: Net) -> torch.Tensor:
    n = lib().mi_nerf_pack_map_bf16_len(C.byref(net))
    if n == 0:
        check(1, "mi_nerf_pack_map_bf16_len")
    m = torch.empty(n, dtype=torch.int32)
    check(lib().mi_nerf_pack_map_bf16(C.byref(net), m.data_ptr(), m.numel()), "mi_nerf_pack_map_bf16")
    return m


def pack_apply_bf16(net: Net, map_dev: torch.Tensor, flat: torch.Tensor) -> torch.Tensor:
    dev = flat.device
    nbytes = lib().mi_nerf_packed_bytes_bf16(C.byref(net))
    out = torch.empty(nbytes, dtype=torch.uint8, device=dev)
    with _guard(dev):
        check(lib().mi_nerf_pack_apply_bf16(C.byref(net), dev_ptr(map_dev, "map", torch.int32), dev_ptr(flat, "flat"), dev_ptr(out, "blob", torch.uint8, 16),
                                            nbytes, stream_ptr(dev)), "mi_nerf_pack_apply_bf16")
    return out


def pack_map_f16s(net: Net, backward: bool = False) -> torch.Tensor:
    n = (lib().mi_nerf_pack_map_bwd_f16s_len if backward else lib().mi_nerf_pack_map_f16s_len)(C.byref(net))
    if n == 0:
        check(1, "mi_nerf_pack_map_f16s_len")
    m = torch.empty(n, dtype=torch.int32)
    check((lib().mi_nerf_pack_map_bwd_f16s if backward else lib().mi_nerf_pack_map_f16s)(C.byref(net), m.data_ptr(), m.numel()), "mi_nerf_pack_map_f16s")
    return m


def pack_apply_f16s(net: Net, map_dev: torch.Tensor, flat: torch.Tensor, out_of_range: Optional[torch.Tensor] = None, backward: bool = False) -> torch.Tensor:
    dev = flat.device
    nbytes = (lib().mi_nerf_packed_bytes_bwd_f16s if backward else lib().mi_nerf_packed_bytes_f16s)(C.byref(net))
    if nbytes == 0:
        check(1, "mi_nerf_packed_bytes_f16s")
    out = torch.empty(nbytes, dtype=torch.uint8, device=dev)
    fn = lib().mi_nerf_pack_apply_bwd_f16s if backward else lib().mi_nerf_pack_apply_f16s
    with _guard(dev):
        check(fn(C.byref(net), dev_ptr(map_dev, "map", torch.int32), dev_ptr(flat, "flat"), dev_ptr(out, "blob", torch.uint8, 16),
                 nbytes, None if out_of_range is None else dev_ptr(out_of_range, "out_of_range", torch.int32), stream_ptr(dev)),
              "mi_nerf_pack_apply_f16s")
    return out


def mlp_rays_train(net: Net, packed: torch.Tensor, rays: torch.Tensor, z: torch.Tensor, stash: Optional[torch.Tensor] = None, f16s: bool = False):
    n, S = z.shape
    if tuple(rays.shape) != (n, 6):
        raise MiNerfError(f"rays must be [n,6], got {tuple(rays.shape)}")
    lay = train_layout(net, n, S)
    if stash is None:
        stash = torch.empty(lay.stash_bytes, dtype=torch.uint8, device=z.device)
    raw = torch.empty(n, S, 4, dtype=torch.float32, device=z.device)
    with _guard(z.device):
        fn = lib().mi_nerf_mlp_rays_train_f16s if f16s else lib().mi_nerf_mlp_rays_train
        check(fn(C.byref(net), dev_ptr(packed, "packed", torch.uint8, 16), dev_ptr(rays, "rays"), dev_ptr(z, "z"), n, S,
                 dev_ptr(raw, "raw", align=16), dev_ptr(stash, "stash", torch.uint8, 16), stash.numel(),
                 stream_ptr(z.device)), "mi_nerf_mlp_rays_train_f16s" if f16s else "mi_nerf_mlp_rays_train")
    return raw, stash


def mlp_backward(net: Net, packed: torch.Tensor, packed_bwd: torch.Tensor, rays: torch.Tensor, z: torch.Tensor, d_raw: torch.Tensor,
                 stash: torch.Tensor, work: Optional[torch.Tensor] = None, stage: int = 0, grads: Optional[torch.Tensor] = None,
                 f16s_wgrad: bool = False, f16s_dgrad: bool = False):
    n, S = z.shape
    if tuple(d_raw.shape) != (n, S, 4) or tuple(rays.shape) != (n, 6):
        raise MiNerfError(f"d_raw must be {(n, S, 4)} and rays {(n, 6)}, got {tuple(d_raw.shape)} / {tuple(rays.shape)}")
    lay = train_layout(net, n, S)
    dev = z.device
    if work is None:
        work = torch.empty(lay.work_bytes, dtype=torch.uint8, device=dev)
    if grads is None:
        grads = torch.empty(param_count(net), dtype=torch.float32, device=dev)
    elif grads.numel() != param_count(net):
        raise MiNerfError(f"grads must have {param_count(net)} elements, got {grads.numel()}")
    with _guard(dev):
        check(lib().mi_nerf_mlp_backward_mode(C.byref(net), dev_ptr(packed, "packed", torch.uint8, 16), dev_ptr(packed_bwd, "packed_bwd", torch.uint8, 16),
                                              dev_ptr(rays, "rays"), dev_ptr(z, "z"), n, S, dev_ptr(d_raw, "d_raw", align=16),
                                              dev_ptr(stash, "stash", torch.uint8, 16), dev_ptr(work, "work", torch.uint8, 16), work.numel(),
                                              dev_ptr(grads, "grads"), int(stage), (1 if f16s_wgrad else 0) | (2 if f16s_dgrad else 0), stream_ptr(dev)), "mi_nerf_mlp_backward_mode")
    return (None if stage == 1 else grads), work


def mlp_embedded_train(net: Net, packed: torch.Tensor, x: torch.Tensor):
    n = x.shape[0]
    if x.dim() != 2 or x.shape[1] != 6 + 6 * net.L_x + 6 * net.L_d:
        raise MiNerfError(f"x must be [n, {6 + 6 * net.L_x + 6 * net.L_d}], got {tuple(x.shape)}")
    lay = train_layout(net, (n + 31) // 32, 32)
    stash = torch.empty(lay.stash_bytes, dtype=torch.uint8, device=x.device)
    out = torch.empty(n, 4, dtype=torch.float32, device=x.device)
    with _guard(x.device):
        check(lib().mi_nerf_mlp_embedded_train(C.byref(net), dev_ptr(packed, "packed", torch.uint8, 16), dev_ptr(x, "x"), n, dev_ptr(out, "out", align=16),
                                               dev_ptr(stash, "stash", torch.uint8, 16), stash.numel(), stream_ptr(x.device)), "mi_nerf_mlp_embedded_train")
    return out, stash


def mlp_embedded_backward(net: Net, packed: torch.Tensor, packed_bwd: torch.Tensor, x: torch.Tensor, d_out: torch.Tensor, stash: torch.Tensor,
                          grads: Optional[torch.Tensor] = None) -> torch.Tensor:
    n = x.shape[0]
    if tuple(d_out.shape) != (n, 4):
        raise MiNerfError(f"d_out must be {(n, 4)}, got {tuple(d_out.shape)}")
    lay = train_layout(net, (n + 31) // 32, 32)
    dev = x.device
    work = torch.empty(lay.work_bytes, dtype=torch.uint8, device=dev)
    if grads is None:
        grads = torch.empty(param_count(net), dtype=torch.float32, device=dev)
    with _guard(dev):
        check(lib().mi_nerf_mlp_embedded_backward(C.byref(net), dev_ptr(packed, "packed", torch.uint8, 16), dev_ptr(packed_bwd, "packed_bwd", torch.uint8, 16),
                                                  dev_ptr(x, "x"), n, dev_ptr(d_out, "d_out", align=16), dev_ptr(stash, "stash", torch.uint8, 16),
                                                  dev_ptr(work, "work", torch.uint8, 16), work.numel(), dev_ptr(grads, "grads"), stream_ptr(dev)),
              "mi_nerf_mlp_embedded_backward")
    return grads


def wgrad_product(delta: torch.Tensor, M: int, x: torch.Tensor, N: int, P: int, want_bias: bool = True, iters: int = 1, timed: bool = False):
    outs, biases, ms = wgrad_products([delta], [x], P, [int(M)], [int(N)], want_bias, iters, timed)
    return outs[0], (biases[0] if want_bias else None), ms


def wgrad_products(deltas: Sequence[torch.Tensor], xs: Sequence[torch.Tensor], P: int, Ms: Optional[Sequence[int]] = None,
                   Ns: Optional[Sequence[int]] = None, want_bias: bool = True, iters: int = 1, timed: bool = False, f16s: bool = False):
    n = len(deltas)
    if n == 0 or len(xs) != n:
        raise MiNerfError("deltas / xs must be non-empty lists of equal length")
    dev = deltas[0].device
    Ms = [d.shape[1] for d in deltas] if Ms is None else list(Ms)
    Ns = [x.shape[1] for x in xs] if Ns is None else list(Ns)
    for d, x, M, N in zip(deltas, xs, Ms, Ns):
        if d.dim() != 2 or x.dim() != 2 or d.shape[0] < P or x.shape[0] < P or d.shape[1] < M or x.shape[1] < N:
            raise MiNerfError(f"operands {tuple(d.shape)} / {tuple(x.shape)} too small for P={P}, M={M}, N={N}")
    outs = [torch.empty(M, N, dtype=torch.float32, device=dev) for M, N in zip(Ms, Ns)]
    biases = [torch.empty(M, dtype=torch.float32, device=dev) for M in Ms] if want_bias else None
    scratch = torch.empty(int(lib().mi_nerf_wgrad_scratch_bytes()), dtype=torch.uint8, device=dev)
    PP, II = C.c_void_p * n, C.c_int * n
    ms = C.c_float(0.0)
    with _guard(dev):
        check((lib().mi_nerf_wgrad_products_f16s if f16s else lib().mi_nerf_wgrad_products)(n, PP(*[dev_ptr(d, "delta") for d in deltas]), II(*[d.stride(0) for d in deltas]), II(*Ms),
                                           PP(*[dev_ptr(x, "x") for x in xs]), II(*[x.stride(0) for x in xs]), II(*Ns), int(P),
                                           PP(*[dev_ptr(o) for o in outs]), II(*Ns), PP(*[dev_ptr(b) for b in biases]) if want_bias else None,
                                           dev_ptr(scratch, "scratch", torch.uint8, 16), scratch.numel(), int(iters),
                                           C.byref(ms) if timed else None, stream_ptr(dev)), "mi_nerf_wgrad_products")
    return outs, biases, (float(ms.value) if timed else None)


def backward_range(net: Net, n_rays: int, S: int, work: torch.Tensor):
    lay = train_layout(net, n_rays, S)
    words = work[lay.work_bytes - 256:lay.work_bytes - 248].view(torch.float32).cpu()
    return float(words[0]), float(words[1])


def backward_range_words(net: Net, n_rays: int, S: int, work: torch.Tensor) -> torch.Tensor:
    lay = train_layout(net, n_rays, S)
    return work[lay.work_bytes - 256:lay.work_bytes - 248].view(torch.float32)


def train_views(net: Net, n_rays: int, S: int, stash: Optional[torch.Tensor] = None, work: Optional[torch.Tensor] = None):
    lay = train_layout(net, n_rays, S)
    n_pts = n_rays * S
    W, D = net.W, net.D
    out = {}
    def view(buf, off, shape):
        cnt = int(np.prod(shape))
        return buf[off:off + 4 * cnt].view(torch.float32).reshape(shape)
    if stash is not None:
        out["stash_h"] = view(stash, lay.stash_h, (D, n_pts, W))
        out["stash_f"] = view(stash, lay.stash_f, (n_pts, W))
        out["stash_g"] = view(stash, lay.stash_g, (n_pts, W // 2))
    if work is not None:
        out["delta_h"] = view(work, lay.delta_h, (D, n_pts, W))
        out["delta_f"] = view(work, lay.delta_f, (n_pts, W))
        out["delta_d"] = view(work, lay.delta_d, (n_pts, W // 2))
    return out


REDUCE_SCRATCH_BYTES = 8192


def image_metrics(pred: torch.Tensor, target: torch.Tensor) -> torch.Tensor:
    if pred.shape != target.shape or pred.numel() == 0:
        raise MiNerfError(f"pred {tuple(pred.shape)} and target {tuple(target.shape)} must match and be non-empty")
    dev = pred.device
    out = torch.empty(2, dtype=torch.float32, device=dev)
    scratch = torch.empty(REDUCE_SCRATCH_BYTES, dtype=torch.uint8, device=dev)
    with _guard(dev):
        check(lib().mi_nerf_image_metrics(dev_ptr(pred, "pred"), dev_ptr(target, "target"), pred.numel(), dev_ptr(out),
                                          dev_ptr(scratch, "scratch", torch.uint8), scratch.numel(), stream_ptr(dev)), "mi_nerf_image_metrics")
    return out


def ssim(pred: torch.Tensor, target: torch.Tensor, *, hw=None, downsample: int = 1, clamp_cs: bool = False, return_map: bool = False):
    from . import _iqa
    if pred.shape != target.shape or pred.numel() == 0:
        raise MiNerfError(f"pred {tuple(pred.shape)} and target {tuple(target.shape)} must match and be non-empty")
    shape = tuple(pred.shape)
    if len(shape) == 2 and shape[1] == 3 and hw is not None and int(hw[0]) * int(hw[1]) == shape[0]:
        n, H, W = 1, int(hw[0]), int(hw[1])
    elif len(shape) == 3 and shape[2] == 3 and hw is None:
        n, H, W = 1, shape[0], shape[1]
    elif len(shape) == 4 and shape[3] == 3 and hw is None:
        n, H, W = shape[0], shape[1], shape[2]
    else:
        raise MiNerfError(f"ssim takes [H,W,3], [H*W,3] with hw=(H,W), or [N,H,W,3]; got {shape} with hw={hw}")
    dev = pred.device
    with _guard(dev):
        L = _iqa.lib()
        ds = int(downsample)
        nbytes = L.mi_iqa_ssim_scratch_bytes(n, H, W, ds)
        f = L.mi_iqa_ssim_downsample_factor(H, W, ds)
        if nbytes == 0 or f == 0:
            raise MiNerfError(f"mi_iqa_ssim refused: {_iqa.last_error()}")
        out = torch.empty(n, dtype=torch.float32, device=dev)
        smap = torch.empty(n, H // f - 10, W // f - 10, 3, dtype=torch.float32, device=dev) if return_map else None
        scratch = torch.empty(nbytes // 8, dtype=torch.float64, device=dev)
        _iqa.check(L.mi_iqa_ssim(dev_ptr(pred, "pred"), dev_ptr(target, "target"), n, H, W, ds, _iqa.SSIM_CLAMP_CS if clamp_cs else 0,
                                 dev_ptr(out), dev_ptr(smap, "map"), dev_ptr(scratch, "scratch", torch.float64, 8), nbytes, stream_ptr(dev)),
                   "mi_iqa_ssim")
    return (out, smap) if return_map else out


def nanmax(x: torch.Tensor) -> torch.Tensor:
    if x.numel() == 0:
        raise MiNerfError("nanmax of an empty tensor")
    dev = x.device
    out = torch.empty(1, dtype=torch.float32, device=dev)
    scratch = torch.empty(REDUCE_SCRATCH_BYTES, dtype=torch.uint8, device=dev)
    with _guard(dev):
        check(lib().mi_nerf_nanmax(dev_ptr(x, "x"), x.numel(), dev_ptr(out), dev_ptr(scratch, "scratch", torch.uint8), scratch.numel(),
                                   stream_ptr(dev)), "mi_nerf_nanmax")
    return out


def to8b(x: torch.Tensor, divisor: Optional[torch.Tensor] = None) -> torch.Tensor:
    dev = x.device
    out = torch.empty(x.shape, dtype=torch.uint8, device=dev)
    with _guard(dev):
        check(lib().mi_nerf_to8b(dev_ptr(x, "x"), x.numel(), dev_ptr(divisor, "divisor"), dev_ptr(out, "out", torch.uint8, 1), stream_ptr(dev)),
              "mi_nerf_to8b")
    return out


def rays_rgb(W: int, H: int, K, poses: torch.Tensor, images: torch.Tensor) -> torch.Tensor:
    n_img = poses.shape[0]
    if tuple(poses.shape[1:]) != (3, 4) or tuple(images.shape) != (n_img, H, W, 3):
        raise MiNerfError(f"poses must be [n,3,4] and images [n,{H},{W},3]; got {tuple(poses.shape)} / {tuple(images.shape)}")
    dev = images.device
    k = K.detach().cpu().numpy() if isinstance(K, torch.Tensor) else np.asarray(K)
    k4 = (C.c_float * 4)(float(np.float32(k[0][0])), float(np.float32(k[1][1])), float(np.float32(k[0][2])), float(np.float32(k[1][2])))
    out = torch.empty(n_img * H * W, 3, 3, dtype=torch.float32, device=dev)
    with _guard(dev):
        check(lib().mi_nerf_rays_rgb(int(W), int(H), k4, dev_ptr(poses, "poses"), dev_ptr(images, "images"), n_img, dev_ptr(out),
                                     stream_ptr(dev)), "mi_nerf_rays_rgb")
    return out


def gather_rows(src: torch.Tensor, idx: torch.Tensor) -> torch.Tensor:
    if idx.dim() != 1 or idx.dtype != torch.int64:
        raise MiNerfError(f"idx must be a 1-d int64 tensor, got {tuple(idx.shape)} {idx.dtype}")
    n_src = src.shape[0]
    row = src.numel() // max(n_src, 1)
    n = int(idx.shape[0])
    dst = torch.empty((n, *src.shape[1:]), dtype=torch.float32, device=src.device)
    if n == 0:
        return dst
    with _guard(src.device):
        check(lib().mi_nerf_permute_rows(dev_ptr(src, "src"), dev_ptr(idx, "idx", torch.int64, 8), n, int(row), dev_ptr(dst), stream_ptr(src.device)),
              "mi_nerf_permute_rows")
    return dst


def permute_rows(src: torch.Tensor, perm: torch.Tensor) -> torch.Tensor:
    n = src.shape[0]
    if perm.shape != (n,):
        raise MiNerfError(f"perm must be [{n}], got {tuple(perm.shape)}")
    return gather_rows(src, perm)


MODE_F32, MODE_BF16, MODE_BF16_64, MODE_BF16_32, MODE_F16S, MODE_F16S_BF16, MODE_F16, MODE_F16_BF16 = 0, 1, 2, 3, 5, 6, 8, 9
PRECISION_FLAGS = ("bf16", "f16s", "coarse_f16s", "f16", "coarse_f16")
_FAMILIES = {(): ("fp32", "fp32"), ("bf16",): ("bf16", "bf16"), ("f16s",): ("f16s", "f16s"), ("bf16", "coarse_f16s"): ("f16s", "bf16"),
             ("f16",): ("f16", "f16"), ("bf16", "coarse_f16"): ("f16", "bf16")}
_MODES = {("fp32", "fp32", 0): MODE_F32, ("bf16", "bf16", 0): MODE_BF16, ("bf16", "bf16", 64): MODE_BF16_64, ("bf16", "bf16", 32): MODE_BF16_32,
          ("f16s", "f16s", 0): MODE_F16S, ("f16s", "bf16", 0): MODE_F16S_BF16, ("f16", "f16", 0): MODE_F16, ("f16", "bf16", 0): MODE_F16_BF16}


class Precision(NamedTuple):
    coarse: str
    fine: str
    points_per_wave: int = 0

    @property
    def mode(self) -> int:
        return _MODES[self]

    @property
    def reads_f16s(self) -> bool:
        return bool({self.coarse, self.fine} & {"f16s", "f16"})


def precision(bf16: bool = False, f16s: bool = False, coarse_f16s: bool = False, f16: bool = False, coarse_f16: bool = False,
              points_per_wave: int = 0) -> Precision:
    on = tuple(k for k, v in zip(PRECISION_FLAGS, (bf16, f16s, coarse_f16s, f16, coarse_f16)) if v)
    if on not in _FAMILIES:
        raise MiNerfError(f"no precision mode sets {' + '.join(on)}: none (fp32), bf16, f16s, f16, or bf16 with one of coarse_f16s / coarse_f16")
    coarse, fine = _FAMILIES[on]
    p = Precision(coarse, fine, 0 if fine in ("fp32", "f16s") else int(points_per_wave))
    if p not in _MODES:
        raise MiNerfError(f"points_per_wave={points_per_wave}: 0 (chosen per launch), or 64 / 32 with bf16 alone")
    return p


def render_cfg(near: float, far: float, Sc: int, Nf: int, det: bool, bf16: bool = False, points_per_wave: int = 0, seed: int = 0,
               ray_offset: int = 0, f16s: bool = False, coarse_f16s: bool = False, f16: bool = False, coarse_f16: bool = False) -> RenderCfg:
    mode = precision(bf16, f16s, coarse_f16s, f16, coarse_f16, points_per_wave).mode
    return RenderCfg(float(near), float(far), int(Sc), int(Nf), int(bool(det)), mode, int(seed) & 0xFFFFFFFF, 0, int(ray_offset))


def workspace_layout(cfg: RenderCfg, n: int) -> WorkspaceLayout:
    wl = WorkspaceLayout()
    check(lib().mi_nerf_render_workspace_layout(C.byref(cfg), n, C.byref(wl)), "mi_nerf_render_workspace_layout")
    return wl


def render_rays(net: Net, packed_c: torch.Tensor, packed_f: Optional[torch.Tensor], cfg: RenderCfg, rays: torch.Tensor,
                t_rand: Optional[torch.Tensor], u: Optional[torch.Tensor], workspace: Optional[torch.Tensor] = None,
                out: Optional[Sequence[torch.Tensor]] = None):
    n = rays.shape[0]
    dev = rays.device
    if tuple(rays.shape) != (n, 6) or (t_rand is not None and tuple(t_rand.shape) != (n, cfg.Sc)):
        raise MiNerfError(f"rays [n,6] / t_rand [n,{cfg.Sc}] expected, got {tuple(rays.shape)} / {None if t_rand is None else tuple(t_rand.shape)}")
    if cfg.Nf > 0 and not cfg.det and u is not None and tuple(u.shape) != (n, cfg.Nf):
        raise MiNerfError(f"u [n,{cfg.Nf}] expected")
    wl = workspace_layout(cfg, n)
    if workspace is None or workspace.numel() < wl.total:
        workspace = torch.empty(max(wl.total, 256), dtype=torch.uint8, device=dev)
    if out is None:
        rgb_c = torch.empty(n, 3, dtype=torch.float32, device=dev)
        disp_c = torch.empty(n, dtype=torch.float32, device=dev)
        rgb_f = torch.empty(n, 3, dtype=torch.float32, device=dev) if cfg.Nf > 0 else None
        disp_f = torch.empty(n, dtype=torch.float32, device=dev) if cfg.Nf > 0 else None
    else:
        rgb_c, disp_c, rgb_f, disp_f = out
    with _guard(dev):
        check(lib().mi_nerf_render_rays(C.byref(net), dev_ptr(packed_c, "packed_coarse", torch.uint8, 16),
                                        dev_ptr(packed_f, "packed_fine", torch.uint8, 16), C.byref(cfg), dev_ptr(rays, "rays"), n,
                                        dev_ptr(t_rand, "t_rand"), dev_ptr(u, "u") if (cfg.Nf > 0 and not cfg.det) else None,
                                        dev_ptr(workspace, "workspace", torch.uint8, 256), workspace.numel(), dev_ptr(rgb_c), dev_ptr(disp_c),
                                        dev_ptr(rgb_f), dev_ptr(disp_f), stream_ptr(dev)), "mi_nerf_render_rays")
    return rgb_c, disp_c, rgb_f, disp_f, workspace


def workspace_views(cfg: RenderCfg, n: int, workspace: torch.Tensor) -> Dict[str, torch.Tensor]:
    wl = workspace_layout(cfg, n)
    Sc, St = cfg.Sc, cfg.Sc + cfg.Nf
    def view(off, shape):
        cnt = int(np.prod(shape))
        return workspace[off:off + cnt * 4].view(torch.float32).view(*shape)
    v = {"z_c": view(wl.z_c, (n, Sc)), "raw_c": view(wl.raw_c, (n, Sc, 4)), "weights_c": view(wl.weights_c, (n, Sc))}
    if cfg.Nf > 0:
        v["z_f"] = view(wl.z_f, (n, St))
        v["raw_f"] = view(wl.raw_f, (n, St, 4))
    return v


def time_mlp_rays(net: Net, packed: torch.Tensor, rays: torch.Tensor, z: torch.Tensor, raw: torch.Tensor, iters: int, bf16: bool = False,
                  points_per_wave: int = 0, f16s: bool = False, f16: bool = False) -> float:
    mode = precision(bf16, f16s, f16=f16, points_per_wave=points_per_wave).mode
    n, S = z.shape
    ms = C.c_float(0.0)
    with _guard(z.device):
        check(lib().mi_nerf_time_mlp_rays(C.byref(net), dev_ptr(packed, "packed", torch.uint8, 16), dev_ptr(rays, "rays"), dev_ptr(z, "z"), n, S,
                                          dev_ptr(raw, "raw", align=16), iters, mode, C.byref(ms),
                                          stream_ptr(z.device)), "mi_nerf_time_mlp_rays")
    return float(ms.value)


def selftest_mfma(device) -> None:
    device = torch.device(device)
    with _guard(device):
        check(lib().mi_nerf_selftest_mfma(stream_ptr(device)), "mi_nerf_selftest_mfma")
```

Measured before the change: 493,500.

## Add fine-only render flag that runs a density-only coarse MLP pass

Adds a MI_NERF_RENDER_FINE_ONLY flag to the render config. When it is set and the coarse family is fp32, the coarse pass uses a new kernel mode that stops after the density head. That mode skips the view-direction encoding, the feature and colour layers, and streaming their weights. Frame rendering in the harness and the distributed path turns the flag on when a fine pass exists, because only the fine colours are used there. The coarse rgb output becomes undefined (None) in that mode, and the flag is rejected for training and geometry outputs.

```diff
diff --git a/include/mi_nerf.h b/include/mi_nerf.h
--- a/include/mi_nerf.h
+++ b/include/mi_nerf.h
@@ -18,6 +18,8 @@
 #define MI_NERF_MODE_F16S_BF16 6
 #define MI_NERF_MODE_F16 8
 #define MI_NERF_MODE_F16_BF16 9
+
+#define MI_NERF_RENDER_FINE_ONLY 1u
 
 #define MI_NERF_OK 0
 #define MI_NERF_EINVAL 1
@@ -121,7 +123,7 @@
     int32_t mode;
 #endif
     uint32_t seed;
-    uint32_t reserved;
+    uint32_t flags;
     int64_t ray_offset;
 } mi_nerf_render_cfg;
 size_t mi_nerf_render_workspace_bytes(const mi_nerf_render_cfg* cfg, int64_t n_rays);
diff --git a/nerf_pytorch_paeng_amd/_lib.py b/nerf_pytorch_paeng_amd/_lib.py
--- a/nerf_pytorch_paeng_amd/_lib.py
+++ b/nerf_pytorch_paeng_amd/_lib.py
@@ -66,7 +66,7 @@
 
 class RenderCfg(C.Structure):
     _fields_ = [("near_", C.c_float), ("far_", C.c_float), ("Sc", C.c_int32), ("Nf", C.c_int32),
-                ("det", C.c_int32), ("mode", C.c_int32), ("seed", C.c_uint32), ("reserved", C.c_uint32), ("ray_offset", C.c_int64)]
+                ("det", C.c_int32), ("mode", C.c_int32), ("seed", C.c_uint32), ("flags", C.c_uint32), ("ray_offset", C.c_int64)]
 
 
 class WorkspaceLayout(C.Structure):
diff --git a/nerf_pytorch_paeng_amd/csrc/api.hip b/nerf_pytorch_paeng_amd/csrc/api.hip
--- a/nerf_pytorch_paeng_amd/csrc/api.hip
+++ b/nerf_pytorch_paeng_amd/csrc/api.hip
@@ -30,6 +30,7 @@
 }
 
 int mlp_rays_fp32(const mi_nerf_net*, const void*, const float*, const float*, int64_t, int, float*, hipStream_t);
+int mlp_rays_fp32_density(const mi_nerf_net*, const void*, const float*, const float*, int64_t, int, float*, hipStream_t);
 int mlp_embedded_fp32(const mi_nerf_net*, const void*, const float*, int64_t, float*, hipStream_t);
 int mlp_rays_bf16(const mi_nerf_net*, const void*, const float*, const float*, int64_t, int, float*, hipStream_t, int points_per_wave, const StratDraw* strat,
                   FineDraw* fine = nullptr);
@@ -406,7 +407,9 @@
     MN_CHECK_ARG(ws_bytes >= L.total, "workspace too small: %zu < %zu", ws_bytes, L.total);
     MN_CHECK_ARG(rays && rgb_c && disp_c && packed_c && (ws || L.total == 0), "NULL pointer");
     MN_CHECK_ARG(cfg->Nf == 0 || (packed_f && rgb_f && disp_f), "fine pass needs packed_fine and outputs");
-    MN_CHECK_ARG(cfg->reserved == 0, "mi_nerf_render_cfg.reserved must be 0");
+    MN_CHECK_ARG((cfg->flags & ~MI_NERF_RENDER_FINE_ONLY) == 0, "mi_nerf_render_cfg.flags 0x%x: only MI_NERF_RENDER_FINE_ONLY (1) is defined", cfg->flags);
+    const bool fine_only = (cfg->flags & MI_NERF_RENDER_FINE_ONLY) != 0;
+    MN_CHECK_ARG(!fine_only || cfg->Nf > 0, "MI_NERF_RENDER_FINE_ONLY with Nf == 0: the coarse colours are the result");
     char* w = (char*)ws;
     float* z_c = (float*)(w + L.z_c);
     float* raw_c = (float*)(w + L.raw_c);
@@ -425,7 +428,9 @@
             return rc;
     } else {
         if (int rc = stage_stratified(n, Sc, cfg->near_, cfg->far_, t_rand, cfg->seed, cfg->ray_offset, z_c, st)) return rc;
-        if (int rc = mlp_rays_family(p.coarse, net, packed_c, rays, z_c, n, Sc, raw_c, st, p.points_per_wave)) return rc;
+        if (fine_only && p.coarse == Family::FP32) {
+            if (int rc = mlp_rays_fp32_density(net, packed_c, rays, z_c, n, Sc, raw_c, st)) return rc;
+        } else if (int rc = mlp_rays_family(p.coarse, net, packed_c, rays, z_c, n, Sc, raw_c, st, p.points_per_wave)) return rc;
     }
     if (cfg->Nf == 0) return stage_composite(raw_c, z_c, rays, 6, n, Sc, rgb_c, disp_c, nullptr, wts_c, nullptr, st);
     {
diff --git a/nerf_pytorch_paeng_amd/csrc/layout.h b/nerf_pytorch_paeng_amd/csrc/layout.h
--- a/nerf_pytorch_paeng_amd/csrc/layout.h
+++ b/nerf_pytorch_paeng_amd/csrc/layout.h
@@ -39,16 +39,25 @@
 
 __host__ __device__ inline uint32_t round_up_u32(uint32_t v, uint32_t m) { return (v + m - 1) / m * m; }
 
+inline uint32_t trunk_stream_quads(int D, int W_net, int skip) {
+    const int W = kernel_width(W_net);
+    const int NT = W / 32;
+    const uint32_t pe_quads = (uint32_t)(pe_ksteps(KERNEL_LX) / 4) * NT;
+    const uint32_t h_quads = (uint32_t)(W / 2 / 4) * NT;
+    uint32_t quads = pe_quads;
+    for (int l = 1; l < D; ++l) quads += h_quads + ((skip >= 0 && l == skip + 1) ? pe_quads : 0);
+    return quads;
+}
+inline uint32_t trunk_stream_bytes(int D, int W_net, int skip) { return trunk_stream_quads(D, W_net, skip) * QUAD_BYTES; }
+
 inline BlobLayout make_layout(int D, int W_net, int skip, int , int ) {
-    constexpr int L_x = KERNEL_LX, L_d = KERNEL_LD;
+    constexpr int L_d = KERNEL_LD;
     const int W = kernel_width(W_net);
     BlobLayout b{};
     const int NT = W / 32;
     const int in_d = 3 + 6 * L_d;
-    const uint32_t pe_quads = (uint32_t)(pe_ksteps(L_x) / 4) * NT;
     const uint32_t h_quads = (uint32_t)(W / 2 / 4) * NT;
-    uint32_t quads = pe_quads;
-    for (int l = 1; l < D; ++l) quads += h_quads + ((skip >= 0 && l == skip + 1) ? pe_quads : 0);
+    uint32_t quads = trunk_stream_quads(D, W_net, skip);
     quads += h_quads;
     quads += (uint32_t)(W / 2 / 4) * (NT / 2);
     b.stream_off = HEADER_BYTES;
diff --git a/nerf_pytorch_paeng_amd/csrc/mlp_fp32.hip b/nerf_pytorch_paeng_amd/csrc/mlp_fp32.hip
--- a/nerf_pytorch_paeng_amd/csrc/mlp_fp32.hip
+++ b/nerf_pytorch_paeng_amd/csrc/mlp_fp32.hip
@@ -64,9 +64,15 @@
     for (int s = 3 * L + 2; s < NPE; ++s) pe[s] = 0.0f;
 }
 
-template <int W, int MODE, int LX, int LD, bool STASH>
+constexpr int MODE_RAYS = 0, MODE_EMBEDDED = 1, MODE_RAYS_DENSITY = 2;
+
+template <int W, int MODE_, int LX, int LD, bool STASH>
 __global__ __launch_bounds__(256) __attribute__((amdgpu_waves_per_eu(1, 1)))
 void mlp_fp32_kernel(const MlpArgs a) {
+    constexpr bool DENSITY = MODE_ == MODE_RAYS_DENSITY;
+    constexpr int MODE = DENSITY ? MODE_RAYS : MODE_;
+    static_assert(MODE_ >= 0 && MODE_ <= 2, "MODE: 0 rays + z, 1 embedded rows, 2 rays + z, density only");
+    static_assert(!(DENSITY && STASH), "the training forward keeps feat and the colour branch's activations");
     constexpr int NT = W / 32;
     constexpr int HN = W / 2;
     constexpr int KPE = pe_ksteps(LX);
@@ -151,7 +157,7 @@
             const float amax = __builtin_fmaxf(__builtin_fmaxf(__builtin_fabsf(p[0]), __builtin_fabsf(p[1])), __builtin_fabsf(p[2])) * (float)(1 << (LX - 1));
             if (__builtin_expect(amax < SINCOS_FAST_LIMIT, 1)) encode_regs<LX, false>(pe, p, hh);
             else encode_regs<LX, true>(pe, p, hh);
-            if (ray != bias_ray) {
+            if (!DENSITY && ray != bias_ray) {
                 bias_ray = ray;
                 const float nrm = __builtin_sqrtf(dx * dx + dy * dy + dz * dz);
                 const float v[3] = {dx / nrm, dy / nrm, dz / nrm};
@@ -219,6 +225,14 @@
         acc_to_b<NT, true>(acc, h);
         MN_STAMP(2);
         const float dens = xhalf_sum(dot_half<HN>(h, side + a.o_dens_w, hh)) + side[a.o_dens_b];
+        if constexpr (DENSITY) {
+            if (valid && hh == 0) {
+                f32x4 o; o[0] = 0.0f; o[1] = 0.0f; o[2] = 0.0f; o[3] = dens;
+                *(f32x4*)(a.out + out_idx * 4) = o;
+            }
+            MN_STAMP(3);
+            continue;
+        }
         acc_init<NT>(acc, side + a.o_bias_feat, hh);
         if constexpr (STASH) {
             float* row = a.stash_h + ((long long)(a.D - 1) * a.stash_rows + out_idx) * W + 4 * hh;
@@ -314,7 +328,8 @@
 template <int W, int MODE, bool STASH = false>
 static int launch(const MlpArgs& args_in, long long n_wtiles, hipStream_t st) {
     MlpArgs args = args_in;
-    const size_t lds = RING_BYTES + (size_t)args.side_floats * 4 + 4 * (W / 2) * 4;
+    constexpr bool DENSITY = MODE == MODE_RAYS_DENSITY;
+    const size_t lds = RING_BYTES + (size_t)args.side_floats * 4 + (DENSITY ? 0 : 4 * (W / 2) * 4);
     MN_CHECK_ARG(lds <= 160 * 1024, "LDS budget exceeded: %zu bytes", lds);
     auto kern = mlp_fp32_kernel<W, MODE, 10, 4, STASH>;
     static LdsOptIn opt_in = {};
@@ -324,12 +339,12 @@
     {
         const long long NW = (long long)grid * 4;
         const long long it_ray = (args.n_rays + NW - 1) / NW * args.tpr, it_flat = (n_wg + grid - 1) / grid;
-        args.ray_major = (MODE == 0 && args.n_rays >= NW && it_ray <= it_flat) ? 1 : 0;
+        args.ray_major = (MODE != MODE_EMBEDDED && args.n_rays >= NW && it_ray <= it_flat) ? 1 : 0;
         if (args.ray_major) {
             args.walk_ray = 0; args.walk_chunk = 1; args.walk_carry = NW;
             args.n_iter = (args.n_rays + NW - 1) / NW * args.tpr;
         } else {
-            const long long tpr = MODE == 0 ? args.tpr : 1;
+            const long long tpr = MODE != MODE_EMBEDDED ? args.tpr : 1;
             args.walk_ray = NW / tpr; args.walk_chunk = (int)(NW % tpr); args.walk_carry = 1;
             args.n_iter = (n_wg + grid - 1) / grid;
         }
@@ -388,8 +403,8 @@
     a.o_wdir_t = L.wdir_t;
 }
 
-int mlp_rays_fp32(const mi_nerf_net* net, const void* packed_dev, const float* rays_dev, const float* z_dev,
-                  int64_t n_rays, int S, float* raw_dev, hipStream_t st) {
+static int rays_fp32(const mi_nerf_net* net, const void* packed_dev, const float* rays_dev, const float* z_dev,
+                     int64_t n_rays, int S, float* raw_dev, hipStream_t st, bool density) {
     if (int rc = check_net(net)) return rc;
     MN_CHECK_ARG(n_rays >= 0 && S >= 1, "bad sizes n_rays=%lld S=%d", (long long)n_rays, S);
     if (n_rays == 0) return MI_NERF_OK;
@@ -399,7 +414,25 @@
     fill_common(a, net, packed_dev, false);
     a.rays = rays_dev; a.z = z_dev; a.out = raw_dev; a.S = S; a.tpr = (S + 31) / 32;
     a.n_wtiles = (long long)n_rays * a.tpr; a.n_rays = n_rays;
+    if (density) {
+        const uint32_t trunk = trunk_stream_bytes(net->D, net->W, net->skip);
+        MN_CHECK_ARG(trunk % SLOT_BYTES == 0 && trunk >= (uint32_t)((NSLOT - 1) * SLOT_BYTES) && trunk < a.stream_bytes,
+                     "density-only pass: the trunk's %u stream bytes are no ring-slot prefix of the stream's %u (D=%d W=%d skip=%d)", trunk,
+                     a.stream_bytes, net->D, net->W, net->skip);
+        a.stream_bytes = trunk;
+        return kernel_width(net->W) == 256 ? launch<256, MODE_RAYS_DENSITY>(a, a.n_wtiles, st) : launch<128, MODE_RAYS_DENSITY>(a, a.n_wtiles, st);
+    }
     return kernel_width(net->W) == 256 ? launch<256, 0>(a, a.n_wtiles, st) : launch<128, 0>(a, a.n_wtiles, st);
+}
+
+int mlp_rays_fp32(const mi_nerf_net* net, const void* packed_dev, const float* rays_dev, const float* z_dev,
+                  int64_t n_rays, int S, float* raw_dev, hipStream_t st) {
+    return rays_fp32(net, packed_dev, rays_dev, z_dev, n_rays, S, raw_dev, st, false);
+}
+
+int mlp_rays_fp32_density(const mi_nerf_net* net, const void* packed_dev, const float* rays_dev, const float* z_dev,
+                          int64_t n_rays, int S, float* raw_dev, hipStream_t st) {
+    return rays_fp32(net, packed_dev, rays_dev, z_dev, n_rays, S, raw_dev, st, true);
 }
 
 int mlp_rays_fp32_stash(const mi_nerf_net* net, const void* packed_dev, const float* rays_dev, const float* z_dev,
diff --git a/nerf_pytorch_paeng_amd/csrc/occ.hip b/nerf_pytorch_paeng_amd/csrc/occ.hip
--- a/nerf_pytorch_paeng_amd/csrc/occ.hip
+++ b/nerf_pytorch_paeng_amd/csrc/occ.hip
@@ -472,7 +472,7 @@
     if (int rc = resolve_grid(grid, &G)) return rc;
     mlp_rays_fn fn;
     if (int rc = mlp_entry(cfg->mode, &fn)) return rc;
-    OCC_CHECK_ARG(cfg->reserved == 0, "mi_nerf_render_cfg.reserved must be 0");
+    OCC_CHECK_ARG(cfg->flags == 0, "mi_nerf_render_cfg.flags must be 0 here (reserved: mi_occ_render_rays keeps its full coarse pass)");
     OCC_CHECK_ARG(net != nullptr, "net is NULL");
     OCC_CHECK_ARG(rays && rgb_c && disp_c && packed_c && bits_c && ws, "NULL pointer (rays, rgb_c, disp_c, packed_coarse, bits_coarse and workspace are required)");
     OCC_CHECK_ARG(cfg->Nf == 0 || (packed_f && bits_f && rgb_f && disp_f), "the fine pass needs packed_fine, bits_fine and its outputs");
diff --git a/nerf_pytorch_paeng_amd/dist.py b/nerf_pytorch_paeng_amd/dist.py
--- a/nerf_pytorch_paeng_amd/dist.py
+++ b/nerf_pytorch_paeng_amd/dist.py
@@ -173,9 +173,10 @@
     _, d = ops.make_o_d(W, H, K, pose, packed.device, row0=r0, n_rows=nr, want_origins=False)
     p = pose if isinstance(pose, torch.Tensor) else torch.as_tensor(pose)
     o = p[:3, -1].to(packed.device, torch.float32).expand(d.shape)
+    fine = int(opts.N_samples_f) > 0
     rc, dc, rf, df = NP.batchify_rays_and_render_by_chunk(o, d, packed, None, H, W, K, opts, seed=seed, ray_offset=r0 * W, bf16=bf16, f16s=f16s,
-                                                          coarse_f16s=coarse_f16s)
-    rgb, disp = (rc, dc) if int(opts.N_samples_f) == 0 else (rf, df)
+                                                          coarse_f16s=coarse_f16s, **({"fine_only": True} if fine else {}))
+    rgb, disp = (rf, df) if fine else (rc, dc)
     return torch.cat([rgb, disp[:, None]], -1)
 
 
diff --git a/nerf_pytorch_paeng_amd/harness.py b/nerf_pytorch_paeng_amd/harness.py
--- a/nerf_pytorch_paeng_amd/harness.py
+++ b/nerf_pytorch_paeng_amd/harness.py
@@ -162,9 +162,12 @@
 def _render_pose(model, posenc, K, pose, hw, opts):
     img_h, img_w = hw
     rays_o, rays_d = make_o_d(img_w, img_h, K, pose[:3, :4])
+    from .train_path import wants_grad
+    fine = int(opts.N_samples_f) > 0
     rgb_c, disp_c, rgb_f, disp_f = NP.batchify_rays_and_render_by_chunk(rays_o, rays_d, model, posenc, img_h, img_w, K, opts, **_precision(opts),
-                                                                        occupancy=getattr(opts, "occupancy", None))
-    return (rgb_c, disp_c) if int(opts.N_samples_f) == 0 else (rgb_f, disp_f)
+                                                                        occupancy=getattr(opts, "occupancy", None),
+                                                                        **({"fine_only": True} if fine and not wants_grad(model) else {}))
+    return (rgb_f, disp_f) if fine else (rgb_c, disp_c)
 
 
 def test(idx, i_test, posenc, model, test_imgs, gt_intrinsic, gt_extrinsic, hw, opts, *, log_dir: Optional[str] = None,
diff --git a/nerf_pytorch_paeng_amd/nerf_process.py b/nerf_pytorch_paeng_amd/nerf_process.py
--- a/nerf_pytorch_paeng_amd/nerf_process.py
+++ b/nerf_pytorch_paeng_amd/nerf_process.py
@@ -116,12 +116,13 @@
 
 
 def _render(rays: torch.Tensor, packed: PackedNeRF, opts, t_rand, u, seed: int, ray_offset: int, prec: ops.Precision,
-            intermediates: bool, occupancy=None, geometry: bool = False) -> Dict[str, torch.Tensor]:
+            intermediates: bool, occupancy=None, geometry: bool = False, fine_only: bool = False) -> Dict[str, torch.Tensor]:
     n = rays.shape[0]
     dev = rays.device
     Sc, Nf = int(opts.N_samples_c), int(opts.N_samples_f)
     det = _det(opts)
-    cfg = ops.render_cfg(float(opts.near), float(opts.far), Sc, Nf, det, seed=seed, ray_offset=ray_offset)
+    cfg = ops.render_cfg(float(opts.near), float(opts.far), Sc, Nf, det, seed=seed, ray_offset=ray_offset,
+                         fine_only=fine_only and occupancy is None)
     cfg.mode = prec.mode
     if t_rand is not None:
         t_rand = as_f32_dev(t_rand, dev)
@@ -143,7 +144,7 @@
         rgb_c, disp_c, rgb_f, disp_f, ws, stats = occ.render_rays(net, blob_c, blob_f if Nf > 0 else None, cfg, occupancy, rays, t_rand, u)
         occupancy.last_stats = occ.add_stats(occupancy.last_stats, stats)
         views = occ.workspace_views
-    out = {"rgb_c": rgb_c, "disp_c": disp_c}
+    out = {"rgb_c": None if fine_only else rgb_c, "disp_c": disp_c}
     if Nf > 0:
         out["rgb_f"], out["disp_f"] = rgb_f, disp_f
     if geometry:
@@ -197,6 +198,21 @@
     return {**({"geometry": True} if geometry else {}), **({"ray_grad": True} if ray_grad else {})}
 
 
+def _fine_only_arg(fine_only, training: bool, geometry, opts) -> None:
+    if not fine_only:
+        return
+    if training:
+        raise MiNerfError("fine_only=True is an inference feature: the training loss reads rgb_c")
+    if geometry:
+        raise MiNerfError("fine_only=True with geometry=True is not built: the coarse geometry outputs are read from the coarse pass")
+    if int(opts.N_samples_f) <= 0:
+        raise MiNerfError("fine_only=True needs N_samples_f > 0: without a fine pass the coarse colours are the result")
+
+
+def _fine_only_kw(fine_only) -> Dict[str, bool]:
+    return {"fine_only": True} if fine_only else {}
+
+
 def _ray_grad_arg(ray_grad, train_occupancy) -> bool:
     if ray_grad and train_occupancy is not None:
         raise MiNerfError("ray_grad=True with train_occupancy= is not built: the occupancy-training node differentiates the parameters only")
@@ -205,10 +221,11 @@
 
 def render_rays(rays, model, posenc, opts, *, t_rand=None, u=None, seed=None, ray_offset: int = 0, bf16: bool = False,
                 return_intermediates: bool = False, f16s: bool = False, coarse_f16s: bool = False, f16: bool = False, coarse_f16: bool = False,
-                occupancy=None, train_occupancy=None, geometry: bool = False, ray_grad: bool = False):
+                occupancy=None, train_occupancy=None, geometry: bool = False, ray_grad: bool = False, fine_only: bool = False):
     prec = ops.precision(bf16, f16s, coarse_f16s, f16, coarse_f16)
     ray_grad = _ray_grad_arg(ray_grad, train_occupancy)
     training = train_path.wants_grad(model) or train_path.wants_ray_grad(model, ray_grad, rays)
+    _fine_only_arg(fine_only, training, geometry, opts)
     occupancy = _occupancy_arg(occupancy, training, prec)
     train_occupancy = _train_occupancy_arg(train_occupancy, training, prec)
     if training:
@@ -226,16 +243,18 @@
         raise MiNerfError(f"rays must be [n, 6] (o, d), got {tuple(rays.shape)}")
     if occupancy is not None and rays.shape[0] > occ.MAX_RAYS_PER_LAUNCH:
         raise MiNerfError(f"render_rays with a grid takes at most {occ.MAX_RAYS_PER_LAUNCH} rays per call (batchify_rays_and_render_by_chunk slabs them)")
-    return _render(rays, packed, opts, t_rand, u, _next_seed(seed), int(ray_offset), prec, return_intermediates, occupancy, **_geometry_kw(geometry))
+    return _render(rays, packed, opts, t_rand, u, _next_seed(seed), int(ray_offset), prec, return_intermediates, occupancy, **_geometry_kw(geometry),
+                   **_fine_only_kw(fine_only))
 
 
 def batchify_rays_and_render_by_chunk(ray_o, ray_d, model, posenc, H, W, K, opts, *, t_rand=None, u=None, seed=None,
                                       ray_offset: int = 0, bf16: bool = False, f16s: bool = False, coarse_f16s: bool = False, f16: bool = False,
                                       coarse_f16: bool = False, occupancy=None, train_occupancy=None, geometry: bool = False,
-                                      ray_grad: bool = False):
+                                      ray_grad: bool = False, fine_only: bool = False):
     prec = ops.precision(bf16, f16s, coarse_f16s, f16, coarse_f16)
     ray_grad = _ray_grad_arg(ray_grad, train_occupancy)
     training = train_path.wants_grad(model) or train_path.wants_ray_grad(model, ray_grad, ray_o, ray_d)
+    _fine_only_arg(fine_only, training, geometry, opts)
     occupancy = _occupancy_arg(occupancy, training, prec)
     train_occupancy = _train_occupancy_arg(train_occupancy, training, prec)
     train_f16s = _train_f16s(prec) if training else False
@@ -271,12 +290,13 @@
             parts.append(train_path.render_train(rays[i:j].contiguous(), model, opts, t_rand=tr, u=uu, seed=seed,
                                                  ray_offset=int(ray_offset) + i, f16s=train_f16s, **_geometry_kw(geometry, ray_grad)))
         else:
-            parts.append(_render(rays[i:j], packed, opts, tr, uu, seed, int(ray_offset) + i, prec, False, occupancy, **_geometry_kw(geometry)))
+            parts.append(_render(rays[i:j], packed, opts, tr, uu, seed, int(ray_offset) + i, prec, False, occupancy, **_geometry_kw(geometry),
+                                 **_fine_only_kw(fine_only)))
     if train_occupancy is not None:
         train_occupancy.last_stats = train_stats
     def cat(key):
         return parts[0][key] if len(parts) == 1 else torch.cat([p[key] for p in parts], dim=0)
-    res = (cat("rgb_c"), cat("disp_c"), cat("rgb_f"), cat("disp_f")) if Nf > 0 else (cat("rgb_c"), cat("disp_c"), None, None)
+    res = (None if fine_only else cat("rgb_c"), cat("disp_c"), cat("rgb_f"), cat("disp_f")) if Nf > 0 else (cat("rgb_c"), cat("disp_c"), None, None)
     if geometry:
         return (*res, {name + "_" + key: cat(name + "_" + key) for key in (("c", "f") if Nf > 0 else ("c",)) for name in geo.EXTRA_KEYS})
     return res
diff --git a/nerf_pytorch_paeng_amd/ops.py b/nerf_pytorch_paeng_amd/ops.py
--- a/nerf_pytorch_paeng_amd/ops.py
+++ b/nerf_pytorch_paeng_amd/ops.py
@@ -573,6 +573,7 @@
 
 MODE_F32, MODE_BF16, MODE_BF16_64, MODE_BF16_32, MODE_F16S, MODE_F16S_BF16, MODE_F16, MODE_F16_BF16 = 0, 1, 2, 3, 5, 6, 8, 9
 PRECISION_FLAGS = ("bf16", "f16s", "coarse_f16s", "f16", "coarse_f16")
+RENDER_FINE_ONLY = 1
 _FAMILIES = {(): ("fp32", "fp32"), ("bf16",): ("bf16", "bf16"), ("f16s",): ("f16s", "f16s"), ("bf16", "coarse_f16s"): ("f16s", "bf16"),
              ("f16",): ("f16", "f16"), ("bf16", "coarse_f16"): ("f16", "bf16")}
 _MODES = {("fp32", "fp32", 0): MODE_F32, ("bf16", "bf16", 0): MODE_BF16, ("bf16", "bf16", 64): MODE_BF16_64, ("bf16", "bf16", 32): MODE_BF16_32,
@@ -606,9 +607,11 @@
 
 
 def render_cfg(near: float, far: float, Sc: int, Nf: int, det: bool, bf16: bool = False, points_per_wave: int = 0, seed: int = 0,
-               ray_offset: int = 0, f16s: bool = False, coarse_f16s: bool = False, f16: bool = False, coarse_f16: bool = False) -> RenderCfg:
+               ray_offset: int = 0, f16s: bool = False, coarse_f16s: bool = False, f16: bool = False, coarse_f16: bool = False,
+               fine_only: bool = False) -> RenderCfg:
     mode = precision(bf16, f16s, coarse_f16s, f16, coarse_f16, points_per_wave).mode
-    return RenderCfg(float(near), float(far), int(Sc), int(Nf), int(bool(det)), mode, int(seed) & 0xFFFFFFFF, 0, int(ray_offset))
+    return RenderCfg(float(near), float(far), int(Sc), int(Nf), int(bool(det)), mode, int(seed) & 0xFFFFFFFF,
+                     RENDER_FINE_ONLY if fine_only else 0, int(ray_offset))
 
 
 def workspace_layout(cfg: RenderCfg, n: int) -> WorkspaceLayout:
```

Result: no change. 492,300 (-0.3%).
